# voutcn/megahit

Hardware: NVIDIA H100
Metric: sorted (k+1)-mer edges/sec at k=27 on 150bp reads (higher is better)
Workload: dtype u32

## Files before the change

include/mhb.h:

```cpp
#ifndef MHB_H
#define MHB_H
#include <stddef.h>
#include <stdint.h>

#ifdef __cplusplus
extern "C" {
#endif

#define MHB_OK 0
#define MHB_ERR_ARG 1
#define MHB_ERR_CUDA 2
#define MHB_ERR_IO 3
#define MHB_ERR_NOMEM 4

#define MHB_NUM_BUCKETS 65536
#define MHB_MAX_MUL 65535
#define MHB_MAX_K 255
#define MHB_SENTINEL_OFFSET 0xFFFFFFFFu

const char *mhb_last_error(void);
const char *mhb_version(void);
int mhb_device_count(void);
uint64_t mhb_launch_count(void);

uint32_t mhb_count_record_words(uint32_t k);
uint32_t mhb_words_per_edge(uint32_t k);
uint32_t mhb_s2s_record_words(uint32_t k);
uint32_t mhb_count_sort_bytes(uint32_t k, uint8_t *bytes);
uint32_t mhb_s2s_sort_bytes(uint32_t k, uint8_t *bytes);
size_t mhb_sort_workspace_bytes(uint64_t n, uint32_t words);


typedef struct {
  const uint32_t *bin;
  uint64_t bin_words;
  uint64_t n_reads;
  uint32_t fixed_len;
  const uint64_t *rec_off;
  const uint64_t *edge_off;
} mhb_dev_reads;

int mhb_count_extract(void *stream, const mhb_dev_reads *reads, uint32_t k, uint32_t *records,
                      uint64_t n_edges, uint64_t *hist256, int hist_byte);

int mhb_check_fixed_len(void *stream, const uint32_t *bin_dev, uint64_t n_reads, uint32_t fixed_len, uint64_t *flag_dev);

int mhb_count_extract_range(void *stream, const mhb_dev_reads *reads, uint32_t k, uint32_t lo, uint32_t hi, int write,
                            uint64_t *per_read, uint32_t *records, uint64_t *hist256, int hist_byte,
                            uint64_t *total_dev);

int mhb_count_extract_owners(void *stream, const mhb_dev_reads *reads, uint32_t k, uint64_t *hist16,
                             const uint8_t *owner_of_byte, const uint64_t *owner_base, uint64_t *cursor_dev,
                             const uint64_t *capacity_dev, const uint32_t *round_lo, const uint32_t *round_hi);

int mhb_sort_records(void *stream, uint32_t *a, uint32_t *b, uint64_t n, uint32_t words,
                     const uint8_t *bytes, uint32_t n_bytes, const uint64_t *first_hist, void *ws,
                     size_t ws_bytes, int *result_in_b);

int mhb_sort_records_relaxed(void *stream, uint32_t *a, uint32_t *b, uint64_t n, uint32_t words, const uint8_t *bytes,
                             uint32_t n_bytes, const uint64_t *first_hist, void *ws, size_t ws_bytes, int *result_in_b);

int mhb_s2s_sort(void *stream, uint32_t *a, uint32_t *b, uint64_t n, uint32_t k, const uint64_t *first_hist, void *ws,
                 size_t ws_bytes, int *result_in_b);
size_t mhb_s2s_sort_workspace_bytes(uint64_t n, uint32_t k);
int mhb_s2s_sort_hist_byte(uint64_t n, uint32_t k);
void mhb_s2s_sort_stats(uint64_t *n_oversized, uint64_t *oversized_items, uint64_t *n_large);

int mhb_s2s_sort_emit(void *stream, uint32_t *a, uint32_t *b, uint64_t n, uint32_t k, const uint64_t *first_hist,
                      uint8_t *bytes_out, uint64_t capacity_bytes, uint64_t *bucket_table, uint64_t *totals, void *ws,
                      size_t ws_bytes);
size_t mhb_s2s_sort_emit_workspace_bytes(uint64_t n, uint32_t k);

int mhb_partition_scatter(void *stream, const uint32_t *recs, uint64_t n, uint32_t words, int byte,
                          const uint8_t *owner_of_byte_dev, const uint64_t *bin_addr_dev, void *ws, size_t ws_bytes);
int mhb_partition_scatter_hist(void *stream, const uint32_t *recs, uint64_t n, uint32_t words, int byte,
                               const uint8_t *owner_of_byte_dev, const uint64_t *bin_addr_dev, void *ws, size_t ws_bytes,
                               int next_byte, uint64_t *owner_next_hist);
int mhb_plan_partition(void *stream, const uint64_t *hist_all_dev, uint32_t world, uint32_t rank, uint32_t record_bytes,
                       const uint64_t *peer_base_host, uint8_t *owner_lut_dev, uint64_t *bin_addr_dev, uint64_t *plan_dev);
int mhb_compact_tip_edges(void *stream, const uint32_t *edges, const uint8_t *aux, uint64_t n_solid, uint32_t k,
                          uint32_t *tips_out, uint8_t *tip_aux_out, uint64_t capacity, uint64_t *cursor_dev);
int mhb_dev_malloc(void **ptr, size_t bytes);
int mhb_dev_free(void *ptr);
int mhb_ipc_export(const void *dev_ptr, uint8_t *handle64);
int mhb_ipc_open(const uint8_t *handle64, void **peer_ptr);
int mhb_ipc_close(void *peer_ptr);

int mhb_sort_pass_ms(int back, double *pass_ms, uint32_t max_passes, uint32_t *n_passes, uint64_t *n_records,
                     uint32_t *words);

size_t mhb_count_solid_scratch_bytes(uint64_t n);
int mhb_count_solid(void *stream, const uint32_t *sorted_records, uint64_t n, uint32_t k, int32_t m,
                    uint32_t *edges_out, uint8_t *aux_out, uint64_t capacity_edges, uint64_t *mul_hist,
                    uint64_t *n_solid_out, void *scratch, size_t scratch_bytes);

int mhb_count_hashed_supported(uint32_t k, int32_t m);
size_t mhb_count_hashed_workspace_bytes(uint64_t n, uint32_t k, int32_t m);
int mhb_count_solid_hashed(void *stream, uint32_t *recs_a, uint32_t *recs_b, uint64_t n, uint32_t k, int32_t m,
                           const uint64_t *hist_byte5, uint32_t *edges_out, uint8_t *aux_out, uint64_t capacity_edges,
                           uint64_t *mul_hist, uint64_t *n_solid_out, void *ws, size_t ws_bytes);

size_t mhb_tipset_bytes(uint64_t n_tip_edges, uint32_t k);
int mhb_tipset_build(void *stream, const uint32_t *edges, const uint8_t *aux, uint64_t n_solid, uint32_t k,
                     void *tipset, size_t tipset_bytes, uint64_t n_tip_edges);
int mhb_count_mark_mercy(void *stream, const mhb_dev_reads *reads, uint32_t k, const void *tipset,
                         size_t tipset_bytes, uint64_t n_tip_edges, uint32_t *first_0_out, uint32_t *last_0_in);
int mhb_count_tip_edges(void *stream, const uint8_t *aux, uint64_t n_solid, uint64_t *n_tip_host);

size_t mhb_mercy_candidates_scratch_bytes(uint64_t n_reads);
int mhb_mercy_candidates(void *stream, const uint32_t *first_0_out, const uint32_t *last_0_in, uint64_t n_reads,
                         uint64_t *cand_ids, uint64_t *n_cand_host, void *scratch, size_t scratch_bytes);
size_t mhb_mercy_edges_scratch_bytes(uint64_t n_cand, uint32_t max_read_len);
int mhb_mercy_edges(void *stream, const mhb_dev_reads *reads, const uint64_t *cand_ids, uint64_t n_cand,
                    uint32_t max_read_len, uint32_t k, const uint32_t *edges, uint64_t n_edges, uint32_t *mercy_out,
                    uint64_t capacity, uint64_t *n_mercy_host, void *scratch, size_t scratch_bytes);
int mhb_mercy_edges_count(void *stream, const mhb_dev_reads *reads, const uint64_t *cand_ids, uint64_t n_cand,
                          uint32_t max_read_len, uint32_t k, uint32_t n_segs, const uint32_t *const *seg_edges,
                          const uint64_t *seg_counts, const void *const *seg_luts, const uint8_t *owner_of_byte,
                          uint64_t *n_mercy_host, void *scratch, size_t scratch_bytes);
int mhb_mercy_edges_write(void *stream, const mhb_dev_reads *reads, const uint64_t *cand_ids, uint64_t n_cand,
                          uint32_t max_read_len, uint32_t k, uint32_t *mercy_out, uint64_t capacity, uint64_t n_mercy,
                          void *scratch, size_t scratch_bytes);

size_t mhb_mercy_planes_words(uint64_t n_cand, uint32_t max_read_len);
int mhb_mercy_probe_owned(void *stream, const mhb_dev_reads *reads, const uint64_t *cand_ids, uint64_t n_cand,
                          uint32_t max_read_len, uint32_t k, const uint32_t *edges, uint64_t n_edges, const void *lut,
                          const uint8_t *owner_of_byte, uint32_t me, uint32_t *planes_out);
int mhb_mercy_count_planes(void *stream, const mhb_dev_reads *reads, const uint64_t *cand_ids, uint64_t n_cand,
                           uint32_t max_read_len, uint32_t k, const uint32_t *planes, uint32_t n_src,
                           uint64_t src_stride_words, uint64_t *n_mercy_host, void *scratch, size_t scratch_bytes);

int mhb_mercy_edges_segs(void *stream, const mhb_dev_reads *reads, const uint64_t *cand_ids, uint64_t n_cand,
                         uint32_t max_read_len, uint32_t k, uint32_t n_segs, const uint32_t *const *seg_edges,
                         const uint64_t *seg_counts, const void *const *seg_luts, const uint8_t *owner_of_byte,
                         uint32_t *mercy_out, uint64_t capacity, uint64_t *n_mercy_host, void *scratch,
                         size_t scratch_bytes);
size_t mhb_edge_lut_bytes(void);
int mhb_edge_lut_build(void *stream, const uint32_t *edges, uint64_t n_edges, uint32_t k, void *lut);

typedef struct {
  const uint32_t *words;
  uint64_t n_words;
  uint64_t n_seqs;
  uint32_t fixed_len;
  const uint64_t *word_off;
  const uint32_t *len;
  const uint64_t *item_off;
  const uint16_t *mult;
  uint32_t fixed_stride;
} mhb_dev_seqs;

int mhb_s2s_extract(void *stream, const mhb_dev_seqs *seqs, uint32_t k, uint32_t *records, uint64_t n_items,
                    uint64_t *hist256, int hist_byte);

int mhb_s2s_extract_edges_pruned(void *stream, const uint32_t *edges, const uint8_t *aux, uint64_t n_edges,
                                 uint64_t n_with_aux, uint32_t k, uint32_t *records, uint64_t capacity,
                                 uint64_t *cursor_dev, uint64_t *hist256, int hist_byte);

int mhb_s2s_extract_range(void *stream, const mhb_dev_seqs *seqs, uint32_t k, uint32_t *records, uint64_t n_items,
                          uint32_t lo, uint32_t hi, uint64_t *cursor_dev, uint64_t capacity, uint64_t *hist256,
                          int hist_byte);

int mhb_s2s_extract_owners(void *stream, const mhb_dev_seqs *seqs, uint32_t k, uint64_t n_items,
                           const uint8_t *owner_of_byte, const uint64_t *owner_base, uint64_t *cursor_dev,
                           const uint64_t *capacity_dev);
int mhb_s2s_bucket_hist(void *stream, const mhb_dev_seqs *seqs, uint32_t k, uint64_t n_items, uint64_t *hist16);
int mhb_s2s_extract_owners_round(void *stream, const mhb_dev_seqs *seqs, uint32_t k, uint64_t n_items,
                                 const uint8_t *owner_of_byte, const uint64_t *owner_base, uint64_t *cursor_dev,
                                 const uint64_t *capacity_dev, const uint32_t *round_lo, const uint32_t *round_hi);
int mhb_s2s_edges_owners(void *stream, const uint32_t *edges, const uint8_t *aux, uint64_t n_edges, uint64_t n_with_aux,
                         uint32_t k, uint64_t *hist16, const uint8_t *owner_of_byte, const uint64_t *owner_base,
                         uint64_t *cursor_dev, const uint64_t *capacity_dev, const uint32_t *round_lo,
                         const uint32_t *round_hi);

size_t mhb_s2s_emit_scratch_bytes(uint64_t n, uint32_t k);
int mhb_s2s_emit(void *stream, const uint32_t *sorted_records, uint64_t n, uint32_t k, uint8_t *bytes_out,
                 uint64_t capacity_bytes, uint64_t *bucket_table, uint64_t *totals, void *scratch,
                 size_t scratch_bytes);

int mhb_s2s_emit_fmt(void *stream, const uint32_t *sorted_records, uint64_t n, uint32_t k, uint8_t *bytes_out,
                     uint64_t capacity_bytes, uint64_t *bucket_table, uint64_t *totals, void *scratch,
                     size_t scratch_bytes, int label_fmt);

int mhb_set_device(int device);

typedef struct {
  uint32_t k;
  int32_t m;
  const uint32_t *bin;
  uint64_t bin_words;
  uint64_t n_reads;
  int want_mercy;
} mhb_count_args;

typedef struct {
  uint64_t n_edge_records;
  uint64_t n_solid;
  uint32_t words_per_edge;
  uint32_t *edges;
  uint64_t n_cand;
  uint64_t *cand_ids;
  uint64_t n_has_tips;
  int64_t counting[MHB_MAX_MUL + 1];
  double t_h2d_ms, t_extract_ms, t_sort_ms, t_count_ms, t_mercy_ms, t_d2h_ms, t_total_ms;
  uint32_t n_sort_passes;
  uint32_t n_rounds;
  double sort_pass_ms[64];
} mhb_count_result;

int mhb_count_host(const mhb_count_args *args, mhb_count_result *res);
int mhb_set_round_limit(uint64_t max_records_per_round);
int mhb_set_s2s_round_limit(uint64_t max_items_per_round);
uint64_t mhb_sdbg_round_budget(uint64_t avail_bytes, uint64_t fixed_bytes, uint32_t k, uint64_t n_total);
int mhb_plan_rounds(const uint64_t *hist256, uint64_t max_records, uint32_t *lo_out, uint32_t *hi_out);
int mhb_plan_rounds16(const uint64_t *hist256, const uint64_t *sub_hist, uint64_t max_records, uint32_t *lo16_out,
                      uint32_t *hi16_out, uint32_t cap_out);

int mhb_plan_read_chunks(const uint32_t *bin, uint64_t bin_words, uint64_t n_reads, uint64_t max_chunk_bytes,
                         uint64_t *first_read_out, uint32_t cap_out);
int mhb_read_stream_decide(uint64_t resident_bytes, uint64_t avail_bytes, int plan_failed, uint64_t chunk_limit);
int mhb_set_read_chunk_limit(uint64_t bytes);
int mhb_read_stream_stats(uint64_t *n_chunks, uint64_t *n_passes, uint64_t *h2d_bytes);
int mhb_read_stream_times(double *h2d_ms, double *kernel_ms, double *fill_ms, double *pass_ms);

typedef struct {
  uint32_t k;
  const uint32_t *words;
  const uint64_t *word_off;
  const uint32_t *len;
  const uint16_t *mult;
  uint64_t n_seqs;
} mhb_s2s_args;

typedef struct {
  uint64_t n_records;
  uint64_t n_items, n_tips, n_large_mul, n_bytes;
  uint32_t words_per_tip_label;
  uint8_t *bytes;
  uint64_t bucket_table[MHB_NUM_BUCKETS * 4];
  uint64_t w_count[9];
  uint64_t ones_in_last;
  double t_total_ms, t_extract_ms, t_sort_ms, t_emit_ms;
} mhb_s2s_result;

int mhb_s2s_host(const mhb_s2s_args *args, mhb_s2s_result *res);
int mhb_set_s2s_chunk_limit(uint64_t bytes);
int mhb_plan_seq_chunks(const uint64_t *word_off, const uint32_t *len, uint64_t n_seqs, uint32_t k, uint64_t max_chunk_bytes,
                        uint64_t *first_seq_out, uint32_t cap_out);
int mhb_plan_mercy_segments(const uint32_t *edges, uint64_t n_edges, uint32_t k, uint64_t max_segment_bytes,
                            uint32_t *first_byte_out, uint32_t cap_out);
int mhb_s2s_stream_stats(int mercy, uint64_t *n_chunks, uint64_t *n_passes, uint64_t *n_rounds, uint64_t *h2d_bytes);
int mhb_s2s_stream_times(int mercy, double *h2d_ms, double *kernel_ms, double *fill_ms, double *pass_ms);
int mhb_selftest_s2s_stream_decide(uint64_t n_seqs, uint64_t n_words, uint32_t k, uint64_t free_bytes, uint64_t chunk_limit,
                                   uint64_t *resident_bytes, int *stream);
int mhb_selftest_mercy_auto_plan(const uint64_t *byte_edges, uint32_t k, uint64_t n_cand_reads, uint64_t cand_words,
                                 uint32_t max_read_len, uint64_t free_bytes, uint32_t *first_byte_out, uint64_t *slot_bytes);
int mhb_selftest_mercy_stream_decide(uint64_t n_edges, uint32_t k, uint64_t n_cand_reads, uint64_t cand_words,
                                     uint32_t max_read_len, uint64_t free_bytes, uint64_t chunk_limit,
                                     uint64_t *resident_bytes, int *stream);

typedef struct {
  uint32_t k;
  int32_t m;
  const uint32_t *bin;
  uint64_t bin_words;
  uint64_t n_reads;
  int32_t need_mercy;
  int32_t want_edges;
  uint8_t *sdbg_out;
  uint64_t sdbg_out_capacity;
} mhb_build_args;

typedef struct {
  uint64_t n_edge_records, n_solid, n_cand, n_mercy, n_sort_items;
  uint32_t words_per_edge, words_per_tip_label;
  uint64_t n_items, n_tips, n_large_mul, n_bytes;
  uint8_t *bytes;
  uint64_t *bucket_table;
  uint64_t w_count[9];
  uint64_t ones_in_last;
  uint32_t *edges;
  uint64_t *cand_ids;
  int64_t *counting;
  double t_total_ms, t_h2d_ms, t_count_ms, t_mercy_ms, t_s2s_ms, t_d2h_ms;
  uint32_t n_rounds_s1, n_rounds_s2;
} mhb_build_result;

int mhb_build_host(const mhb_build_args *args, mhb_build_result *res);

int mhb_read2sdbg_host(const mhb_build_args *args, mhb_build_result *res);
int mhb_set_r2s_round_limit(uint64_t max_s1_records, uint64_t max_s2_items);
int mhb_set_r2s_sparse_mercy(int mode);
int mhb_r2s_mercy_stats(int *sparse, uint64_t *n_entries, uint64_t *host_bytes);

typedef struct {
  uint32_t k, step;
  const uint32_t *contig_words;
  const uint64_t *contig_word_off;
  const uint32_t *contig_len;
  uint64_t n_contigs;
  const uint32_t *bin;
  uint64_t bin_words;
  uint64_t n_reads;
} mhb_iterate_args;

typedef struct {
  uint64_t n_flanks;
  uint64_t n_aligned_reads;
  uint64_t n_candidates;
  uint64_t n_edges;
  uint32_t words_per_edge;
  uint32_t *edges;
  double t_total_ms;
} mhb_iterate_result;

int mhb_iterate_host(const mhb_iterate_args *args, mhb_iterate_result *res);

typedef struct {
  const char *type;
  const uint8_t *data[2];
  uint64_t size[2];
} mhb_buildlib_lib;

typedef struct {
  const mhb_buildlib_lib *libs;
  uint32_t n_libs;
} mhb_buildlib_args;

typedef struct {
  uint32_t *bin;
  uint64_t bin_words;
  uint64_t n_reads, n_bases;
  uint32_t n_libs;
  uint64_t *lib_begin, *lib_end;
  uint32_t *lib_max_len;
  uint64_t n_chunks;
  uint64_t n_walk_passes;
  double t_total_ms;
} mhb_buildlib_result;

int mhb_buildlib_host(const mhb_buildlib_args *args, mhb_buildlib_result *res);
void mhb_buildlib_free(mhb_buildlib_result *res);
int mhb_set_buildlib_chunk(uint64_t bytes);

int mhb_mercy_host(uint32_t k, const uint32_t *edges, uint64_t n_edges, const uint32_t *cand_bin, uint64_t cand_words,
                   uint32_t **mercy_out, uint64_t *n_mercy_out, uint64_t *n_cand_reads_out);

void mhb_free(void *p);
int mhb_release(void);

typedef struct {
  uint32_t k;
  int32_t m;
  double host_mem;
  int32_t num_cpu_threads;
  const char *read_lib_file;
  const char *output_prefix;
  int32_t mem_flag;
} mhb_count_opts;

typedef struct {
  double host_mem;
  uint32_t k;
  uint32_t k_from;
  int32_t num_cpu_threads;
  const char *contig;
  const char *bubble;
  const char *addi_contig;
  const char *local_contig;
  const char *input_prefix;
  const char *output_prefix;
  int32_t need_mercy;
  int32_t mem_flag;
} mhb_seq2sdbg_opts;

typedef struct {
  uint32_t k;
  int32_t m;
  double host_mem;
  int32_t num_cpu_threads;
  const char *read_lib_file;
  const char *output_prefix;
  int32_t mem_flag;
  int32_t need_mercy;
} mhb_read2sdbg_opts;

typedef struct {
  const char *contig_file;
  const char *bubble_file;
  const char *read_file;
  int32_t num_cpu_threads;
  uint32_t k;
  uint32_t step;
  const char *output_prefix;
} mhb_iterate_opts;

int mhb_count_run(const mhb_count_opts *opts);
int mhb_seq2sdbg_run(const mhb_seq2sdbg_opts *opts);
int mhb_iterate_run(const mhb_iterate_opts *opts);
int mhb_read2sdbg_run(const mhb_read2sdbg_opts *opts);
int mhb_buildlib_run(const char *lib_file, const char *out_prefix);

int mhb_count_run_multi(const mhb_count_opts *opts, int n_gpus);
// ... 62 lines not shown
```

megahit_b200/csrc/mhb_count.cuh:

```cuda
#pragma once
#include <stdlib.h>
#include <string.h>

#include "mhb.h"
#include "mhb_kernels.cuh"

namespace mhb {

static constexpr int kReadsPerBatch = 64;
static constexpr int kStageWords = 4096;
static constexpr int kExtractThreads = 256;

struct ReadsView {
  const u32 *bin;
  u64 bin_words;
  u64 n_reads;
  u32 fixed_len;
  u32 fixed_stride;
  const u64 *rec_off;
  const u64 *edge_off;
  __device__ __forceinline__ u64 rec_start(u64 r) const { return fixed_len ? r * fixed_stride : rec_off[r]; }
};

template <class F>
__device__ __forceinline__ void for_each_read(const ReadsView &rv, F &&f) {
  __shared__ __align__(16) u32 s_stage[2][kStageWords];
  __shared__ __align__(8) u64 s_bar[2];
  const u32 tid = threadIdx.x, warp = tid >> 5;
  constexpr int NW = kExtractThreads / 32;
  const u64 n_batches = (rv.n_reads + kReadsPerBatch - 1) / kReadsPerBatch;
  if (tid == 0) {
    mbar_init(&s_bar[0], 1);
    mbar_init(&s_bar[1], 1);
    mbar_fence_init();
  }
  __syncthreads();

  auto geom = [&](u64 b, u64 &r0, u64 &r1, u64 &a0, u64 &a1) {
    r0 = b * kReadsPerBatch;
    r1 = r0 + kReadsPerBatch < rv.n_reads ? r0 + kReadsPerBatch : rv.n_reads;
    const u64 w0 = rv.rec_start(r0);
    const u64 w1 = r1 < rv.n_reads ? rv.rec_start(r1) : rv.bin_words;
    a0 = w0 & ~3ull;
    a1 = (w1 + 3) & ~3ull;
  };
  auto issue = [&](u64 b, int st) {
    u64 r0, r1, a0, a1;
    geom(b, r0, r1, a0, a1);
    if (a1 - a0 <= (u64)kStageWords && tid == 0) {
      const u32 bytes = (u32)(a1 - a0) * 4;
      mbar_expect_tx(&s_bar[st], bytes);
      bulk_g2s(&s_stage[st][0], rv.bin + a0, bytes, &s_bar[st]);
    }
  };

  u32 parity[2] = {0, 0};
  u64 b = blockIdx.x;
  int st = 0;
  if (b < n_batches) issue(b, 0);
  for (; b < n_batches; b += gridDim.x, st ^= 1) {
    const u64 nb = b + gridDim.x;
    if (nb < n_batches) issue(nb, st ^ 1);
    u64 r0, r1, a0, a1;
    geom(b, r0, r1, a0, a1);
    const bool staged = (a1 - a0) <= (u64)kStageWords;
    if (staged) {
      mbar_wait(&s_bar[st], parity[st]);
      parity[st] ^= 1;
    }
    for (u64 r = r0 + warp; r < r1; r += NW) {
      const u64 w = rv.rec_start(r);
      const u32 *rec = staged ? &s_stage[st][w - a0] : rv.bin + w;
      const u32 L = rec[0];
      f(r, rec + 1, div_ceil(L, 16), L);
    }
    __syncthreads();
  }
}

template <int W, int WR>
__global__ void __launch_bounds__(kExtractThreads)
    k_count_extract(ReadsView rv, u32 k, u32 *__restrict__ records, u64 *hist, int hist_byte) {
  __shared__ u32 s_hist[256];
  for (int i = threadIdx.x; i < 256; i += kExtractThreads) s_hist[i] = 0;
  const u32 lane = lane_id();
  const u32 K1 = k + 1;
  for_each_read(rv, [&](u64 r, const u32 *s, u32 nwords, u32 L) {
    if (L < K1) return;
    const u32 n_e = L - k;
    const u64 base = rv.fixed_len ? r * (u64)(rv.fixed_len - k) : rv.edge_off[r];
    for (u32 q0 = 0; q0 < n_e; q0 += 32) {
      const u32 q = q0 + lane;
      if (q < n_e) {
        u32 rec[WR], strand;
        make_count_record<W, WR>(s, nwords, L, k, q, rec, strand);
        st_rec<WR>(records, base + q, rec);
        if (hist) atomicAdd(&s_hist[rec_byte<WR>(rec, hist_byte)], 1u);
      }
    }
  });
  __syncthreads();
  if (hist)
    for (int i = threadIdx.x; i < 256; i += kExtractThreads)
      if (s_hist[i]) atomicAdd((unsigned long long *)&hist[i], (unsigned long long)s_hist[i]);
}

static __global__ void __launch_bounds__(kExtractThreads)
    k_count_extract_roll(ReadsView rv, u32 k, u32 *__restrict__ records, u64 *hist, int hist_byte) {
  __shared__ u32 s_hist[256];
  for (int i = threadIdx.x; i < 256; i += kExtractThreads) s_hist[i] = 0;
  const u32 lane = lane_id();
  const u32 K1 = k + 1;
  const u32 hshift = 8u * (u32)hist_byte;
  for_each_read(rv, [&](u64 r, const u32 *s, u32 nwords, u32 L) {
    if (L < K1) return;
    const u32 n_e = L - k;
    const u64 base = rv.fixed_len ? r * (u64)(rv.fixed_len - k) : rv.edge_off[r];
    for (u32 q0 = 0; q0 < n_e; q0 += 128) {
      const u32 q = q0 + 4 * lane;
      if (q < n_e) {
        u64 rec[4];
        u32 strand[4];
        make_count_records_roll<4>(s, nwords, L, k, q, rec, strand);
        const u32 cnt = n_e - q < 4u ? n_e - q : 4u;
#pragma unroll
        for (int j = 0; j < 4; ++j) {
          if ((u32)j < cnt) {
            reinterpret_cast<uint2 *>(records)[base + q + j] = make_uint2((u32)(rec[j] >> 32), (u32)rec[j]);
            if (hist) atomicAdd(&s_hist[(u32)(rec[j] >> hshift) & 255u], 1u);
          }
        }
      }
    }
  });
  __syncthreads();
  if (hist)
    for (int i = threadIdx.x; i < 256; i += kExtractThreads)
      if (s_hist[i]) atomicAdd((unsigned long long *)&hist[i], (unsigned long long)s_hist[i]);
}

template <int W, int WR, bool WRITE>
__global__ void __launch_bounds__(kExtractThreads)
    k_count_extract_range(ReadsView rv, u32 k, u32 lo, u32 hi, u64 *__restrict__ per_read, u32 *__restrict__ records,
                          u64 *hist, int hist_byte) {
  __shared__ u32 s_hist[256];
  for (int i = threadIdx.x; i < 256; i += kExtractThreads) s_hist[i] = 0;
  const u32 lane = lane_id();
  const u32 lt_mask = lanemask_lt();
  const u32 K1 = k + 1;
  for_each_read(rv, [&](u64 r, const u32 *s, u32 nwords, u32 L) {
    if (L < K1) {
      if (!WRITE && lane == 0) per_read[r] = 0;
      return;
    }
    const u32 n_e = L - k;
    u64 run = WRITE ? per_read[r] : 0ull;
    for (u32 q0 = 0; q0 < n_e; q0 += 32) {
      const u32 q = q0 + lane;
      u32 rec[WR], strand;
      bool in = false;
      if (q < n_e) {
        make_count_record<W, WR>(s, nwords, L, k, q, rec, strand);
        const u32 top = rec[0] >> 16;
        in = top >= lo && top <= hi;
      }
      const u32 mask = __ballot_sync(0xffffffffu, in);
      if (in) {
        if constexpr (WRITE) st_rec<WR>(records, run + __popc(mask & lt_mask), rec);
        if (hist) atomicAdd(&s_hist[rec_byte<WR>(rec, hist_byte)], 1u);
      }
      run += __popc(mask);
    }
    if (!WRITE && lane == 0) per_read[r] = run;
  });
  __syncthreads();
  if (hist)
    for (int i = threadIdx.x; i < 256; i += kExtractThreads)
      if (s_hist[i]) atomicAdd((unsigned long long *)&hist[i], (unsigned long long)s_hist[i]);
}

enum { kCountOwnHist = 0, kCountOwnWrite = 1 };
template <int W, int WR, int MODE>
__global__ void __launch_bounds__(kExtractThreads)
    k_count_extract_owners(ReadsView rv, u32 k, unsigned long long *__restrict__ hist16, OwnerSink sink,
                           const u32 *__restrict__ round_lo, const u32 *__restrict__ round_hi) {
  const u32 lane = lane_id(), lt = lanemask_lt();
  const u32 K1 = k + 1;
  for_each_read(rv, [&](u64, const u32 *s, u32 nwords, u32 L) {
    if (L < K1) return;
    const u32 n_e = L - k;
    for (u32 q0 = 0; q0 < n_e; q0 += 32) {
      const u32 q = q0 + lane;
      u32 rec[WR], strand;
      bool in = q < n_e;
      u32 b = 0xFFFFFFFFu;
      if (in) {
        make_count_record<W, WR>(s, nwords, L, k, q, rec, strand);
        b = rec[0] >> 16;
      }
      if constexpr (MODE == kCountOwnHist) {
        const u32 peers = __match_any_sync(0xffffffffu, b);
        if (in && lane == (u32)__ffs(peers) - 1) atomicAdd(hist16 + b, (unsigned long long)__popc(peers));
      } else {
        if (in) {
          const u32 o = __ldg(sink.owner + (b >> 8));
          in = b >= __ldg(round_lo + o) && b <= __ldg(round_hi + o);
        }
        const u32 mask = __ballot_sync(0xffffffffu, in);
        if (mask) sink.template put<WR>(in, rec, mask, lane, lt);
      }
    }
  });
}

template <int WR>
__device__ __forceinline__ bool same_edge(const u32 (&a)[WR], const u32 (&b)[WR]) {
  bool eq = true;
#pragma unroll
  for (int j = 0; j < WR; ++j) {
    const u32 m = (j == WR - 1) ? ~63u : ~0u;
    eq = eq && ((a[j] & m) == (b[j] & m));
  }
  return eq;
}

static constexpr int kMulHistSmem = 1024;

static __global__ void __launch_bounds__(1024) k_scan_u64(u64 *v, u64 nb, u64 *total_out) {
  __shared__ u64 s_w[33];
  __shared__ u64 s_carry;
  if (threadIdx.x == 0) s_carry = 0;
  __syncthreads();
  const u32 lane = lane_id(), warp = threadIdx.x >> 5;
  for (u64 base = 0; base < nb; base += 1024) {
    const u64 i = base + threadIdx.x;
    const u64 x = i < nb ? v[i] : 0;
    u64 inc = x;
#pragma unroll
    for (int d = 1; d < 32; d <<= 1) {
      u64 t = __shfl_up_sync(0xffffffffu, inc, d);
      if (lane >= (u32)d) inc += t;
    }
    if (lane == 31) s_w[warp] = inc;
    __syncthreads();
    if (warp == 0) {
      u64 w = s_w[lane], winc = w;
#pragma unroll
      for (int d = 1; d < 32; d <<= 1) {
        u64 t = __shfl_up_sync(0xffffffffu, winc, d);
        if (lane >= (u32)d) winc += t;
      }
      s_w[lane] = winc - w;
      if (lane == 31) s_w[32] = winc;
    }
    __syncthreads();
    if (i < nb) v[i] = s_carry + s_w[warp] + inc - x;
    __syncthreads();
    if (threadIdx.x == 0) s_carry += s_w[32];
    __syncthreads();
  }
  if (threadIdx.x == 0 && total_out) *total_out = s_carry;
}

struct TipsetHeader {
  u64 capacity;
  u64 filter_words;
  u32 fold;
  u32 filter_bits;
  u32 resident;
  u32 reserved;
};
static_assert(sizeof(TipsetHeader) == 32, "tip set header");
static constexpr u64 kTipFilterSmemWords = 224 * 1024 / 4;
static constexpr u64 kTipMul = 0x9E3779B97F4A7C15ull;

struct TipsetPlan {
  u64 capacity, filter_words;
  u32 fold, filter_bits, resident;
  __host__ __device__ u64 global_words() const { return fold * filter_words; }
  __host__ __device__ u64 folded_words() const { return fold > 1 ? filter_words : 0; }
};

inline TipsetPlan tipset_plan(u64 n_tip, const char *spec) {
  TipsetPlan p;
  p.capacity = 1024;
  while (p.capacity < 2 * n_tip) p.capacity <<= 1;
  char *end = nullptr;
  const unsigned long long forced = spec && *spec ? strtoull(spec, &end, 10) : 0ull;
  if (forced > 0 && end && *end == '\0') {
    p.filter_words = (forced + 3) & ~3ull;
    p.fold = 1;
    p.resident = p.filter_words <= kTipFilterSmemWords;
  } else {
    const u64 want = ((n_tip + 1) / 2 + 3) & ~3ull;
    p.filter_words = want < 1024 ? 1024 : (want > kTipFilterSmemWords ? kTipFilterSmemWords : want);
    p.fold = (u32)((n_tip + p.filter_words - 1) / p.filter_words);
    if (p.fold < 1) p.fold = 1;
    p.resident = 3 * n_tip <= 32 * kTipFilterSmemWords && !(spec && !strcmp(spec, "global"));
  }
  const u64 probed_words = p.resident ? p.filter_words : p.global_words();
  p.filter_bits = 32 * probed_words >= 5 * n_tip ? 3 : 2;
  return p;
}
__host__ __device__ constexpr u32 tipset_slot_words(u32 W) { return W == 2 ? 4u : W + 1; }

template <int W>
__device__ __forceinline__ u32 hash_key(const u32 (&key)[W]) {
  u32 h = 0x9E3779B1u;
#pragma unroll
  for (int j = 0; j < W; ++j) {
    h = (h ^ key[j]) * 0x85EBCA77u;
    h ^= h >> 15;
  }
  h *= 0x2C1B3C6Du;
  return h ^ (h >> 13);
}

__device__ __forceinline__ u64 tip_filter_hash64(u64 key, u32 K1) { return (key >> (64 - 2 * K1)) * kTipMul; }
template <int W>
__device__ __forceinline__ u64 tip_filter_hash(const u32 (&key)[W], u32 K1) {
  if constexpr (W == 1) {
    return (u64)(key[0] >> (32 - 2 * K1)) * kTipMul;
  } else if constexpr (W == 2) {
    return tip_filter_hash64(((u64)key[0] << 32) | key[1], K1);
  } else {
    u64 a = 0;
#pragma unroll
    for (int j = 0; j < W; j += 2) {
      a = (a ^ (((u64)key[j] << 32) | (j + 1 < W ? key[j + 1] : 0u))) * kTipMul;
      a ^= a >> 32;
    }
    return a * kTipMul;
  }
}
__device__ __forceinline__ u32 tip_filter_word(u64 h, u32 n_words) { return __umulhi((u32)(h >> 32), n_words); }
__device__ __forceinline__ u32 tip_filter_mask(u64 h, u32 bits) {
  const u32 lo = (u32)h;
  return (1u << (lo >> 27)) | (1u << ((lo >> 22) & 31u)) | (bits > 2 ? 1u << ((lo >> 17) & 31u) : 0u);
}

static __global__ void k_count_tips(const uint8_t *aux, u64 n, unsigned long long *out) {
  u64 c = 0;
  for (u64 i = (u64)blockIdx.x * blockDim.x + threadIdx.x; i < n; i += (u64)gridDim.x * blockDim.x)
    c += aux[i] != 0;
  for (int d = 16; d; d >>= 1) c += __shfl_xor_sync(0xffffffffu, c, d);
  if (lane_id() == 0 && c) atomicAdd(out, (unsigned long long)c);
}

template <int W>
__global__ void k_tipset_insert(const u32 *__restrict__ edges, const uint8_t *__restrict__ aux, u64 n, u32 k,
                                u32 *filter, TipsetPlan plan, u32 *table) {
  const u64 i = (u64)blockIdx.x * blockDim.x + threadIdx.x;
  if (i >= n || aux[i] == 0) return;
  const u32 WE = words_per_edge(k), SW = tipset_slot_words(W);
  u32 key[W];
#pragma unroll
  for (int j = 0; j < W; ++j) {
    const u32 keep = 2 * (k + 1) - 32 * j;
    key[j] = edges[i * WE + j] & top_mask(keep > 32 ? 32 : keep);
  }
  const u64 fh = tip_filter_hash<W>(key, k + 1);
  atomicOr(&filter[tip_filter_word(fh, (u32)plan.global_words())], tip_filter_mask(fh, plan.filter_bits));
  const u64 cap = plan.capacity;
  u64 slot = hash_key<W>(key) & (cap - 1);
  while (true) {
    u32 *e = table + slot * SW;
    if (atomicCAS(e, 0u, (u32)aux[i]) == 0u) {
#pragma unroll
      for (int j = 0; j < W; ++j) e[1 + j] = key[j];
      return;
    }
    slot = (slot + 1) & (cap - 1);
  }
}

static __global__ void k_tipset_fold(const u32 *__restrict__ filter, u64 n, u32 fold, u32 *__restrict__ folded) {
  for (u64 i = (u64)blockIdx.x * blockDim.x + threadIdx.x; i < n; i += (u64)gridDim.x * blockDim.x) {
    u32 w = 0;
    for (u32 j = 0; j < fold; ++j) w |= filter[i * fold + j];
    folded[i] = w;
  }
}

static constexpr int kMarkThreads = 1024;

struct TipsetDev {
  const u32 *filter;
  const u32 *table;
  u32 n1, n2, filter_bits;
  u64 cap;
  bool smem;
};
__device__ __forceinline__ TipsetDev tipset_open(const void *tipset, u32 smem_words, u32 *s_filter) {
  const TipsetHeader hd = *reinterpret_cast<const TipsetHeader *>(tipset);
  TipsetPlan p;
  p.capacity = hd.capacity;
  p.filter_words = hd.filter_words;
  p.fold = hd.fold;
  TipsetDev t;
  t.filter = reinterpret_cast<const u32 *>((const char *)tipset + sizeof(TipsetHeader));
  t.table = t.filter + p.global_words() + p.folded_words();
  t.filter_bits = hd.filter_bits;
  t.cap = hd.capacity;
  t.smem = hd.resident && hd.filter_words <= smem_words;
  t.n1 = t.smem ? (u32)hd.filter_words : (u32)p.global_words();
  t.n2 = t.smem && hd.fold > 1 ? (u32)p.global_words() : 0u;
  if (t.smem) {
// ... 571 lines not shown
```

megahit_b200/csrc/mhb_device.cu:

```cuda
#include <cuda_runtime.h>
#include <stdarg.h>
#include <stdio.h>
#include <stdlib.h>
#include <string.h>

#include "mhb.h"
#include "mhb_count.cuh"
#include "mhb_internal.h"
#include "mhb_mercy.cuh"
#include "mhb_s2s.cuh"
#include "mhb_common.cuh"

using namespace mhb;

static thread_local char g_err[1024] = "";
int mhb_set_error(int code, const char *fmt, ...) {
  va_list ap;
  va_start(ap, fmt);
  vsnprintf(g_err, sizeof(g_err), fmt, ap);
  va_end(ap);
  return code;
}
extern "C" const char *mhb_last_error(void) { return g_err; }
extern "C" const char *mhb_version(void) { return "megahit_b200 0.1 (sm_90a; formats of megahit v1.2.9)"; }
extern "C" int mhb_device_count(void) {
  int n = 0;
  if (cudaGetDeviceCount(&n) != cudaSuccess) {
    cudaGetLastError();
    return 0;
  }
  return n;
}
extern "C" void mhb_free(void *p) { free(p); }
unsigned long long g_mhb_launches = 0;
extern "C" uint64_t mhb_launch_count(void) { return g_mhb_launches; }


extern "C" uint32_t mhb_count_record_words(uint32_t k) { return count_record_words(k); }
extern "C" uint32_t mhb_words_per_edge(uint32_t k) { return words_per_edge(k); }
extern "C" uint32_t mhb_s2s_record_words(uint32_t k) { return s2s_record_words(k); }

extern "C" uint32_t mhb_count_sort_bytes(uint32_t k, uint8_t *bytes) {
  const u32 wr = count_record_words(k), total_bits = 32 * wr, key_bits = 2 * (k + 1);
  const u32 lo = (total_bits - key_bits) / 8;
  u32 n = 0;
  for (u32 b = lo; b < 4 * wr; ++b) bytes[n++] = (uint8_t)b;
  return n;
}
extern "C" uint32_t mhb_s2s_sort_bytes(uint32_t k, uint8_t *bytes) {
  const u32 w = s2s_record_words(k), total_bits = 32 * w, key_bits = 2 * k;
  const u32 lo = (total_bits - key_bits) / 8;
  u32 n = 0;
  for (u32 b = 2; b < 4 * w; ++b)
    if (b == 2 || b >= lo) bytes[n++] = (uint8_t)b;
  return n;
}


static int g_sm_count = 0;
static int g_bound_device = -1;
int mhb_sm_count() {
  if (!g_sm_count) {
    int dev = 0;
    cudaGetDevice(&dev);
    cudaDeviceGetAttribute(&g_sm_count, cudaDevAttrMultiProcessorCount, dev);
    if (g_sm_count <= 0) g_sm_count = 132;
    if (g_bound_device < 0) g_bound_device = dev;
  }
  return g_sm_count;
}

ReadsView make_reads_view(const mhb_dev_reads *r) {
  ReadsView v;
  v.bin = r->bin;
  v.bin_words = r->bin_words;
  v.n_reads = r->n_reads;
  v.fixed_len = r->fixed_len;
  v.fixed_stride = r->fixed_len ? 1 + div_ceil(r->fixed_len, 16) : 0;
  v.rec_off = r->rec_off;
  v.edge_off = r->edge_off;
  return v;
}

int check_reads(const mhb_dev_reads *r, uint32_t k) {
  if (!r || k < 1 || k > MHB_MAX_K) return mhb_set_error(MHB_ERR_ARG, "bad reads/k (k=%u)", k);
  if (r->n_reads && !r->bin) return mhb_set_error(MHB_ERR_ARG, "reads->bin is NULL");
  if (((uintptr_t)r->bin & 15) != 0) return mhb_set_error(MHB_ERR_ARG, "reads->bin must be 16-byte aligned");
  if (!r->fixed_len && r->n_reads && (!r->rec_off || !r->edge_off))
    return mhb_set_error(MHB_ERR_ARG, "variable-length reads need rec_off and edge_off");
  return MHB_OK;
}

static int grow_scratch(size_t bytes, void **out) {
  static void *buf[64] = {nullptr};
  static size_t cap[64] = {0};
  int dev = 0;
  CK(cudaGetDevice(&dev));
  if (dev < 0 || dev >= 64) return mhb_set_error(MHB_ERR_CUDA, "device index %d out of range", dev);
  if (cap[dev] < bytes) {
    CK(cudaDeviceSynchronize());
    if (buf[dev]) cudaFree(buf[dev]);
    buf[dev] = nullptr;
    cap[dev] = 0;
    const size_t want = (bytes + 4095) & ~(size_t)4095;
    CK(cudaMalloc(&buf[dev], want));
    cap[dev] = want;
  }
  *out = buf[dev];
  return MHB_OK;
}
static int scan64(cudaStream_t st, u64 *v, u64 n, u64 *total_dev, u64 *bsum);

static __global__ void k_check_fixed_len(const u32 *__restrict__ bin, u64 n_reads, u32 stride, u32 L, unsigned long long *flag) {
  bool bad = false;
  for (u64 r = (u64)blockIdx.x * blockDim.x + threadIdx.x; r < n_reads; r += (u64)gridDim.x * blockDim.x) bad |= bin[r * stride] != L;
  if (__any_sync(0xffffffffu, bad) && (threadIdx.x & 31) == 0) atomicOr(flag, 1ull);
}
extern "C" int mhb_check_fixed_len(void *stream, const uint32_t *bin_dev, uint64_t n_reads, uint32_t fixed_len, uint64_t *flag_dev) {
  if (n_reads == 0) return MHB_OK;
  if (!bin_dev || !flag_dev || !fixed_len) return mhb_set_error(MHB_ERR_ARG, "bad arguments");
  k_check_fixed_len<<<mhb_sm_count() * 8, 256, 0, (cudaStream_t)stream>>>(bin_dev, n_reads, 1 + div_ceil(fixed_len, 16), fixed_len,
                                                                     (unsigned long long *)flag_dev);
  CK_LAUNCH();
  return MHB_OK;
}

extern "C" int mhb_count_extract(void *stream, const mhb_dev_reads *reads, uint32_t k, uint32_t *records,
                                 uint64_t n_edges, uint64_t *hist256, int hist_byte) {
  if (int rc = check_reads(reads, k)) return rc;
  if (reads->n_reads == 0 || n_edges == 0) return MHB_OK;
  cudaStream_t st = (cudaStream_t)stream;
  const ReadsView rv = make_reads_view(reads);
  const u32 W = count_key_words(k), WR = count_record_words(k);
  const int grid = (int)grid_cap(rv.n_reads, kReadsPerBatch, 8);
  static const bool roll = getenv("MHB_EXTRACT_ROLL") && !strcmp(getenv("MHB_EXTRACT_ROLL"), "1");
  if (roll && W == 2 && WR == 2 && k + 1 >= 17) {
    k_count_extract_roll<<<grid, kExtractThreads, 0, st>>>(rv, k, records, hist256, hist_byte);
    CK_LAUNCH();
    return MHB_OK;
  }
#define M(WW)                                                                                              \
  if (W == WW && WR == WW)                                                                                 \
    k_count_extract<WW, WW><<<grid, kExtractThreads, 0, st>>>(rv, k, records, hist256, hist_byte);         \
  else if (W == WW && WR == WW + 1)                                                                        \
    k_count_extract<WW, WW + 1><<<grid, kExtractThreads, 0, st>>>(rv, k, records, hist256, hist_byte);     \
  else
  MHB_FOR_W(M) return mhb_set_error(MHB_ERR_ARG, "unsupported k=%u", k);
#undef M
  CK_LAUNCH();
  return MHB_OK;
}

extern "C" int mhb_count_extract_range(void *stream, const mhb_dev_reads *reads, uint32_t k, uint32_t lo, uint32_t hi,
                                       int write, uint64_t *per_read, uint32_t *records, uint64_t *hist256, int hist_byte,
                                       uint64_t *total_dev) {
  if (int rc = check_reads(reads, k)) return rc;
  if (lo > hi || hi > 65535) return mhb_set_error(MHB_ERR_ARG, "bad bucket range [%u, %u]", lo, hi);
  if (!per_read || (write && !records) || (!write && !total_dev)) return mhb_set_error(MHB_ERR_ARG, "null buffer");
  cudaStream_t st = (cudaStream_t)stream;
  if (reads->n_reads == 0) {
    if (!write) CK(cudaMemsetAsync(total_dev, 0, 8, st));
    return MHB_OK;
  }
  const ReadsView rv = make_reads_view(reads);
  const u32 W = count_key_words(k), WR = count_record_words(k);
  const int grid = (int)grid_cap(rv.n_reads, kReadsPerBatch, 8);
#define M2(WW, WRR)                                                                                                   \
  if (W == WW && WR == WRR) {                                                                                         \
    if (write)                                                                                                        \
      k_count_extract_range<WW, WRR, true><<<grid, kExtractThreads, 0, st>>>(rv, k, lo, hi, per_read, records, hist256, hist_byte); \
    else                                                                                                              \
      k_count_extract_range<WW, WRR, false><<<grid, kExtractThreads, 0, st>>>(rv, k, lo, hi, per_read, records, hist256, hist_byte); \
  } else
#define M(WW) M2(WW, WW) M2(WW, WW + 1)
  MHB_FOR_W(M) return mhb_set_error(MHB_ERR_ARG, "unsupported k=%u", k);
#undef M
#undef M2
  CK_LAUNCH();
  if (!write) {
    u64 *bsum = nullptr;
    if (int rc = grow_scratch(((rv.n_reads / kScanTile) + 2) * 8, (void **)&bsum)) return rc;
    if (int rc = scan64(st, per_read, rv.n_reads, total_dev, bsum)) return rc;
    CK(cudaMemcpyAsync(per_read + rv.n_reads, total_dev, 8, cudaMemcpyDeviceToDevice, st));
  }
  return MHB_OK;
}

extern "C" int mhb_count_extract_owners(void *stream, const mhb_dev_reads *reads, uint32_t k, uint64_t *hist16,
                                        const uint8_t *owner_of_byte, const uint64_t *owner_base, uint64_t *cursor_dev,
                                        const uint64_t *capacity_dev, const uint32_t *round_lo, const uint32_t *round_hi) {
  if (int rc = check_reads(reads, k)) return rc;
  if (!hist16 && (!owner_of_byte || !owner_base || !cursor_dev || !capacity_dev || !round_lo || !round_hi))
    return mhb_set_error(MHB_ERR_ARG, "bad args");
  if (reads->n_reads == 0) return MHB_OK;
  cudaStream_t st = (cudaStream_t)stream;
  const ReadsView rv = make_reads_view(reads);
  const u32 W = count_key_words(k), WR = count_record_words(k);
  const int grid = (int)grid_cap(rv.n_reads, kReadsPerBatch, 8);
  const OwnerSink sink{owner_of_byte, owner_base, (unsigned long long *)cursor_dev, capacity_dev};
  unsigned long long *h = (unsigned long long *)hist16;
#define M2(WW, WRR)                                                                                                         \
  if (W == WW && WR == WRR) {                                                                                               \
    if (hist16)                                                                                                             \
      k_count_extract_owners<WW, WRR, kCountOwnHist><<<grid, kExtractThreads, 0, st>>>(rv, k, h, sink, round_lo, round_hi);  \
    else                                                                                                                    \
      k_count_extract_owners<WW, WRR, kCountOwnWrite><<<grid, kExtractThreads, 0, st>>>(rv, k, h, sink, round_lo, round_hi); \
  } else
#define M(WW) M2(WW, WW) M2(WW, WW + 1)
  MHB_FOR_W(M) return mhb_set_error(MHB_ERR_ARG, "unsupported k=%u", k);
#undef M
#undef M2
  CK_LAUNCH();
  return MHB_OK;
}

extern "C" int mhb_count_solid(void *stream, const uint32_t *sorted_records, uint64_t n, uint32_t k, int32_t m,
                               uint32_t *edges_out, uint8_t *aux_out, uint64_t capacity_edges, uint64_t *mul_hist,
                               uint64_t *n_solid_out, void *scratch, size_t scratch_bytes) {
  if (k < 1 || k > MHB_MAX_K || !mul_hist || !n_solid_out) return mhb_set_error(MHB_ERR_ARG, "bad args");
  if (n == 0) return MHB_OK;
  const size_t need = mhb_count_solid_scratch_bytes(n);
  if (scratch_bytes < need) return mhb_set_error(MHB_ERR_ARG, "count scratch too small (%zu < %zu)", scratch_bytes, need);
  cudaStream_t st = (cudaStream_t)stream;
  const u32 WR = count_record_words(k);
  {
#define M(WW)                                                                                                          \
  if (WR == WW) {                                                                                                      \
    constexpr int CH = 32 * count3_ipl(WW);                                                                            \
    const u64 n_chunks = (n + CH - 1) / CH;                                                                            \
    if (n_chunks >= (1ull << 32)) return mhb_set_error(MHB_ERR_ARG, "too many records for one count launch");          \
    const u64 n_sblk = (n_chunks + kScanTile - 1) / kScanTile;                                                         \
    char *p = (char *)scratch;                                                                                         \
    u32 *ticket = (u32 *)p;                                                                                            \
    p += 256;                                                                                                          \
    uint2 *solid_list = (uint2 *)p;                                                                                    \
    p += pad256((size_t)n_chunks * CH * 8);                                                                            \
    u32 *chunk_count = (u32 *)p;                                                                                       \
    p += pad256((size_t)n_chunks * 4);                                                                                 \
    u64 *chunk_off = (u64 *)p;                                                                                         \
    p += pad256((size_t)n_chunks * 8);                                                                                 \
    u64 *bsum = (u64 *)p;                                                                                              \
    CK(cudaMemsetAsync(ticket, 0, 256, st));                                                                           \
    const size_t smem = (size_t)kCount3Warps * count3_warp_words(WW) * 4;                                              \
    static int bps = 0;                                                                                                \
    if (!bps) {                                                                                                        \
      CK(cudaFuncSetAttribute(k_count_lanes<WW>, cudaFuncAttributeMaxDynamicSharedMemorySize, (int)smem));             \
      CK(cudaOccupancyMaxActiveBlocksPerMultiprocessor(&bps, k_count_lanes<WW>, kCount3Warps * 32, smem));             \
      if (bps < 1) bps = 1;                                                                                            \
    }                                                                                                                  \
    u64 grid = (u64)sm_count() * bps;                                                                                  \
    if (grid > (n_chunks + kCount3Warps - 1) / kCount3Warps) grid = (n_chunks + kCount3Warps - 1) / kCount3Warps;      \
    k_count_lanes<WW><<<(unsigned)grid, kCount3Warps * 32, smem, st>>>(sorted_records, n, k, m, (u32)n_chunks, ticket,  \
                                                                      solid_list, chunk_count, mul_hist);             \
    CK_LAUNCH();                                                                                                       \
    k_scan32_sums<<<(unsigned)n_sblk, kScanThreads, 0, st>>>(chunk_count, n_chunks, bsum);                             \
    CK_LAUNCH();                                                                                                       \
    k_scan_u64<<<1, 1024, 0, st>>>(bsum, n_sblk, n_solid_out);                                                         \
    CK_LAUNCH();                                                                                                       \
    k_scan32_apply<<<(unsigned)n_sblk, kScanThreads, 0, st>>>(chunk_count, n_chunks, bsum, chunk_off);                 \
    CK_LAUNCH();                                                                                                       \
    k_count_write<WW><<<grid_cap(n_chunks, 8, 16), 256, 0, st>>>(sorted_records, k, (u32)n_chunks, solid_list, chunk_count, \
                                                    chunk_off, edges_out, aux_out, capacity_edges);                   \
  }
    MHB_FOR_WR(M)
#undef M
    CK_LAUNCH();
    return MHB_OK;
  }
  return mhb_set_error(MHB_ERR_ARG, "unsupported k=%u", k);
}

extern "C" size_t mhb_count_solid_scratch_bytes(uint64_t n) {
  return (size_t)(n + 1024) * 8 + (size_t)(n / 128 + 2) * 12 + (size_t)(n / 128 / kScanTile + 2) * 8 + 4096;
}

static TipsetPlan tipset_plan_env(uint64_t n_tip) { return tipset_plan(n_tip, getenv("MHB_TIPSET_FILTER")); }

extern "C" size_t mhb_tipset_bytes(uint64_t n_tip_edges, uint32_t k) {
  const TipsetPlan p = tipset_plan_env(n_tip_edges);
  return sizeof(TipsetHeader) + (p.global_words() + p.folded_words()) * 4 +
         p.capacity * (size_t)tipset_slot_words(count_key_words(k)) * 4;
}

static int small_scratch(unsigned long long **out) {
  static unsigned long long *buf[64] = {nullptr};
  int dev = 0;
  CK(cudaGetDevice(&dev));
  if (dev < 0 || dev >= 64) return mhb_set_error(MHB_ERR_CUDA, "device index %d out of range", dev);
  if (!buf[dev]) CK(cudaMalloc((void **)&buf[dev], 256));
  *out = buf[dev];
  return MHB_OK;
}

extern "C" int mhb_count_tip_edges(void *stream, const uint8_t *aux, uint64_t n_solid, uint64_t *n_tip_host) {
  cudaStream_t st = (cudaStream_t)stream;
  unsigned long long *d = nullptr;
  *n_tip_host = 0;
  if (n_solid == 0) return MHB_OK;
  if (int rc = small_scratch(&d)) return rc;
  CK(cudaMemsetAsync(d, 0, 8, st));
  k_count_tips<<<sm_count() * 4, 256, 0, st>>>(aux, n_solid, d);
  CK_LAUNCH();
  CK(cudaMemcpyAsync(n_tip_host, d, 8, cudaMemcpyDeviceToHost, st));
  CK(cudaStreamSynchronize(st));
  return MHB_OK;
}

extern "C" int mhb_tipset_build(void *stream, const uint32_t *edges, const uint8_t *aux, uint64_t n_solid, uint32_t k,
                                void *tipset, size_t tipset_bytes, uint64_t n_tip_edges) {
  if (tipset_bytes < mhb_tipset_bytes(n_tip_edges, k)) return mhb_set_error(MHB_ERR_ARG, "tipset too small");
  cudaStream_t st = (cudaStream_t)stream;
  const TipsetPlan plan = tipset_plan_env(n_tip_edges);
  TipsetHeader hdr;
  memset(&hdr, 0, sizeof(hdr));
  hdr.capacity = plan.capacity;
  hdr.filter_words = plan.filter_words;
  hdr.fold = plan.fold;
  hdr.filter_bits = plan.filter_bits;
  hdr.resident = plan.resident;
  CK(cudaMemsetAsync(tipset, 0, mhb_tipset_bytes(n_tip_edges, k), st));
  CK(cudaMemcpyAsync(tipset, &hdr, sizeof(hdr), cudaMemcpyHostToDevice, st));
  if (n_solid == 0) return MHB_OK;
  u32 *filter = (u32 *)((char *)tipset + sizeof(TipsetHeader));
  u32 *table = filter + plan.global_words() + plan.folded_words();
  const u32 W = count_key_words(k);
  const u64 g = (n_solid + 255) / 256;
#define M(WW) \
  if (W == WW) k_tipset_insert<WW><<<(unsigned)g, 256, 0, st>>>(edges, aux, n_solid, k, filter, plan, table);
  MHB_FOR_W(M)
#undef M
  CK_LAUNCH();
  if (plan.fold > 1) {
    k_tipset_fold<<<(unsigned)((plan.filter_words + 255) / 256), 256, 0, st>>>(filter, plan.filter_words, plan.fold,
                                                                              filter + plan.global_words());
    CK_LAUNCH();
  }
  return MHB_OK;
}

template <class Kernel>
static int launch_mark(Kernel kern, int threads, const ReadsView &rv, uint32_t k, const void *tipset, u32 smem_words,
                       uint32_t *first_0_out, uint32_t *last_0_in, cudaStream_t st) {
  const size_t smem = (size_t)smem_words * 4;
  CK(cudaFuncSetAttribute(kern, cudaFuncAttributeMaxDynamicSharedMemorySize, (int)smem));
  int bps = 0;
  CK(cudaOccupancyMaxActiveBlocksPerMultiprocessor(&bps, kern, threads, smem));
  if (bps < 1) return mhb_set_error(MHB_ERR_CUDA, "mercy-mark kernel: no CTA of %d threads and %zu B fits an SM", threads, smem);
  const u64 warps = threads / 32;
  u64 grid = (u64)sm_count() * bps;
  if (grid > (rv.n_reads + warps - 1) / warps) grid = (rv.n_reads + warps - 1) / warps;
  kern<<<(unsigned)grid, threads, smem, st>>>(rv, k, tipset, smem_words, first_0_out, last_0_in);
  CK_LAUNCH();
  return MHB_OK;
}

extern "C" int mhb_count_mark_mercy(void *stream, const mhb_dev_reads *reads, uint32_t k, const void *tipset,
                                    size_t tipset_bytes, uint64_t n_tip_edges, uint32_t *first_0_out,
                                    uint32_t *last_0_in) {
  if (int rc = check_reads(reads, k)) return rc;
  if (reads->n_reads == 0) return MHB_OK;
  if (tipset_bytes < mhb_tipset_bytes(n_tip_edges, k)) return mhb_set_error(MHB_ERR_ARG, "bad tipset");
  cudaStream_t st = (cudaStream_t)stream;
  const ReadsView rv = make_reads_view(reads);
  const u32 W = count_key_words(k), WR = count_record_words(k);
  const TipsetPlan plan = tipset_plan_env(n_tip_edges);
  const u32 smem_words = plan.resident ? (u32)plan.filter_words : 0u;
  static const bool roll = !(getenv("MHB_EXTRACT_ROLL") && !strcmp(getenv("MHB_EXTRACT_ROLL"), "0"));
  if (roll && W == 2 && WR == 2 && k + 1 >= 17)
    return launch_mark(k_mark_mercy_roll, kMarkThreads, rv, k, tipset, smem_words, first_0_out, last_0_in, st);
#define M(WW)                                                                                                          \
  if (W == WW && WR == WW)                                                                                             \
    return launch_mark(k_mark_mercy<WW, WW>, mark_threads(WW), rv, k, tipset, smem_words, first_0_out, last_0_in, st);                   \
  else if (W == WW && WR == WW + 1)                                                                                    \
    return launch_mark(k_mark_mercy<WW, WW + 1>, mark_threads(WW), rv, k, tipset, smem_words, first_0_out, last_0_in, st);               \
  else
  MHB_FOR_W(M) return mhb_set_error(MHB_ERR_ARG, "unsupported k=%u", k);
#undef M
}

static SeqsView make_seqs_view(const mhb_dev_seqs *s) {
  SeqsView v;
  v.words = s->words;
  v.n_words = s->n_words;
  v.n_seqs = s->n_seqs;
  v.fixed_len = s->fixed_len;
  v.word_off = s->word_off;
  v.len = s->len;
  v.item_off = s->item_off;
  v.mult = s->mult;
  v.fixed_stride = s->fixed_stride;
  return v;
}

extern "C" int mhb_s2s_extract(void *stream, const mhb_dev_seqs *seqs, uint32_t k, uint32_t *records,
                               uint64_t n_items, uint64_t *hist256, int hist_byte) {
  if (!seqs || k < 9 || k > MHB_MAX_K) return mhb_set_error(MHB_ERR_ARG, "kmer size must be >= 9 and <= 255");
  if (n_items == 0) return MHB_OK;
  if (!seqs->mult && !(seqs->fixed_len && seqs->fixed_stride))
    return mhb_set_error(MHB_ERR_ARG, "seqs->mult is NULL (only allowed for fixed-stride edge records)");
  if (!seqs->fixed_len && (!seqs->word_off || !seqs->len || !seqs->item_off))
    return mhb_set_error(MHB_ERR_ARG, "variable-length sequences need word_off, len and item_off");
  if (seqs->fixed_len && seqs->fixed_len < k + 1) return mhb_set_error(MHB_ERR_ARG, "fixed_len < k+1");
  cudaStream_t st = (cudaStream_t)stream;
  const SeqsView sv = make_seqs_view(seqs);
  const u32 W = s2s_record_words(k);
  if (seqs->fixed_len == k + 1 && seqs->fixed_stride && !seqs->mult && k + 1 <= 32 && k + 1 > 16 &&
      n_items == seqs->n_seqs * 6) {
    const unsigned ge = grid_cap(seqs->n_seqs, 256, 32);
    if (W == 2) k_s2s_extract_edges<2><<<ge, 256, 0, st>>>(seqs->words, seqs->n_seqs, seqs->fixed_stride, k, records, hist256, hist_byte);
    else if (W == 3) k_s2s_extract_edges<3><<<ge, 256, 0, st>>>(seqs->words, seqs->n_seqs, seqs->fixed_stride, k, records, hist256, hist_byte);
    else return mhb_set_error(MHB_ERR_ARG, "internal: unexpected record width %u", W);
    CK_LAUNCH();
    return MHB_OK;
  }
  const unsigned g = grid_cap(n_items, 256, 32);
#define M(WW) \
  if (W == WW) k_s2s_extract<WW><<<g, 256, 0, st>>>(sv, k, records, n_items, hist256, hist_byte);
  MHB_FOR_WR(M)
#undef M
  CK_LAUNCH();
  return MHB_OK;
}

extern "C" int mhb_s2s_extract_edges_pruned(void *stream, const uint32_t *edges, const uint8_t *aux, uint64_t n_edges,
                                            uint64_t n_with_aux, uint32_t k, uint32_t *records, uint64_t capacity,
                                            uint64_t *cursor_dev, uint64_t *hist256, int hist_byte) {
  if (!edges || (!aux && n_with_aux) || !records || !cursor_dev || k < 9 || k > MHB_MAX_K || n_with_aux > n_edges)
    return mhb_set_error(MHB_ERR_ARG, "bad args");
  if (n_edges == 0) return MHB_OK;
  cudaStream_t st = (cudaStream_t)stream;
  const u32 W = s2s_record_words(k), WE = words_per_edge(k);
  const unsigned g = grid_cap(n_edges, 256, 32);
#define M(WW)                                                                                                        \
  if (W == WW)                                                                                                       \
    k_s2s_extract_edges_pruned<WW><<<g, 256, 0, st>>>(edges, aux, n_edges, n_with_aux, WE, k, records,               \
                                                               (unsigned long long *)cursor_dev, capacity, hist256, hist_byte);
  MHB_FOR_WR(M)
#undef M
  CK_LAUNCH();
  return MHB_OK;
}

template <class Sink>
static int launch_extract_range(cudaStream_t st, const mhb_dev_seqs *seqs, uint32_t k, uint64_t n_items, uint32_t lo,
                                uint32_t hi, const Sink &sink, uint64_t *hist256, int hist_byte) {
  if (!seqs->mult && !(seqs->fixed_len && seqs->fixed_stride))
    return mhb_set_error(MHB_ERR_ARG, "seqs->mult is NULL (only allowed for fixed-stride edge records)");
  if (!seqs->fixed_len && (!seqs->word_off || !seqs->len || !seqs->item_off))
    return mhb_set_error(MHB_ERR_ARG, "variable-length sequences need word_off, len and item_off");
  if (seqs->fixed_len && seqs->fixed_len < k + 1) return mhb_set_error(MHB_ERR_ARG, "fixed_len < k+1");
  const SeqsView sv = make_seqs_view(seqs);
// ... 367 lines not shown
```

megahit_b200/csrc/mhb_hashcount.cu:

```cuda
#include <cuda_runtime.h>
#include <stdio.h>
#include <string.h>

#include "mhb.h"
#include "mhb_common.cuh"
#include "mhb_count.cuh"

using namespace mhb;

namespace {

constexpr int kHcHist = 1024;
constexpr u64 kHcEmpty = ~0ull;
constexpr int kHcBatch = 8;
constexpr u32 kRemBits = 42;
constexpr u32 kHcHotCount = 256;
constexpr int kHcHotRound = 32;
constexpr int kHcMaxProbes = 48;
constexpr int kHcStack = 72;
constexpr u32 kHcHistDone = 1u << 31;
constexpr u32 kHcPrefetchChunk = 16384;

__device__ __forceinline__ u64 rec_key64(const uint2 r) { return ((u64)r.x << 32) | r.y; }

// ... 180 lines not shown
      ntk = atomicAdd(ticket, 1u);
    }
    auto publish_next = [&]() {
      if (tid != 0) return;
      s.nx_sl[(it + 1) & 1] = tk;
      if (tk < n_slices) {
        s.nx_range[(it + 1) & 1] = nx;
        hc_prefetch_l2(recs, nx.x, nx.y);
      }
      tk = ntk;
    };
    if (hi <= lo) {
      publish_next();
      __syncthreads();
      continue;
    }
    const u64 base = lo / (u64)m + sl;
    u32 out_cursor = 0, sp = 0;
    u64 prefix = 0;
    u32 bits = 0;
    bool hist_done = false, first = true;
    while (true) {
      const u32 par = q & 1;
      ++q;
      for (u64 i0 = lo + tid; i0 < hi; i0 += (u64)THREADS * kHcBatch) {
        uint2 v[kHcBatch];
#pragma unroll
        for (int j = 0; j < kHcBatch; ++j) {
          const u64 i = i0 + (u64)j * THREADS;
          v[j] = i < hi ? recs[i] : make_uint2(0, 0);
        }
#pragma unroll
        for (int j = 0; j < kHcBatch; ++j) {
          const u64 i = i0 + (u64)j * THREADS;
          if (i >= hi) break;
          const u64 key = rec_key64(v[j]);
          const u64 r = (key >> 6) & ((1ull << kRemBits) - 1);
          if (bits && (r >> (kRemBits - bits)) != prefix) continue;
          const u32 h = hc_insert<G>(s, r);
          if (h == (u32)SLOTS) {
            s.overflow[par] = 1;
            continue;
          }
          smem_add(&s.cnt[h], 1u);
          const u32 p = (u32)(key >> 3) & 7u, nx_ = (u32)key & 7u;
          if (p < 4) smem_add(&s.pt[h], 1u << (8 * p));
          if (nx_ < 4) smem_add(&s.nt[h], 1u << (8 * nx_));
        }
        if (s.overflow[par]) break;
      }
      if (first) publish_next();
      first = false;
      __syncthreads();
      const bool overflowed = s.overflow[par] != 0;
      if (tid == 0) s.n_solid[par ^ 1] = s.n_hot[par ^ 1] = s.overflow[par ^ 1] = 0;
      const bool count_hist = !overflowed && !hist_done;
      for (u32 slot = tid; slot < (u32)SLOTS; slot += THREADS) {
        const u64 key = s.keys[slot];
        const bool on = key != kHcEmpty;
        u32 c = 0, ptv = 0, ntv = 0;
        if (on) {
          c = s.cnt[slot];
          ptv = s.pt[slot];
          ntv = s.nt[slot];
          s.keys[slot] = kHcEmpty;
          s.cnt[slot] = 0;
          s.pt[slot] = 0;
          s.nt[slot] = 0;
        }
        if (overflowed) continue;
        const u32 c16 = c > 65535u ? 65535u : c;
        if (count_hist) {
          const u32 ones = __ballot_sync(0xffffffffu, on && c16 == 1u), twos = __ballot_sync(0xffffffffu, on && c16 == 2u);
          if (on && c16 > 2u) {
            if (c16 < (u32)kHcHist) smem_add(&s.cta_hist[c16], 1u);
            else atomicAdd((unsigned long long *)&mul_hist[c16], 1ull);
          }
          if ((tid & 31) == 0) {
            if (ones) smem_add(&s.cta_hist[1], (u32)__popc(ones));
            if (twos) smem_add(&s.cta_hist[2], (u32)__popc(twos));
          }
        }
        const bool solid = on && c >= um;
        const u32 sm_ = __ballot_sync(0xffffffffu, solid);
        if (!sm_) continue;
        u32 wbase = 0;
        if ((tid & 31) == 0) wbase = atomicAdd(&s.n_solid[par], (u32)__popc(sm_));
        wbase = __shfl_sync(0xffffffffu, wbase, 0);
        if (solid) {
          const u32 rank = wbase + __popc(sm_ & lane_lt_mask());
          if (rank < (u32)MAX_SOLID) {
            u64 e = (key << 22) | ((u64)c16 << 6);
            if (c >= kHcHotCount) {
              s.hot_rank[atomicAdd(&s.n_hot[par], 1u)] = (uint16_t)rank;
            } else {
              e |= (hc_any_byte_ge(ptv, um) ? 0ull : 1ull) | (hc_any_byte_ge(ntv, um) ? 0ull : 2ull);
            }
            s.sorted[rank] = e;
            smem_add(&s.cell_cur[(u32)((e << bits) >> cshift)], 1u);
          }
        }
      }
      __syncthreads();
      const u32 ns = s.n_solid[par];
      const bool failed = overflowed || ns > (u32)MAX_SOLID;
      if (!failed && ns) {
        const u32 n_hot = s.n_hot[par];
        if (n_hot) {
          for (u32 i = tid; i < n_hot; i += THREADS) {
            const u64 r = s.sorted[s.hot_rank[i]] >> 22;
            u32 h = hc_hash<G>(r);
            while (atomicCAS((unsigned long long *)&s.keys[h], kHcEmpty, r) != kHcEmpty) h = (h + 1) & (SLOTS - 1);
            s.pt[h] = i;
          }
          for (u32 h0 = 0; h0 < n_hot; h0 += kHcHotRound) {
            for (u32 i = tid; i < (u32)kHcHotRound * 8; i += THREADS) s.wide[i >> 3][i & 7] = 0;
            __syncthreads();
            for (u64 i0 = lo + tid; i0 < hi; i0 += (u64)THREADS * kHcBatch) {
              uint2 v[kHcBatch];
#pragma unroll
              for (int j = 0; j < kHcBatch; ++j) {
                const u64 i = i0 + (u64)j * THREADS;
                v[j] = i < hi ? recs[i] : make_uint2(0, 0);
              }
#pragma unroll
              for (int j = 0; j < kHcBatch; ++j) {
                const u64 i = i0 + (u64)j * THREADS;
                if (i >= hi) break;
                const u64 key = rec_key64(v[j]);
                const u64 r = (key >> 6) & ((1ull << kRemBits) - 1);
                if (bits && (r >> (kRemBits - bits)) != prefix) continue;
                const u32 slot = hc_lookup<G>(s, r);
                if (slot == (u32)SLOTS) continue;
                const u32 hidx = s.pt[slot] - h0;
                if (hidx >= (u32)kHcHotRound) continue;
                const u32 p = (u32)(key >> 3) & 7u, nx_ = (u32)key & 7u;
                if (p < 4) smem_add(&s.wide[hidx][p], 1u);
                if (nx_ < 4) smem_add(&s.wide[hidx][4 + nx_], 1u);
              }
            }
            __syncthreads();
            for (u32 i = tid; i < (u32)kHcHotRound && h0 + i < n_hot; i += THREADS) {
              bool has_in = false, has_out = false;
#pragma unroll
              for (int c = 0; c < 4; ++c) {
                has_in = has_in || s.wide[i][c] >= um;
                has_out = has_out || s.wide[i][4 + c] >= um;
              }
              s.sorted[s.hot_rank[h0 + i]] |= (has_in ? 0ull : 1ull) | (has_out ? 0ull : 2ull);
            }
            __syncthreads();
          }
          for (u32 i = tid; i < (u32)SLOTS; i += THREADS) {
            s.keys[i] = kHcEmpty;
            s.pt[i] = 0;
          }
        }
        hc_scan_cells<G>(s);
        for (u32 i = tid; i < ns; i += THREADS) {
          const u64 e = s.sorted[i];
          s.tmp[atomicAdd(&s.cell_cur[(u32)((e << bits) >> cshift)], 1u)] = e;
        }
        __syncthreads();
        for (u32 i = tid; i < (u32)CELLS; i += THREADS) s.cell_cur[i] = 0;
        for (u32 i = tid; i < ns; i += THREADS) {
          const u64 e = s.tmp[i];
          const u32 c = (u32)((e << bits) >> cshift);
          const u32 b0 = s.cell_base[c], b1 = c + 1 < (u32)CELLS ? s.cell_base[c + 1] : ns;
          u32 r = b0;
          for (u32 j = b0; j < b1; ++j) r += s.tmp[j] < e ? 1u : 0u;
          list[base + out_cursor + r] = e;
        }
        out_cursor += ns;
      }
      if (failed) {
        for (u32 i = tid; i < (u32)CELLS; i += THREADS) s.cell_cur[i] = 0;
        if (bits + 2 > kRemBits || sp + 4 > (u32)kHcStack) {
          if (tid == 0) atomicExch(err_flag, 1u);
        } else {
          const u32 flag = (hist_done || !overflowed) ? kHcHistDone : 0u;
          if (tid == 0)
            for (int c = 3; c >= 0; --c) {
              s.st_prefix[sp + 3 - c] = (prefix << 2) | (u64)c;
              s.st_bits[sp + 3 - c] = (bits + 2) | flag;
            }
          sp += 4;
        }
        __syncthreads();
      }
      if (sp == 0) break;
      --sp;
      prefix = s.st_prefix[sp];
      bits = s.st_bits[sp] & ~kHcHistDone;
      hist_done = (s.st_bits[sp] & kHcHistDone) != 0;
    }
    if (tid == 0) slice_count[sl] = out_cursor;
  }
  __syncthreads();
  for (u32 i = tid; i < kHcHist; i += THREADS)
    if (s.cta_hist[i]) atomicAdd((unsigned long long *)&mul_hist[i], (unsigned long long)s.cta_hist[i]);
}

using HcGeomB = HcGeom<512, 12, 2>;

__global__ void k_slice_counts(const u64 *__restrict__ bounds, u32 T, u32 *__restrict__ cnt) {
  const u32 b = blockIdx.x * blockDim.x + threadIdx.x;
  if (b >= 65536u) return;
  const u64 nb = bounds[b + 1] - bounds[b];
  cnt[b] = (u32)((nb + T - 1) / T);
}

__global__ void __launch_bounds__(256)
    k_hash_gather(const u64 *__restrict__ list, const u64 *__restrict__ n_slices_dev, const u32 *__restrict__ slice_count,
                  const u64 *__restrict__ slice_dst, const u64 *__restrict__ slice_base, const u32 *__restrict__ slice_bucket,
                  u32 we, u32 *__restrict__ edges, uint8_t *__restrict__ aux, u64 capacity, const u32 *err_flag,
                  u64 *n_solid_out) {
  const u32 lane = threadIdx.x & 31;
  if (blockIdx.x == 0 && threadIdx.x == 0 && *err_flag) *n_solid_out = ~0ull;
  const u64 n_slices = *n_slices_dev;
  for (u64 sl = (u64)blockIdx.x * 8 + (threadIdx.x >> 5); sl < n_slices; sl += (u64)gridDim.x * 8) {
    const u32 cnt = slice_count[sl];
    if (!cnt) continue;
    const u64 base = slice_base[sl], off = slice_dst[sl], b = slice_bucket[sl];
    for (u32 x = lane; x < cnt; x += 32) {
      if (off + x >= capacity) break;
      const u64 ent = list[base + x];
      const u64 key = (b << 48) | ((ent >> 22) << 6);
      u32 *e = edges + (off + x) * we;
      e[0] = (u32)(key >> 32);
      e[1] = (u32)key;
      if (we == 3) e[2] = 0;
      e[we - 1] |= (u32)(ent >> 6) & 0xFFFFu;
      aux[off + x] = (uint8_t)(ent & 3u);
    }
  }
}

int scan_counts(cudaStream_t st, const u32 *in, u64 n, u64 *out, u64 *total_dev, u64 *bsum) {
  const u64 nb = (n + kScanTile - 1) / kScanTile;
  k_scan32_sums<<<(unsigned)nb, kScanThreads, 0, st>>>(in, n, bsum);
  CK_LAUNCH();
  k_scan_u64<<<1, 1024, 0, st>>>(bsum, nb, total_dev);
  CK_LAUNCH();
  k_scan32_apply<<<(unsigned)nb, kScanThreads, 0, st>>>(in, n, bsum, out);
  CK_LAUNCH();
  return MHB_OK;
}

template <class G>
static int launch_hash_count(cudaStream_t st, const uint2 *recs, const ulonglong2 *plan, const u64 *n_slices_dev, int m, u32 *misc,
                             u64 *list, u32 *slice_count, u64 *mul_hist) {
  static int bps = 0;
  const size_t smem = sizeof(HcShared<G>);
  if (!bps) {
    CK(cudaFuncSetAttribute(k_hash_count<G>, cudaFuncAttributeMaxDynamicSharedMemorySize, (int)smem));
    CK(cudaOccupancyMaxActiveBlocksPerMultiprocessor(&bps, k_hash_count<G>, G::THREADS, smem));
    if (bps < 1) return mhb_set_error(MHB_ERR_CUDA, "hash-count kernel does not fit an SM (%zu B shared memory)", smem);
    if (getenv("MHB_VERBOSE")) fprintf(stderr, "[mhb] hash count: %d threads, %d slots, %zu B smem, %d CTA/SM, slice %u\n", G::THREADS, G::SLOTS, smem, bps, G::SLICE);
  }
  k_hash_count<G><<<sm_count() * bps, G::THREADS, smem, st>>>(recs, plan, n_slices_dev, m, misc, list, slice_count, mul_hist,
                                                             misc + 1);
  CK_LAUNCH();
  return MHB_OK;
}

struct HcLayout {
  size_t sort_ws, off_bounds, off_bcnt, off_soff, off_bsum, off_misc, off_scount, off_sdst, off_sbase, off_sbucket, off_plan,
      off_list, total;
  uint64_t max_slices;
};
HcLayout hc_layout(uint64_t n, int32_t m) {
  HcLayout L;
  L.max_slices = n / HcGeomB::SLICE + 65536 + 2;
  L.sort_ws = pad256(mhb_sort_workspace_bytes(n, 2));
  size_t p = L.sort_ws;
  L.off_bounds = p;
  p += pad256(65537 * 8);
  L.off_bcnt = p;
  p += pad256(65537 * 4);
  L.off_soff = p;
  p += pad256(65537 * 8);
  L.off_bsum = p;
  p += pad256((L.max_slices / kScanTile + 4) * 8);
  L.off_misc = p;
  p += 256;
  L.off_scount = p;
  p += pad256(L.max_slices * 4);
  L.off_sdst = p;
  p += pad256(L.max_slices * 8);
  L.off_sbase = p;
  p += pad256(L.max_slices * 8);
  L.off_sbucket = p;
  p += pad256(L.max_slices * 4);
  L.off_plan = p;
  p += pad256(L.max_slices * 16);
  L.off_list = p;
  p += pad256((size_t)(n / (uint64_t)(m < 1 ? 1 : m) + L.max_slices + 8) * 8);
  L.total = p;
  return L;
}

}

extern "C" int mhb_count_hashed_supported(uint32_t k, int32_t m) {
  return count_record_words(k) == 2 && 2 * (k + 1) >= 24 && m >= 1 && m <= kHcHist;
}

extern "C" size_t mhb_count_hashed_workspace_bytes(uint64_t n, uint32_t k, int32_t m) {
  (void)k;
  return hc_layout(n, m).total;
}

extern "C" int mhb_count_solid_hashed(void *stream, uint32_t *recs_a, uint32_t *recs_b, uint64_t n, uint32_t k, int32_t m,
                                      const uint64_t *hist_byte5, uint32_t *edges_out, uint8_t *aux_out,
                                      uint64_t capacity_edges, uint64_t *mul_hist, uint64_t *n_solid_out, void *ws,
                                      size_t ws_bytes) {
  if (!mhb_count_hashed_supported(k, m)) return mhb_set_error(MHB_ERR_ARG, "hashed count needs 8-byte records (13 <= k <= 28) and 1 <= m <= %d", kHcHist);
  if (!mul_hist || !n_solid_out || !ws) return mhb_set_error(MHB_ERR_ARG, "bad args");
  if (n == 0) return MHB_OK;
  if (n >= (1ull << 40)) return mhb_set_error(MHB_ERR_ARG, "too many records for one hashed count call");
  const HcLayout L = hc_layout(n, m);
  if (ws_bytes < L.total) return mhb_set_error(MHB_ERR_ARG, "hashed count workspace too small (%zu < %zu)", ws_bytes, L.total);
  cudaStream_t st = (cudaStream_t)stream;
  const uint8_t bytes[3] = {5, 6, 7};
  int in_b = 0;
  if (int rc = mhb_sort_records_impl(st, recs_a, recs_b, n, 2, bytes, 3, hist_byte5, ws, L.sort_ws, &in_b, nullptr)) return rc;
  const uint2 *recs = (const uint2 *)(in_b ? recs_b : recs_a);
  char *w = (char *)ws;
  u64 *bounds = (u64 *)(w + L.off_bounds);
  u32 *bcnt = (u32 *)(w + L.off_bcnt);
  u64 *slice_off = (u64 *)(w + L.off_soff);
  u64 *bsum = (u64 *)(w + L.off_bsum);
  u32 *misc = (u32 *)(w + L.off_misc);
  u32 *slice_count = (u32 *)(w + L.off_scount);
  u64 *slice_dst = (u64 *)(w + L.off_sdst);
  u64 *slice_base = (u64 *)(w + L.off_sbase);
  u32 *slice_bucket = (u32 *)(w + L.off_sbucket);
  ulonglong2 *plan = (ulonglong2 *)(w + L.off_plan);
  u64 *list = (u64 *)(w + L.off_list);
  u64 *n_slices_dev = (u64 *)(misc + 2);
  CK(cudaMemsetAsync(misc, 0, 256, st));
  CK(cudaMemsetAsync(slice_count, 0, L.max_slices * 4, st));
  k_bucket_bounds<2><<<(65537 + 255) / 256, 256, 0, st>>>(reinterpret_cast<const u32 *>(recs), n, bounds);
  CK_LAUNCH();
  k_slice_counts<<<65536 / 256, 256, 0, st>>>(bounds, HcGeomB::SLICE, bcnt);
  CK_LAUNCH();
  if (int rc = scan_counts(st, bcnt, 65536, slice_off, n_slices_dev, bsum)) return rc;
  CK(cudaMemcpyAsync(slice_off + 65536, n_slices_dev, 8, cudaMemcpyDeviceToDevice, st));
  k_slice_plan<<<65536 / 256, 256, 0, st>>>(recs, bounds, slice_off, m, plan, slice_base, slice_bucket);
  CK_LAUNCH();
  if (int rc = launch_hash_count<HcGeomB>(st, recs, plan, n_slices_dev, m, misc, list, slice_count, mul_hist)) return rc;
  if (int rc = scan_counts(st, slice_count, L.max_slices, slice_dst, n_solid_out, bsum)) return rc;
  k_hash_gather<<<sm_count() * 4, 256, 0, st>>>(list, n_slices_dev, slice_count, slice_dst, slice_base, slice_bucket,
                                               words_per_edge(k), edges_out, aux_out, capacity_edges, misc + 1, n_solid_out);
  CK_LAUNCH();
  return MHB_OK;
}
```

megahit_b200/csrc/mhb_internal.h:

```cpp
#pragma once
#include <stddef.h>
#include <stdint.h>
#include <stdio.h>
#include <sys/time.h>

#include <algorithm>
#include <functional>
#include <string>
#include <vector>

#include "mhb.h"

int mhb_set_error(int code, const char *fmt, ...);

#define XINFO(...)                                                    \
  do {                                                                \
    fprintf(stderr, "INFO  %-30s: %4d - ", "megahit_b200", __LINE__); \
    fprintf(stderr, __VA_ARGS__);                                     \
  } while (0)

inline double now_s() {
  timeval tv;
  gettimeofday(&tv, nullptr);
  return tv.tv_sec + tv.tv_usec * 1e-6;
}

#define CKR(call)        \
  do {                   \
    int rc_ = (call);    \
    if (rc_) return rc_; \
  } while (0)

inline size_t pad256(size_t bytes) { return (bytes + 255) & ~(size_t)255; }

size_t free_device_bytes();

struct DevBuf {
  void *p = nullptr;
  size_t bytes = 0;
  DevBuf() = default;
  DevBuf(const DevBuf &) = delete;
  DevBuf &operator=(const DevBuf &) = delete;
  ~DevBuf() { release(); }
  int alloc(size_t b, const char *what);
  int ensure(size_t b, const char *what) { return p && bytes >= b ? MHB_OK : alloc(b, what); }
  void release();
  void swap(DevBuf &o) {
    std::swap(p, o.p);
    std::swap(bytes, o.bytes);
  }
  template <class T>
  T *as() const { return reinterpret_cast<T *>(p); }
  static void reset_peak();
  static size_t peak_bytes();
};

template <class F>
uint64_t largest_round(uint64_t n_max, size_t fixed, size_t avail, F bytes) {
  if (fixed + bytes(1) > avail) return 0;
  uint64_t lo = 1, hi = std::max<uint64_t>(n_max, 1);
  while (lo < hi) {
    const uint64_t mid = lo + (hi - lo + 1) / 2;
    if (fixed + bytes(mid) <= avail) lo = mid;
    else hi = mid - 1;
  }
  return lo;
}

struct CountWork {
  bool hashed;
  size_t bytes;
  size_t ws_bytes;
  int hist_byte;
};
CountWork count_work_plan(uint64_t n, uint32_t k, int32_t m);
int run_count_stage(void *stream, const CountWork &cw, uint32_t *d_a, uint32_t *d_b, uint64_t n, uint32_t k, int32_t m,
                    const uint64_t *d_hist0, uint32_t *d_edges, uint8_t *d_aux, uint64_t cap_edges, uint64_t *d_mul_hist,
                    uint64_t *d_nsolid, char *work, double *pass_ms, uint32_t *n_passes);
size_t round_bytes(uint64_t n, uint32_t WR, uint32_t WE, int32_t m, uint32_t k);
uint64_t count_round_limit();

int mhb_sort_records_impl(void *stream, uint32_t *a, uint32_t *b, uint64_t n, uint32_t words, const uint8_t *bytes,
                          uint32_t n_bytes, const uint64_t *first_hist, void *ws, size_t ws_bytes, int *result_in_b,
                          double *pass_ms_host);
int mhb_sort_records_ex(void *stream, uint32_t *a, uint32_t *b, uint64_t n, uint32_t words, const uint8_t *bytes,
                        uint32_t n_bytes, const uint64_t *first_hist, void *ws, size_t ws_bytes, int *result_in_b,
                        double *pass_ms_host, int relaxed);
int mhb_sort_records_untraced(void *stream, uint32_t *a, uint32_t *b, uint64_t n, uint32_t words, const uint8_t *bytes,
                              uint32_t n_bytes, const uint64_t *first_hist, void *ws, size_t ws_bytes, int *result_in_b);

size_t mhb_arena_bytes(void);

struct ReadLibIndex {
  uint32_t fixed_len = 0;
  std::vector<uint64_t> rec_off, unit_off;
  uint64_t n_units = 0;
  uint64_t word_of(uint64_t r) const {
    return fixed_len ? r * (1 + (fixed_len + 15) / 16) : rec_off.empty() ? 0 : rec_off[r];
  }
};
enum class FixedCheck { kFull, kSerial, kSampled };
int index_read_lib(const uint32_t *bin, uint64_t bin_words, uint64_t n_reads, uint32_t k, ReadLibIndex *ix,
                   FixedCheck check = FixedCheck::kFull);
int load_read_lib(const std::string &prefix, std::vector<uint32_t> *bin, long long *n_reads, long long *total_bases);

int write_bytes(const std::string &path, const void *data, size_t n);
int write_sdbg_info(const std::string &prefix, uint32_t k, uint32_t words_per_tip_label, int num_files,
                    const std::vector<const uint64_t *> &tables);
int write_edges_info(const std::string &prefix, uint32_t k, uint32_t words_per_edge,
                     const std::vector<std::vector<int64_t>> &counts);
int write_counting(const std::string &prefix, const int64_t *hist);
void append_cand_reversed(const uint32_t *read, std::vector<uint32_t> *out);
void log_sdbg_summary(const uint64_t tot[16]);

struct StreamStats {
  uint64_t chunks = 0, passes = 0, h2d_bytes = 0;
  double copy_ms = 0, kernel_ms = 0, fill_ms = 0, pass_ms = 0;
};

constexpr int kMaxRanks = 16;
inline uint64_t seq_items(uint32_t len, uint32_t k) { return len >= k + 1 ? 2ull * (len - k + 2) : 0; }
inline void fold_bucket_hist(const uint64_t *h16, uint64_t *h256) {
  for (int b = 0; b < 256; ++b) h256[b] = 0;
  for (int b = 0; b < 65536; ++b) h256[b >> 8] += h16[b];
}
void owner_bounds(const uint64_t *total256, int world, uint32_t *bounds, uint8_t *owner);
using BucketRanges = std::vector<std::pair<uint32_t, uint32_t>>;
int plan_bucket_rounds(const uint64_t *h256, const uint64_t *h16, uint32_t byte_lo, uint32_t byte_hi, uint64_t cap,
                       uint32_t cap_out, int rank, BucketRanges *ranges);
int plan_stage_rounds(const uint64_t *h16, uint64_t cap, BucketRanges *ranges);
int plan_bucket_passes(uint64_t cap, const std::function<int(uint64_t *)> &top,
                       const std::function<int(const std::vector<uint32_t> &, uint64_t *)> &sub, BucketRanges *ranges,
                       std::vector<uint64_t> *pre);
struct OwnerPlan {
  int world = 0;
  uint32_t bounds[kMaxRanks + 1];
  uint8_t owner[256];
  int R = 1;
  std::vector<uint32_t> lo, hi;
  std::vector<uint64_t> n, off;
  size_t at(int t, int o, int s) const { return ((size_t)t * world + o) * world + s; }
};
int plan_owner_rounds(const uint64_t *const *h16, int world, const uint64_t *cap, OwnerPlan *p);
void plan_chunks(const uint64_t *word_off, uint64_t stride_words, uint64_t extra_bytes, uint64_t n, uint64_t max_bytes,
                 std::vector<uint64_t> *first);
void edge_byte_starts(const uint32_t *edges, uint64_t n_edges, uint32_t WE, uint64_t start[257]);
int plan_mercy_segments(const uint64_t start[257], uint32_t WE, uint64_t target, uint64_t limit, std::vector<uint32_t> *first);
void plan_seq_shares(const uint32_t *len, uint64_t n, uint32_t k, uint32_t n_ranks, uint64_t *first);
void plan_read_shares(const uint32_t *bin, const ReadLibIndex &ix, uint64_t n_reads, uint32_t n_ranks, uint64_t *first);

class ChunkStager {
 public:
  struct Copies {
    size_t off[6], bytes[6];
    int n = 0;
    void add(size_t o, size_t b) {
      if (b) {
        off[n] = o;
        bytes[n++] = b;
      }
    }
  };
  using Fill = std::function<int(uint64_t chunk, char *host, Copies *up)>;
  using Run = std::function<int(uint64_t chunk, const char *slot)>;
  ChunkStager() = default;
  ChunkStager(const ChunkStager &) = delete;
  ChunkStager &operator=(const ChunkStager &) = delete;
  ~ChunkStager();
  int init(size_t slot_bytes, uint64_t n_chunks, StreamStats *stats);
  size_t device_bytes() const { return 2 * slot_bytes_; }
  void bind(char *device) { dev_ = device; }
  int pass(void *stream, const Fill &fill, const Run &run);
  int upload(void *stream, const char *host, const std::vector<size_t> &off, const Run &run);

 private:
  int stage(uint64_t i, const Fill &fill);
  size_t slot_bytes_ = 0;
  uint64_t n_chunks_ = 0;
  StreamStats *st_ = nullptr;
  char *dev_ = nullptr;
  char *host_[2] = {nullptr, nullptr};
  void *copy_ = nullptr;
  std::vector<void *> ev_;
};

struct ChunkView {
  uint64_t index, first, n;
  const uint32_t *words;
  uint64_t n_words;
  const void *side[4];
  template <class T>
  const T *at(int j) const { return static_cast<const T *>(side[j]); }
};
class ChunkStream {
 public:
  struct Side {
    const void *host = nullptr;
    uint32_t elem = 0;
  };
  struct Input {
    const uint32_t *image = nullptr;
    uint64_t words = 0;
    uint64_t n = 0;
    const uint64_t *word_off = nullptr;
    uint64_t stride = 0;
    Side side[4];
    uint64_t word_of(uint64_t i) const { return !n ? 0 : word_off ? word_off[i] : i * stride; }
  };
  ChunkStream() = default;
  ChunkStream(const ChunkStream &) = delete;
  ChunkStream &operator=(const ChunkStream &) = delete;
  int init(const Input &in, std::vector<uint64_t> first, StreamStats *stats, uint32_t pieces = 1);
  static size_t image_bytes(uint64_t words) { return pad256(((words * 4 + 15) & ~(uint64_t)15) + 16); }
  static size_t side_bytes(uint64_t units, uint32_t elem) { return pad256((units + 1) * (elem ? elem : 8)); }
  size_t device_bytes() const { return (resident_ ? 1 : 2) * slot_bytes_; }
  int bind(void *device, void *stream);
  uint64_t n_chunks() const { return resident_ ? 0 : first_.size() - 1; }
  uint64_t max_chunk_units() const { return max_units_; }
  const std::vector<uint64_t> &bounds() const { return first_; }
  int pass(void *stream, const std::function<int(const ChunkView &)> &fn);

 private:
  int fill(uint64_t i, char *h, ChunkStager::Copies *up) const;
  ChunkView view(uint64_t i, const char *slot) const;
  Input in_;
  bool resident_ = true;
  std::vector<uint64_t> first_, pieces_;
  uint64_t max_units_ = 0;
  size_t side_at_[4] = {0, 0, 0, 0}, slot_bytes_ = 0;
  char *dev_ = nullptr;
  ChunkStager stager_;
};
int init_read_stream(ChunkStream *rs, const uint32_t *bin, uint64_t bin_words, uint64_t n_reads, const ReadLibIndex &ix,
                     uint64_t max_chunk_bytes, uint32_t pieces = 1);
void read_stream_stats_reset();
uint64_t read_chunk_limit();
uint64_t read_chunk_auto_bytes();

struct HostSeqs {
  std::vector<uint32_t> words;
  std::vector<uint64_t> word_off{0};
  std::vector<uint32_t> len;
  std::vector<uint16_t> mult;
  size_t size() const { return len.size(); }
  void append_packed(const uint32_t *w, uint32_t L, uint16_t m);
  void append_ascii(const char *s, uint32_t L, bool reverse, uint16_t m);
};

int seq2sdbg_check_opts(const mhb_seq2sdbg_opts *o);
bool seq2sdbg_prebuilt(const mhb_seq2sdbg_opts *o, double t0);
int seq2sdbg_load(const mhb_seq2sdbg_opts *o, HostSeqs *seqs);

int iterate_check_opts(const mhb_iterate_opts *o);
int iterate_load(const mhb_iterate_opts *o, HostSeqs *contigs, std::vector<uint32_t> *bin, uint64_t *n_reads);
int iterate_write_info(const std::string &prefix, uint32_t k_out, uint32_t words_per_edge, uint64_t n);

int iterate_check_args(uint32_t k, uint32_t step);
struct IterFlanks {
  DevBuf tab, lut;
  uint64_t n = 0;
};
int iter_build_flanks(const mhb_iterate_args *a, IterFlanks *f);
int iter_collect(const mhb_iterate_args *a, const IterFlanks &f, DevBuf *set, uint64_t *n_set, uint64_t *n_cand,
                 uint64_t *n_aligned);
int iter_sort_unique(uint32_t *a, uint32_t *b, uint64_t n, uint32_t k, uint32_t step, uint32_t **out, uint64_t *n_out);
int hist_byte(void *stream, const uint32_t *recs, uint64_t n, uint32_t words, int byte, uint64_t *hist);

int read2sdbg_load(const mhb_read2sdbg_opts *o, std::vector<uint32_t> *bin, long long *n_reads);
int read2sdbg_build(const mhb_read2sdbg_opts *o, std::vector<uint32_t> &bin, long long n_reads, double t0);

struct OwnerRoute {
  int n_owners;
  const uint8_t *owner;
  const uint64_t *base, *row0, *info0, *off, *cap;
  uint64_t *cursor;
  const uint32_t *lo, *hi;
};

class R2sShare {
 public:
  R2sShare();
  ~R2sShare();
  R2sShare(const R2sShare &) = delete;
  R2sShare &operator=(const R2sShare &) = delete;
  int load(const mhb_build_args *a, const ReadLibIndex &li, uint64_t first, uint64_t end);
  bool want_cand_lists(size_t avail) const;
  int bind_planes(bool lists);
  bool cand_lists() const;
  uint64_t base_of(uint64_t read) const;
  const std::vector<std::vector<uint64_t>> &cand_made() const;
  void cand_take(std::vector<std::vector<uint64_t>> *lists);
  uint32_t s1_record_words() const;
  bool s1_narrow() const;
  uint64_t s1_round_budget(size_t avail, int n_owners, uint64_t n_total) const;
  uint64_t s2_round_budget(size_t avail, uint64_t n_total) const;
  int s1_hist(uint64_t *hist);
  int s2_hist(uint64_t *hist);
  int s1_count(const OwnerRoute &rt);
  int s1_store(const OwnerRoute &rt);
  int s1_own(uint32_t *recs, uint64_t *info, uint64_t n, uint64_t n_max);
  void s1_end();
  void *planes() const;
  int or_planes(const void *peer_planes);
  int mercy_count(uint64_t *n_items, uint64_t *n_mercy);
  int s2_send(const OwnerRoute &rt);
  int s2_own(uint32_t *items, uint64_t n, uint64_t n_max);
  void s2_result(std::vector<uint8_t> *bytes, std::vector<uint64_t> *table, uint64_t *totals);
  int counting(uint64_t *hist);
  uint64_t n_reads() const;

 private:
  struct Impl;
  Impl *d_;
};
int mercy_probe_owned(void *stream, const mhb_dev_reads *reads, const uint64_t *cand_ids, uint64_t n_cand,
                      uint32_t max_read_len, uint32_t k, const uint32_t *edges, uint64_t n_edges, const void *lut,
                      const uint8_t *owner_of_byte, uint32_t me, uint32_t *planes_out, bool accumulate);

struct SdbgStitch {
  std::vector<uint8_t> bytes;
  std::vector<uint64_t> table = std::vector<uint64_t>((size_t)65536 * 4);
  uint64_t tot[16] = {0};
  int append(void *stream, const uint8_t *d_bytes, uint64_t cap_bytes, const uint64_t *d_table, const uint64_t *d_totals);

 private:
  std::vector<uint64_t> round_table = std::vector<uint64_t>((size_t)65536 * 4);
};

template <class R>
void set_sdbg_totals(R *res, const uint64_t tot[16]) {
  res->n_bytes = tot[0];
  res->n_items = tot[1];
  res->n_tips = tot[2];
  res->n_large_mul = tot[3];
  for (int i = 0; i < 9; ++i) res->w_count[i] = tot[4 + i];
  res->ones_in_last = tot[13];
}
template <class R>
void get_sdbg_totals(const R &res, uint64_t tot[16]) {
  std::fill(tot, tot + 16, 0);
  tot[0] = res.n_bytes;
  tot[1] = res.n_items;
  tot[2] = res.n_tips;
  tot[3] = res.n_large_mul;
  for (int i = 0; i < 9; ++i) tot[4 + i] = res.w_count[i];
  tot[13] = res.ones_in_last;
}
```

megahit_b200/csrc/mhb_sort3.cuh:

```cuda
#pragma once
#include "mhb_kernels.cuh"

namespace mhb {

template <int WR>
struct SortGeom {
  static constexpr int THREADS = 384;
  static constexpr int MIN_BLOCKS = 2;
  static constexpr int IPT = WR <= 2 ? 18 : (WR <= 3 ? 12 : (WR <= 4 ? 10 : (WR <= 6 ? 6 : (WR <= 9 ? 4 : 2))));
  static constexpr int TILE = THREADS * IPT;
  static constexpr int NW = THREADS / 32;
  static constexpr size_t SMEM = 256 * 8  + (size_t)NW * 256 * 4  + 256 * 4  +
                                 256 * 4  + 16 * 4  + (size_t)TILE * WR * 4;
};

__global__ void k_hist_scan256(const u64 *hist, u64 *bin_addr, u64 out_addr, u32 rec_bytes) {
  __shared__ u64 s[256];
  const u32 t = threadIdx.x;
  s[t] = hist[t];
  __syncthreads();
  for (int d = 1; d < 256; d <<= 1) {
    u64 v = t >= (u32)d ? s[t - d] : 0;
    __syncthreads();
    s[t] += v;
    __syncthreads();
  }
  bin_addr[t] = out_addr + (s[t] - hist[t]) * rec_bytes;
}

template <int WR>
__global__ void k_hist_byte(const u32 *in, u64 n, int byte_idx, u64 *hist) {
  __shared__ u32 s_h[256];
  for (int i = threadIdx.x; i < 256; i += blockDim.x) s_h[i] = 0;
  __syncthreads();
  for (u64 i = (u64)blockIdx.x * blockDim.x + threadIdx.x; i < n; i += (u64)gridDim.x * blockDim.x) {
    u32 r[WR];
    ld_rec<WR>(in, i, r);
    atomicAdd(&s_h[rec_byte<WR>(r, byte_idx)], 1u);
  }
  __syncthreads();
  for (int i = threadIdx.x; i < 256; i += blockDim.x)
    if (s_h[i]) atomicAdd((unsigned long long *)&hist[i], (unsigned long long)s_h[i]);
}

template <int WR>
__device__ __forceinline__ u32 rec_digit(const u32 (&r)[WR], u32 widx, u32 bsel) {
  u32 w;
  if constexpr (WR == 1) w = r[0];
  else if constexpr (WR == 2) w = widx ? r[1] : r[0];
  else w = pick<WR>(r, widx);
  return __byte_perm(w, 0, 0x4440u | bsel);
}

template <int WR>
__device__ __forceinline__ void ld_rec_pinned(const u32 *base, u64 idx, u32 (&r)[WR]) {
  const u32 *p = base + idx * WR;
  if constexpr (WR % 4 == 0) {
#pragma unroll
    for (int j = 0; j < WR; j += 4)
      asm volatile("ld.global.nc.v4.u32 {%0, %1, %2, %3}, [%4];"
                   : "=r"(r[j]), "=r"(r[j + 1]), "=r"(r[j + 2]), "=r"(r[j + 3])
                   : "l"(p + j));
  } else if constexpr (WR % 2 == 0) {
#pragma unroll
    for (int j = 0; j < WR; j += 2) asm volatile("ld.global.nc.v2.u32 {%0, %1}, [%2];" : "=r"(r[j]), "=r"(r[j + 1]) : "l"(p + j));
  } else {
#pragma unroll
    for (int j = 0; j < WR; ++j) asm volatile("ld.global.nc.u32 %0, [%1];" : "=r"(r[j]) : "l"(p + j));
  }
}

template <int WR>
__device__ __forceinline__ void st_global_rec(u64 addr, const u32 (&q)[WR]) {
  if constexpr (WR % 4 == 0) {
#pragma unroll
    for (int j = 0; j < WR; j += 4)
      asm volatile("st.global.v4.u32 [%0], {%1, %2, %3, %4};" ::"l"(addr + 4 * j), "r"(q[j]), "r"(q[j + 1]), "r"(q[j + 2]), "r"(q[j + 3]));
  } else if constexpr (WR % 2 == 0) {
#pragma unroll
    for (int j = 0; j < WR; j += 2) asm volatile("st.global.v2.u32 [%0], {%1, %2};" ::"l"(addr + 4 * j), "r"(q[j]), "r"(q[j + 1]));
  } else {
#pragma unroll
    for (int j = 0; j < WR; ++j) asm volatile("st.global.u32 [%0], %1;" ::"l"(addr + 4 * j), "r"(q[j]));
  }
}
__device__ __forceinline__ void red_shared_inc(u32 *p) {
  asm volatile("red.shared.add.u32 [%0], 1;" ::"r"(smem_u32(p)));
}
template <int WR>
__device__ __forceinline__ void st_shared_rec(u32 *base, u32 idx, const u32 (&q)[WR]) {
  const u32 a = smem_u32(base) + idx * (WR * 4);
  if constexpr (WR % 4 == 0) {
#pragma unroll
    for (int j = 0; j < WR; j += 4)
      asm volatile("st.shared.v4.u32 [%0], {%1, %2, %3, %4};" ::"r"(a + 4 * j), "r"(q[j]), "r"(q[j + 1]), "r"(q[j + 2]), "r"(q[j + 3]));
  } else if constexpr (WR % 2 == 0) {
#pragma unroll
    for (int j = 0; j < WR; j += 2) asm volatile("st.shared.v2.u32 [%0], {%1, %2};" ::"r"(a + 4 * j), "r"(q[j]), "r"(q[j + 1]));
  } else {
#pragma unroll
    for (int j = 0; j < WR; ++j) asm volatile("st.shared.u32 [%0], %1;" ::"r"(a + 4 * j), "r"(q[j]));
  }
}

#ifdef MHB_SORT_TIMELINE
__device__ unsigned long long *g_sort_timeline = nullptr;
__device__ unsigned long long g_sort_timeline_rows = 0;
#define MHB_TL_DECL                                                                             \
  __shared__ unsigned int s_tl_depth_max, s_tl_depth_sum, s_tl_spin_max, s_tl_spin_sum;         \
  unsigned long long tl_t0 = 0, tl_g0 = 0, tl_v[8] = {0, 0, 0, 0, 0, 0, 0, 0};                  \
  unsigned int tl_depth = 0, tl_spin = 0;
#define MHB_TL_START()                                                                          \
  do {                                                                                          \
    if (tid == 0) {                                                                             \
      tl_t0 = clock64();                                                                        \
      asm volatile("mov.u64 %0, %%globaltimer;" : "=l"(tl_g0));                                 \
      s_tl_depth_max = s_tl_depth_sum = s_tl_spin_max = s_tl_spin_sum = 0;                      \
    }                                                                                           \
    tl_depth = tl_spin = 0;                                                                     \
  } while (0)
#define MHB_TL_MARK(i)                         \
  do {                                         \
    if (tid == 0) tl_v[i] = clock64() - tl_t0; \
  } while (0)
#define MHB_TL_DEPTH() (++tl_depth)
#define MHB_TL_SPIN() (++tl_spin)
#define MHB_TL_LB_DONE()                       \
  do {                                         \
    atomicMax(&s_tl_depth_max, tl_depth);      \
    atomicAdd(&s_tl_depth_sum, tl_depth);      \
    atomicMax(&s_tl_spin_max, tl_spin);        \
    atomicAdd(&s_tl_spin_sum, tl_spin);        \
  } while (0)
#define MHB_TL_FLUSH()                                                                          \
  do {                                                                                          \
    if (tid == 0 && g_sort_timeline && (unsigned long long)tile < g_sort_timeline_rows) {       \
      unsigned long long *row = g_sort_timeline + (unsigned long long)tile * 16;                \
      unsigned int smid;                                                                        \
      asm volatile("mov.u32 %0, %%smid;" : "=r"(smid));                                         \
      row[0] = tile;                                                                            \
      row[1] = smid;                                                                            \
      row[2] = tl_g0;                                                                           \
      for (int q_ = 0; q_ < 8; ++q_) row[3 + q_] = tl_v[q_];                                    \
      row[11] = s_tl_depth_max;                                                                 \
      row[12] = s_tl_depth_sum;                                                                 \
      row[13] = s_tl_spin_max;                                                                  \
      row[14] = s_tl_spin_sum;                                                                  \
      row[15] = blockIdx.x;                                                                     \
    }                                                                                           \
  } while (0)
#else
#define MHB_TL_DECL
#define MHB_TL_START() ((void)0)
#define MHB_TL_MARK(i) ((void)0)
#define MHB_TL_DEPTH() ((void)0)
#define MHB_TL_SPIN() ((void)0)
#define MHB_TL_LB_DONE() ((void)0)
#define MHB_TL_FLUSH() ((void)0)
#endif

template <int WR, bool HAS_NEXT = true>
__global__ void __launch_bounds__(SortGeom<WR>::THREADS, SortGeom<WR>::MIN_BLOCKS)
    k_radix_pass3(const u32 *__restrict__ in, u64 n, u32 num_tiles, int byte_idx,
                  const u64 *__restrict__ bin_addr , u64 *lookback,
                  u32 *tile_counter, u64 *next_hist, int next_byte, u32 epoch) {
  using G = SortGeom<WR>;
  constexpr int THREADS = G::THREADS, IPT = G::IPT, TILE = G::TILE, NW = G::NW;
  constexpr int LB1 = 1, LBW = 2;
  extern __shared__ __align__(16) unsigned char smem_raw[];
  u64 *s_glob = reinterpret_cast<u64 *>(smem_raw);
  u32 *s_cnt = reinterpret_cast<u32 *>(s_glob + 256);
  u32 *s_next = s_cnt + NW * 256;
  u32 *s_early = s_next + 256;
  u32 *s_misc = s_early + 256;
  u32 *s_recs = s_misc + 16;

  const u32 tid = threadIdx.x, lane = tid & 31, warp = tid >> 5;
  const u32 lt_mask = lanemask_lt();
  const u32 widx = (u32)(WR - 1 - (byte_idx >> 2)), bsel = (u32)(byte_idx & 3);
  const u32 nwidx = (u32)(WR - 1 - (next_byte >> 2)), nbsel = (u32)(next_byte & 3);
  u32 *my_cnt = s_cnt + warp * 256;
  MHB_TL_DECL

  for (int i = tid; i < 256; i += THREADS) s_next[i] = 0;
  for (int i = tid; i < 256; i += THREADS) s_early[i] = 0;
  for (int i = tid; i < NW * 256; i += THREADS) s_cnt[i] = 0;
  if (tid == 0) s_misc[0] = atomicAdd(tile_counter, 1u);
  __syncthreads();
  u32 tile = s_misc[0];

  u32 r[IPT][WR];
  auto load_tile = [&](u32 t) {
    const u64 tb = (u64)t * TILE;
    const u64 warp_base = tb + (u64)warp * 32 * IPT + lane;
    if (tb + TILE <= n) {
#pragma unroll
      for (int i = 0; i < IPT; ++i) ld_rec_pinned<WR>(in, warp_base + (u64)i * 32, r[i]);
    } else {
#pragma unroll
      for (int i = 0; i < IPT; ++i) {
        const u64 idx = warp_base + (u64)i * 32;
        if (idx < n) {
          ld_rec_pinned<WR>(in, idx, r[i]);
        } else {
#pragma unroll
          for (int j = 0; j < WR; ++j) r[i][j] = 0xFFFFFFFFu;
        }
      }
    }
  };

  while (tile < num_tiles) {
    u32 next_ticket = 0;
    MHB_TL_START();
    if (tid == 0) next_ticket = atomicAdd(tile_counter, 1u);
    const u64 tile_base = (u64)tile * TILE;
    const bool full = tile_base + TILE <= n;
    const u32 valid = full ? (u32)TILE : (u32)(n - tile_base);

    load_tile(tile);

#ifdef MHB_SORT_TIMELINE
    if (tid == 0) {
      volatile u32 sink = r[0][0];
      (void)sink;
      tl_v[0] = clock64() - tl_t0;
    }
#endif
#pragma unroll
    for (int i = 0; i < IPT; ++i) red_shared_inc(&s_early[rec_digit<WR>(r[i], widx, bsel)]);
    __syncthreads();
    if (tid < 256) {
      const u32 c = s_early[tid] - ((tid == 255u) ? (u32)(TILE - valid) : 0u);
      st_relaxed(lookback + (u64)tile * 256 + tid, (tile == 0 ? kLbInclusive : kLbPartial) | lb_epoch(epoch) | (u64)c);
    }

    MHB_TL_MARK(1);
    u32 rk[IPT];
#pragma unroll
    for (int i = 0; i < IPT; ++i) {
      const u32 d = rec_digit<WR>(r[i], widx, bsel);
      u32 peers = 0xffffffffu;
#pragma unroll
      for (int bit = 0; bit < 8; ++bit) {
        u32 mask;
        asm("{\n\t.reg .pred p;\n\t.reg .b32 t;\n\tand.b32 t, %1, %2;\n\tsetp.ne.u32 p, t, 0;\n\t"
            "vote.sync.ballot.b32 %0, p, 0xffffffff;\n\t@!p not.b32 %0, %0;\n\t}"
            : "=r"(mask)
            : "r"(d), "r"(1u << bit));
        peers &= mask;
      }
      volatile u32 *slot = my_cnt + d;
      const u32 old = *slot;
      __syncwarp();
      const u32 below = __popc(peers & lt_mask);
      if ((peers >> lane) <= 1u) *slot = old + below + 1u;
      __syncwarp();
      rk[i] = ((old + below) << 8) | d;
    }
    __syncthreads();
    MHB_TL_MARK(2);

    u32 total = 0, excl = 0;
    if (tid < 256) {
#pragma unroll
      for (int w = 0; w < NW; ++w) total += s_cnt[w * 256 + tid];
      u32 inc = total;
#pragma unroll
      for (int dd = 1; dd < 32; dd <<= 1) {
        const u32 t = __shfl_up_sync(0xffffffffu, inc, dd);
        if (lane >= (u32)dd) inc += t;
      }
      if (lane == 31) s_misc[4 + warp] = inc;
      excl = inc - total;
    }
    __syncthreads();
    u32 pub = 0;
    u64 win[LB1];
    if (tid == 0) s_misc[0] = next_ticket;
    if (tid < 256) {
#pragma unroll
      for (int w = 0; w < 7; ++w) excl += (warp > (u32)w) ? s_misc[4 + w] : 0u;
      pub = total - ((tid == 255u) ? (u32)(TILE - valid) : 0u);
#pragma unroll
      for (int j = 0; j < LB1; ++j)
        win[j] = (tile > (u32)j) ? ld_relaxed(lookback + (u64)(tile - 1 - j) * 256 + tid) : 0ull;
      u32 run = excl;
#pragma unroll
      for (int w = 0; w < NW; ++w) {
        const u32 c = s_cnt[w * 256 + tid];
        s_cnt[w * 256 + tid] = run;
        run += c;
      }
    }
    __syncthreads();
    MHB_TL_MARK(3);

#pragma unroll
    for (int i = 0; i < IPT; ++i) {
      const u32 pos = my_cnt[rk[i] & 255u] + (rk[i] >> 8);
      st_rec<WR>(s_recs, pos, r[i]);
    }
    MHB_TL_MARK(4);
    const u32 next_tile = s_misc[0];

    if (tid < 256) {
      u64 prefix = 0;
      if (tile > 0) {
        const u64 epv = lb_epoch(epoch);
        u32 p = tile - 1;
        bool done = false;
#pragma unroll
        for (int j = 0; j < LB1; ++j) {
          if (!done) {
            u64 v = win[j];
            const u64 *pp = lookback + (u64)(p - j) * 256 + tid;
            MHB_TL_DEPTH();
            while ((v & kLbStatusMask) == 0 || (v & lb_epoch(255)) != epv) {
              MHB_TL_SPIN();
              v = ld_relaxed(pp);
            }
            prefix += v & kLbValueMask;
            if ((v & kLbStatusMask) == kLbInclusive || p == (u32)j) done = true;
          }
        }
        while (!done) {
          p -= LB1;
          u64 wv[LBW];
#pragma unroll
          for (int j = 0; j < LBW; ++j)
            wv[j] = (p >= (u32)j) ? ld_relaxed(lookback + (u64)(p - j) * 256 + tid) : 0ull;
#pragma unroll
          for (int j = 0; j < LBW; ++j) {
            if (!done) {
              u64 v = wv[j];
              const u64 *pp = lookback + (u64)(p - j) * 256 + tid;
              MHB_TL_DEPTH();
              while ((v & kLbStatusMask) == 0 || (v & lb_epoch(255)) != epv) {
                MHB_TL_SPIN();
                v = ld_relaxed(pp);
              }
              prefix += v & kLbValueMask;
              if ((v & kLbStatusMask) == kLbInclusive || p == (u32)j) done = true;
            }
          }
          p -= (u32)(LBW - LB1);
        }
        st_relaxed(lookback + (u64)tile * 256 + tid, kLbInclusive | epv | (prefix + (u64)pub));
      }
      s_glob[tid] = bin_addr[tid] + (prefix - (u64)excl) * (u64)(WR * 4);
      MHB_TL_LB_DONE();
      MHB_TL_MARK(5);
    }
    __syncthreads();
    MHB_TL_MARK(6);

    {
      uint4 *z = reinterpret_cast<uint4 *>(s_cnt);
      for (int i = tid; i < NW * 256 / 4; i += THREADS) z[i] = make_uint4(0u, 0u, 0u, 0u);
      for (int i = tid; i < 256; i += THREADS) s_early[i] = 0;
    }
    if (full) {
      const u64 my_off = (u64)tid * (WR * 4);
#pragma unroll
      for (int i = 0; i < IPT; ++i) {
        const u32 p = (u32)i * THREADS + tid;
        u32 q[WR];
        ld_rec<WR>(s_recs, p, q);
        const u32 dd = rec_digit<WR>(q, widx, bsel);
        st_rec<WR>(reinterpret_cast<u32 *>(s_glob[dd] + my_off + (u64)i * (THREADS * WR * 4)), 0, q);
        if constexpr (HAS_NEXT) atomicAdd(&s_next[rec_digit<WR>(q, nwidx, nbsel)], 1u);
      }
    } else {
#pragma unroll
      for (int i = 0; i < IPT; ++i) {
        const u32 p = (u32)i * THREADS + tid;
        if (p < valid) {
          u32 q[WR];
          ld_rec<WR>(s_recs, p, q);
          const u32 dd = rec_digit<WR>(q, widx, bsel);
          st_rec<WR>(reinterpret_cast<u32 *>(s_glob[dd] + (u64)p * (WR * 4)), 0, q);
          if constexpr (HAS_NEXT) atomicAdd(&s_next[rec_digit<WR>(q, nwidx, nbsel)], 1u);
        }
      }
    }
    __syncthreads();
    MHB_TL_MARK(7);
    MHB_TL_FLUSH();
    tile = next_tile;
  }

  if constexpr (HAS_NEXT) {
    for (int i = tid; i < 256; i += THREADS)
      if (s_next[i]) atomicAdd((unsigned long long *)&next_hist[i], (unsigned long long)s_next[i]);
  }
}

}
```

megahit_b200/csrc/mhb_sortdisp.cu:

```cuda
#include <cuda_runtime.h>
#include <stdio.h>
#include <stdlib.h>
#include <string.h>

#include "mhb.h"
#include "mhb_common.cuh"
#include "mhb_kernels.cuh"
#include "mhb_sort3.cuh"
#include "mhb_part.cuh"

using namespace mhb;

template <int WR>
static u64 sort_tiles(u64 n) {
  return (n + SortGeom<WR>::TILE - 1) / SortGeom<WR>::TILE;
}
static u64 sort_num_tiles(u64 n, u32 words) {
#define M(WW) \
  if (words == WW) return sort_tiles<WW>(n);
  MHB_FOR_WR(M)
#undef M
  return 0;
}
static constexpr size_t kSortHeadBytes = (size_t)(72 + 1) * 256 * 8  + 256 * 8  + 128 * 4 + 256 * 8 ;

extern "C" size_t mhb_sort_workspace_bytes(uint64_t n, uint32_t words) {
  return kSortHeadBytes + (size_t)sort_num_tiles(n, words) * 256 * 8 + 256;
}

template <int WR>
static int launch_radix_pass(cudaStream_t st, const u32 *in, u64 n, int byte_idx, const u64 *bin_base,
                             u64 *lookback, u32 *tile_counter, u64 *next_hist, int next_byte, u32 epoch) {
  using G = SortGeom<WR>;
  static int blocks_per_sm = 0;
  if (!blocks_per_sm) {
    CK(cudaFuncSetAttribute(k_radix_pass3<WR, true>, cudaFuncAttributeMaxDynamicSharedMemorySize, (int)G::SMEM));
    CK(cudaFuncSetAttribute(k_radix_pass3<WR, false>, cudaFuncAttributeMaxDynamicSharedMemorySize, (int)G::SMEM));
    CK(cudaOccupancyMaxActiveBlocksPerMultiprocessor(&blocks_per_sm, k_radix_pass3<WR, true>, G::THREADS, G::SMEM));
    if (blocks_per_sm < 1) return mhb_set_error(MHB_ERR_CUDA, "radix pass kernel (WR=%d) does not fit an SM", WR);
    if (getenv("MHB_VERBOSE")) fprintf(stderr, "[mhb] radix pass WR=%d: %d threads x %d rec, %zu B smem, %d CTA/SM\n", WR, G::THREADS, G::IPT, G::SMEM, blocks_per_sm);
  }
  const u64 tiles = sort_tiles<WR>(n);
  u64 grid = (u64)blocks_per_sm * sm_count();
  if (grid > tiles) grid = tiles;
  if (next_hist)
    k_radix_pass3<WR, true><<<(int)grid, G::THREADS, G::SMEM, st>>>(in, n, (u32)tiles, byte_idx, bin_base, lookback,
                                                                     tile_counter, next_hist, next_byte, epoch);
  else
    k_radix_pass3<WR, false><<<(int)grid, G::THREADS, G::SMEM, st>>>(in, n, (u32)tiles, byte_idx, bin_base, lookback,
                                                                      tile_counter, nullptr, 0, epoch);
  CK_LAUNCH();
  return MHB_OK;
}

template <int WR, bool OWNER_LUT>
static int launch_part_unstable(cudaStream_t st, const u32 *in, u64 n, int byte_idx, const u64 *bin_base,
                                unsigned long long *gcursor, u32 *tile_counter, u64 *next_hist, int next_byte,
                                const uint8_t *lut) {
  using C = PartCfg<WR>;
  constexpr size_t SMEM_HIST = OWNER_LUT ? C::SMEM_OWNER_HIST : C::SMEM;
  static int bps = 0;
  if (!bps) {
    CK(cudaFuncSetAttribute(k_part_unstable<WR, OWNER_LUT, true>, cudaFuncAttributeMaxDynamicSharedMemorySize, (int)SMEM_HIST));
    CK(cudaFuncSetAttribute(k_part_unstable<WR, OWNER_LUT, false>, cudaFuncAttributeMaxDynamicSharedMemorySize, (int)C::SMEM));
    CK(cudaOccupancyMaxActiveBlocksPerMultiprocessor(&bps, k_part_unstable<WR, OWNER_LUT, true>, C::THREADS, SMEM_HIST));
    if (bps < 1) return mhb_set_error(MHB_ERR_CUDA, "partition pass (WR=%d) does not fit an SM", WR);
    if (getenv("MHB_VERBOSE")) fprintf(stderr, "[mhb] unstable partition pass WR=%d owner=%d: %d threads x %d rec, %zu B smem, %d CTA/SM\n", WR, (int)OWNER_LUT, C::THREADS, C::IPT, SMEM_HIST, bps);
  }
  const u64 tiles = (n + C::TILE - 1) / C::TILE;
  u64 grid = (u64)bps * sm_count();
  if (grid > tiles) grid = tiles;
  if (next_hist)
    k_part_unstable<WR, OWNER_LUT, true><<<(int)grid, C::THREADS, SMEM_HIST, st>>>(in, n, (u32)tiles, byte_idx, bin_base, gcursor,
                                                                                   tile_counter, next_hist, next_byte, lut);
  else
    k_part_unstable<WR, OWNER_LUT, false><<<(int)grid, C::THREADS, C::SMEM, st>>>(in, n, (u32)tiles, byte_idx, bin_base, gcursor,
                                                                                  tile_counter, nullptr, 0, lut);
  CK_LAUNCH();
  return MHB_OK;
}

#ifdef MHB_SORT_TIMELINE
extern "C" int mhb_debug_set_sort_timeline(unsigned long long *dev_buf, unsigned long long rows) {
  CK(cudaMemcpyToSymbol(g_sort_timeline, &dev_buf, sizeof(dev_buf)));
  CK(cudaMemcpyToSymbol(g_sort_timeline_rows, &rows, sizeof(rows)));
  return MHB_OK;
}
#endif

namespace {
struct SortTrace {
  cudaEvent_t ev[74];
  bool created = false;
  uint32_t n_passes = 0, words = 0;
  uint64_t n = 0;
};
SortTrace g_trace[4];
uint64_t g_trace_seq = 0;
}

static int sort_records_core(void *stream, uint32_t *a, uint32_t *b, uint64_t n, uint32_t words, const uint8_t *bytes,
                             uint32_t n_bytes, const uint64_t *first_hist, void *ws, size_t ws_bytes, int *result_in_b,
                             double *pass_ms_host, int relaxed, bool trace);
int mhb_sort_records_impl(void *stream, uint32_t *a, uint32_t *b, uint64_t n, uint32_t words, const uint8_t *bytes,
                          uint32_t n_bytes, const uint64_t *first_hist, void *ws, size_t ws_bytes, int *result_in_b,
                          double *pass_ms_host) {
  return sort_records_core(stream, a, b, n, words, bytes, n_bytes, first_hist, ws, ws_bytes, result_in_b, pass_ms_host, 1, true);
}
int mhb_sort_records_ex(void *stream, uint32_t *a, uint32_t *b, uint64_t n, uint32_t words, const uint8_t *bytes,
                        uint32_t n_bytes, const uint64_t *first_hist, void *ws, size_t ws_bytes, int *result_in_b,
                        double *pass_ms_host, int relaxed) {
  return sort_records_core(stream, a, b, n, words, bytes, n_bytes, first_hist, ws, ws_bytes, result_in_b, pass_ms_host, relaxed, true);
}
int mhb_sort_records_untraced(void *stream, uint32_t *a, uint32_t *b, uint64_t n, uint32_t words, const uint8_t *bytes,
                              uint32_t n_bytes, const uint64_t *first_hist, void *ws, size_t ws_bytes, int *result_in_b) {
  return sort_records_core(stream, a, b, n, words, bytes, n_bytes, first_hist, ws, ws_bytes, result_in_b, nullptr, 1, false);
}
static int sort_records_core(void *stream, uint32_t *a, uint32_t *b, uint64_t n, uint32_t words, const uint8_t *bytes,
                             uint32_t n_bytes, const uint64_t *first_hist, void *ws, size_t ws_bytes, int *result_in_b,
                             double *pass_ms_host, int relaxed, bool trace) {
  if (pass_ms_host && !trace) return mhb_set_error(MHB_ERR_ARG, "per-pass times need a traced sort");
  if (words < 1 || words > 17 || n_bytes > 72 || !result_in_b)
    return mhb_set_error(MHB_ERR_ARG, "bad sort geometry (words=%u n_bytes=%u)", words, n_bytes);
  *result_in_b = 0;
  if (n == 0 || n_bytes == 0) return MHB_OK;
  if (ws_bytes < mhb_sort_workspace_bytes(n, words)) return mhb_set_error(MHB_ERR_ARG, "sort workspace too small");
  if (n >= (1ull << 53)) return mhb_set_error(MHB_ERR_ARG, "too many records");
  cudaStream_t st = (cudaStream_t)stream;
  u64 *hist = (u64 *)ws;
  u64 *bin_base = hist + (72 + 1) * 256;
  u32 *tile_counter = (u32 *)(bin_base + 256);
  unsigned long long *gcursor = (unsigned long long *)(tile_counter + 128);
  u64 *lookback = (u64 *)((char *)ws + kSortHeadBytes);
  CK(cudaMemsetAsync(ws, 0, mhb_sort_workspace_bytes(n, words), st));
  if (first_hist) {
    CK(cudaMemcpyAsync(hist, first_hist, 256 * 8, cudaMemcpyDeviceToDevice, st));
  } else {
#define M(WW) \
  if (words == WW) k_hist_byte<WW><<<sm_count() * 4, 256, 0, st>>>(a, n, bytes[0], hist);
    MHB_FOR_WR(M)
#undef M
    CK_LAUNCH();
  }
  SortTrace *tr = nullptr;
  if (trace) {
    tr = &g_trace[g_trace_seq++ & 3];
    if (!tr->created) {
      for (int i = 0; i < 74; ++i) CK(cudaEventCreate(&tr->ev[i]));
      tr->created = true;
    }
    tr->n_passes = n_bytes;
    tr->words = words;
    tr->n = n;
    CK(cudaEventRecord(tr->ev[0], st));
  }
  u32 *in = a, *out = b;
  for (u32 p = 0; p < n_bytes; ++p) {
    k_hist_scan256<<<1, 256, 0, st>>>(hist + (u64)p * 256, bin_base, (u64)(uintptr_t)out, words * 4);
    CK_LAUNCH();
    u64 *next_hist = p + 1 < n_bytes ? hist + (u64)(p + 1) * 256 : nullptr;
    const int next_byte = p + 1 < n_bytes ? bytes[p + 1] : 0;
    int rc = MHB_ERR_ARG;
    if (p == 0 && relaxed && words == 2) rc = launch_part_unstable<2, false>(st, in, n, bytes[p], bin_base, gcursor, tile_counter + p, next_hist, next_byte, nullptr);
    else if (p == 0 && relaxed && words == 3) rc = launch_part_unstable<3, false>(st, in, n, bytes[p], bin_base, gcursor, tile_counter + p, next_hist, next_byte, nullptr);
    else {
#define M(WW) \
  if (words == WW) rc = launch_radix_pass<WW>(st, in, n, bytes[p], bin_base, lookback, tile_counter + p, next_hist, next_byte, p + 1);
      MHB_FOR_WR(M)
#undef M
    }
    if (rc) return rc;
    if (tr) CK(cudaEventRecord(tr->ev[p + 1], st));
    u32 *t = in;
    in = out;
    out = t;
  }
  *result_in_b = (in == b) ? 1 : 0;
  if (pass_ms_host) {
    CK(cudaEventSynchronize(tr->ev[n_bytes]));
    for (u32 p = 0; p < n_bytes; ++p) {
      float ms = 0;
      CK(cudaEventElapsedTime(&ms, tr->ev[p], tr->ev[p + 1]));
      pass_ms_host[p] = ms;
    }
  }
  return MHB_OK;
}

int hist_byte(void *stream, const uint32_t *recs, uint64_t n, uint32_t words, int byte, uint64_t *hist) {
  if (words < 1 || words > 17 || byte < 0 || byte >= (int)(4 * words)) return mhb_set_error(MHB_ERR_ARG, "bad geometry");
  if (n == 0) return MHB_OK;
  cudaStream_t st = (cudaStream_t)stream;
#define M(WW) \
  if (words == WW) k_hist_byte<WW><<<sm_count() * 4, 256, 0, st>>>(recs, n, byte, hist);
  MHB_FOR_WR(M)
#undef M
  CK_LAUNCH();
  return MHB_OK;
}

static int partition_scatter_impl(void *stream, const uint32_t *recs, uint64_t n, uint32_t words, int byte,
                                  const uint8_t *owner_of_byte_dev, const uint64_t *bin_addr_dev, void *ws, size_t ws_bytes,
                                  int next_byte, uint64_t *owner_next_hist) {
  if (words < 1 || words > 17 || byte < 0 || byte >= (int)(4 * words)) return mhb_set_error(MHB_ERR_ARG, "bad geometry");
  if (!owner_of_byte_dev) return mhb_set_error(MHB_ERR_ARG, "the partition pass needs an owner table");
  if (n == 0) return MHB_OK;
  if (ws_bytes < kSortHeadBytes) return mhb_set_error(MHB_ERR_ARG, "sort workspace too small");
  cudaStream_t st = (cudaStream_t)stream;
  u32 *tile_counter = (u32 *)((u64 *)ws + (72 + 1) * 256 + 256);
  unsigned long long *gcursor = (unsigned long long *)(tile_counter + 128);
  CK(cudaMemsetAsync(ws, 0, kSortHeadBytes, st));
  int rc = MHB_ERR_ARG;
#define M(WW)                                                                                                        \
  if (words == WW)                                                                                                   \
    rc = launch_part_unstable<WW, true>(st, recs, n, byte, bin_addr_dev, gcursor, tile_counter, owner_next_hist, next_byte, \
                                        owner_of_byte_dev);
  MHB_FOR_WR(M)
#undef M
  return rc;
}
extern "C" int mhb_partition_scatter(void *stream, const uint32_t *recs, uint64_t n, uint32_t words, int byte,
                                     const uint8_t *owner_of_byte_dev, const uint64_t *bin_addr_dev, void *ws,
                                     size_t ws_bytes) {
  return partition_scatter_impl(stream, recs, n, words, byte, owner_of_byte_dev, bin_addr_dev, ws, ws_bytes, 0, nullptr);
}
extern "C" int mhb_partition_scatter_hist(void *stream, const uint32_t *recs, uint64_t n, uint32_t words, int byte,
                                          const uint8_t *owner_of_byte_dev, const uint64_t *bin_addr_dev, void *ws,
                                          size_t ws_bytes, int next_byte, uint64_t *owner_next_hist) {
  if (!owner_next_hist || next_byte < 0 || next_byte >= (int)(4 * words))
    return mhb_set_error(MHB_ERR_ARG, "bad owner-histogram arguments");
  return partition_scatter_impl(stream, recs, n, words, byte, owner_of_byte_dev, bin_addr_dev, ws, ws_bytes, next_byte,
                                owner_next_hist);
}

extern "C" int mhb_dev_malloc(void **ptr, size_t bytes) {
  CK(cudaMalloc(ptr, bytes));
  return MHB_OK;
}
extern "C" int mhb_dev_free(void *ptr) {
  CK(cudaFree(ptr));
  return MHB_OK;
}
extern "C" int mhb_ipc_export(const void *dev_ptr, uint8_t *handle64) {
  static_assert(sizeof(cudaIpcMemHandle_t) == 64, "handle size");
  cudaIpcMemHandle_t h;
  CK(cudaIpcGetMemHandle(&h, const_cast<void *>(dev_ptr)));
  memcpy(handle64, &h, 64);
  return MHB_OK;
}
extern "C" int mhb_ipc_open(const uint8_t *handle64, void **peer_ptr) {
  cudaIpcMemHandle_t h;
  memcpy(&h, handle64, 64);
  CK(cudaIpcOpenMemHandle(peer_ptr, h, cudaIpcMemLazyEnablePeerAccess));
  return MHB_OK;
}
extern "C" int mhb_ipc_close(void *peer_ptr) {
  CK(cudaIpcCloseMemHandle(peer_ptr));
  return MHB_OK;
}

extern "C" int mhb_sort_pass_ms(int back, double *pass_ms, uint32_t max_passes, uint32_t *n_passes, uint64_t *n_records,
                                uint32_t *words) {
  if (back < 0 || back > 3 || (uint64_t)back >= g_trace_seq) return mhb_set_error(MHB_ERR_ARG, "no such sort in the trace ring");
  SortTrace &tr = g_trace[(g_trace_seq - 1 - back) & 3];
  CK(cudaEventSynchronize(tr.ev[tr.n_passes]));
  for (u32 p = 0; p < tr.n_passes && p < max_passes; ++p) {
    float ms = 0;
    CK(cudaEventElapsedTime(&ms, tr.ev[p], tr.ev[p + 1]));
    pass_ms[p] = ms;
  }
  if (n_passes) *n_passes = tr.n_passes;
  if (n_records) *n_records = tr.n;
  if (words) *words = tr.words;
  return MHB_OK;
}

extern "C" int mhb_sort_records(void *stream, uint32_t *a, uint32_t *b, uint64_t n, uint32_t words,
                                const uint8_t *bytes, uint32_t n_bytes, const uint64_t *first_hist, void *ws,
                                size_t ws_bytes, int *result_in_b) {
  return mhb_sort_records_ex(stream, a, b, n, words, bytes, n_bytes, first_hist, ws, ws_bytes, result_in_b, nullptr, 0);
}

extern "C" int mhb_sort_records_relaxed(void *stream, uint32_t *a, uint32_t *b, uint64_t n, uint32_t words,
                                        const uint8_t *bytes, uint32_t n_bytes, const uint64_t *first_hist, void *ws,
                                        size_t ws_bytes, int *result_in_b) {
  return mhb_sort_records_ex(stream, a, b, n, words, bytes, n_bytes, first_hist, ws, ws_bytes, result_in_b, nullptr, 1);
}
```

megahit_b200/dev.py:

```python
from __future__ import annotations

import ctypes as C
import os

import numpy as np
import torch

from . import lib


def _ptr(t):
    return C.c_void_p(t.data_ptr()) if t is not None else None


def _stream():
    return C.c_void_p(torch.cuda.current_stream().cuda_stream)


def sort_records(a: torch.Tensor, b: torch.Tensor, n: int, words: int, sort_bytes, first_hist=None, ws=None, relaxed=False):
    L = lib.load()
    need = L.mhb_sort_workspace_bytes(n, words)
    if ws is None or ws.numel() < need:
        ws = torch.empty(need, dtype=torch.uint8, device=a.device)
    bytes_arr = (C.c_uint8 * len(sort_bytes))(*sort_bytes)
    in_b = C.c_int(0)
    fn = L.mhb_sort_records_relaxed if relaxed else L.mhb_sort_records
    lib._check(fn(_stream(), _ptr(a), _ptr(b), n, words, bytes_arr, len(sort_bytes), _ptr(first_hist), _ptr(ws), ws.numel(),
                  C.byref(in_b)))
    return b if in_b.value else a


def s2s_sort(a: torch.Tensor, b: torch.Tensor, n: int, k: int, first_hist=None, ws=None):
    L = lib.load()
    need = L.mhb_s2s_sort_workspace_bytes(n, k)
    if ws is None or ws.numel() < need:
        ws = torch.empty(need, dtype=torch.uint8, device=a.device)
    in_b = C.c_int(0)
    lib._check(L.mhb_s2s_sort(_stream(), _ptr(a), _ptr(b), n, k, _ptr(first_hist), _ptr(ws), ws.numel(), C.byref(in_b)))
    return b if in_b.value else a


def s2s_sort_emit(a: torch.Tensor, b: torch.Tensor, n: int, k: int, first_hist, bytes_out: torch.Tensor, table: torch.Tensor,
                  totals: torch.Tensor, ws=None, cap_bytes: int | None = None):
    L = lib.load()
    need = L.mhb_s2s_sort_emit_workspace_bytes(n, k)
    if ws is None or ws.numel() < need:
        ws = torch.empty(need, dtype=torch.uint8, device=a.device)
    cap = bytes_out.numel() if cap_bytes is None else cap_bytes
    lib._check(L.mhb_s2s_sort_emit(_stream(), _ptr(a), _ptr(b), n, k, _ptr(first_hist), _ptr(bytes_out), cap, _ptr(table),
                                   _ptr(totals), _ptr(ws), ws.numel()))
    return totals


class CountPlan:

    def __init__(self, n_reads: int, read_len: int, k: int, m: int, device, want_mercy: bool = True, mode: str | None = None):
        import os
        L = lib.load()
        self.L, self.k, self.m, self.n_reads, self.read_len, self.device = L, k, m, n_reads, read_len, device
        self.want_mercy = want_mercy
        mode = mode or os.environ.get("MHB_COUNT_MODE") or "auto"
        ok = bool(L.mhb_count_hashed_supported(k, m))
        if mode == "hashed" and not ok:
            raise lib.MhbError(f"hashed count is not available for k={k}, m={m}")
        self.hashed = ok and mode in ("hashed", "auto")
        self.n = n_reads * (read_len - k) if read_len >= k + 1 else 0
        self.WR, self.WE = lib.count_record_words(k), lib.words_per_edge(k)
        self.sort_bytes = lib.count_sort_bytes(k)
        n = self.n
        i32 = dict(dtype=torch.int32, device=device)
        self.a = torch.empty(n * self.WR + 4, **i32)
        self.b = torch.empty(n * self.WR + 4, **i32)
        if self.hashed:
            self.ws = torch.empty(L.mhb_count_hashed_workspace_bytes(n, k, m), dtype=torch.uint8, device=device)
            self.scratch = None
        else:
            self.ws = torch.empty(L.mhb_sort_workspace_bytes(n, self.WR), dtype=torch.uint8, device=device)
            self.scratch = torch.empty(L.mhb_count_solid_scratch_bytes(n), dtype=torch.uint8, device=device)
        self.cap_edges = n // max(1, m) + 1
        self.edges = torch.empty(self.cap_edges * self.WE, **i32)
        self.aux = torch.empty(self.cap_edges, dtype=torch.uint8, device=device)
        self.mul_hist = torch.zeros(65536, dtype=torch.int64, device=device)
        self.hist0 = torch.zeros(256, dtype=torch.int64, device=device)
        self.n_solid_dev = torch.zeros(8, dtype=torch.int64, device=device)
        self.first = torch.empty(n_reads + 1, **i32) if want_mercy else None
        self.last = torch.empty(n_reads + 1, **i32) if want_mercy else None
        self.tipset = None
        self.events = {}

    def _reads(self, bin_dev: torch.Tensor) -> lib.DevReads:
        return lib.DevReads(bin_dev.data_ptr(), bin_dev.numel(), self.n_reads, self.read_len, None, None)

    def _mark(self, name):
        ev = torch.cuda.Event(enable_timing=True)
        ev.record()
        self.events.setdefault(name, []).append(ev)

    def extract(self, bin_dev):
        self.hist0.zero_()
        lib._check(self.L.mhb_count_extract(_stream(), C.byref(self._reads(bin_dev)), self.k, _ptr(self.a), self.n,
                                            _ptr(self.hist0), 5 if self.hashed else self.sort_bytes[0]))

    def sort(self):
        if self.hashed:
            return None
        self.sorted = sort_records(self.a, self.b, self.n, self.WR, self.sort_bytes, self.hist0, self.ws, relaxed=True)
        return self.sorted

    def count(self):
        self.mul_hist.zero_()
        self.n_solid_dev.zero_()
        if self.hashed:
            lib._check(self.L.mhb_count_solid_hashed(_stream(), _ptr(self.a), _ptr(self.b), self.n, self.k, self.m,
                                                     _ptr(self.hist0), _ptr(self.edges), _ptr(self.aux), self.cap_edges,
                                                     _ptr(self.mul_hist), _ptr(self.n_solid_dev), _ptr(self.ws), self.ws.numel()))
            return
        lib._check(self.L.mhb_count_solid(_stream(), _ptr(self.sorted), self.n, self.k, self.m, _ptr(self.edges),
                                          _ptr(self.aux), self.cap_edges, _ptr(self.mul_hist), _ptr(self.n_solid_dev),
                                          _ptr(self.scratch), self.scratch.numel()))

    def mercy(self, bin_dev):
        n_solid = int(self.n_solid_dev[0].item())
        n_tip = C.c_uint64(0)
        lib._check(self.L.mhb_count_tip_edges(_stream(), _ptr(self.aux), n_solid, C.byref(n_tip)))
        need = self.L.mhb_tipset_bytes(n_tip.value, self.k)
        if self.tipset is None or self.tipset.numel() < need:
            self.tipset = torch.empty(need, dtype=torch.uint8, device=self.device)
        lib._check(self.L.mhb_tipset_build(_stream(), _ptr(self.edges), _ptr(self.aux), n_solid, self.k,
                                           _ptr(self.tipset), need, n_tip.value))
        lib._check(self.L.mhb_count_mark_mercy(_stream(), C.byref(self._reads(bin_dev)), self.k, _ptr(self.tipset),
                                               need, n_tip.value, _ptr(self.first), _ptr(self.last)))
        return n_solid, n_tip.value

    def mercy_edges(self, bin_dev: torch.Tensor, n_solid: int) -> int:
        L = self.L
        if not hasattr(self, "cand"):
            self.cand = torch.empty(self.n_reads + 1, dtype=torch.int64, device=self.device)
            self.cand_scratch = torch.empty(L.mhb_mercy_candidates_scratch_bytes(self.n_reads), dtype=torch.uint8, device=self.device)
            self.mercy_scratch = None
        nc = C.c_uint64(0)
        lib._check(L.mhb_mercy_candidates(_stream(), _ptr(self.first), _ptr(self.last), self.n_reads, _ptr(self.cand), C.byref(nc),
                                          _ptr(self.cand_scratch), self.cand_scratch.numel()))
        self.n_cand = nc.value
        if not self.n_cand:
            return 0
        need = L.mhb_mercy_edges_scratch_bytes(self.n_cand, self.read_len)
        if self.mercy_scratch is None or self.mercy_scratch.numel() < need:
            self.mercy_scratch = torch.empty(int(need * 1.2), dtype=torch.uint8, device=self.device)
        nm = C.c_uint64(0)
        lib._check(L.mhb_mercy_edges(_stream(), C.byref(self._reads(bin_dev)), _ptr(self.cand), self.n_cand, self.read_len, self.k,
                                     _ptr(self.edges), n_solid, C.c_void_p(self.edges.data_ptr() + n_solid * self.WE * 4),
                                     self.cap_edges - n_solid, C.byref(nm), _ptr(self.mercy_scratch), self.mercy_scratch.numel()))
        return nm.value

    def run(self, bin_dev: torch.Tensor, timed: bool = False):
        if timed:
            self._mark("t0")
        self.extract(bin_dev)
        if timed:
            self._mark("extract")
        self.sort()
        if timed:
            self._mark("sort")
        self.count()
        if timed:
            self._mark("count")
        if self.want_mercy:
            n_solid, _ = self.mercy(bin_dev)
        else:
            n_solid = int(self.n_solid_dev[0].item())
        if timed:
            self._mark("mercy")
        return n_solid

    def edges_host(self, n_solid: int) -> np.ndarray:
        return self.edges[: n_solid * self.WE].cpu().numpy().view(np.uint32).reshape(-1, self.WE)


class S2sPlan:

    def __init__(self, n_seqs: int, seq_len: int, k: int, device):
        L = lib.load()
        self.L, self.k, self.n_seqs, self.seq_len, self.device = L, k, n_seqs, seq_len, device
        self.W = lib.s2s_record_words(k)
        self.sort_bytes = lib.s2s_sort_bytes(k)
        self.n_items = n_seqs * 2 * (seq_len - k + 2)
        n = self.n_items
        i32 = dict(dtype=torch.int32, device=device)
        self.a = torch.empty(n * self.W + 4, **i32)
        self.b = torch.empty(n * self.W + 4, **i32)
        self.ws = torch.empty(L.mhb_s2s_sort_emit_workspace_bytes(n, k), dtype=torch.uint8, device=device)
        wpt = (k + 15) // 16
        self.cap_bytes = n * (4 + 4 * wpt) + 16
        self.bytes = torch.empty(self.cap_bytes, dtype=torch.uint8, device=device)
        self.table = torch.zeros(65536 * 4, dtype=torch.int64, device=device)
        self.totals = torch.zeros(16, dtype=torch.int64, device=device)
        self.hist0 = torch.zeros(256, dtype=torch.int64, device=device)
        self.cursor = torch.zeros(1, dtype=torch.int64, device=device)
        self.events = []

    def run(self, words: torch.Tensor, mult: torch.Tensor | None = None, n_seqs: int | None = None, stride: int = 0,
            timed: bool = False, aux: torch.Tensor | None = None, n_aux: int = 0):
        n_seqs = self.n_seqs if n_seqs is None else n_seqs
        assert n_seqs <= self.n_seqs
        self.n_items = n_seqs * 2 * (self.seq_len - self.k + 2)
        if aux is not None and mult is None and not os.environ.get("MHB_S2S_NO_PRUNE"):
            return self._run_pruned(words, n_seqs, aux, n_aux, timed)
        seqs = lib.DevSeqs(words.data_ptr(), words.numel(), n_seqs, self.seq_len, None, None, None,
                           mult.data_ptr() if mult is not None else None, stride)
        self.hist0.zero_()
        ev = [torch.cuda.Event(enable_timing=True) for _ in range(4)] if timed else None
        if timed:
            ev[0].record()
        lib._check(self.L.mhb_s2s_extract(_stream(), C.byref(seqs), self.k, _ptr(self.a), self.n_items, _ptr(self.hist0),
                                          lib.s2s_sort_hist_byte(self.n_items, self.k)))
        if timed:
            ev[1].record()
        self._sort_emit(self.hist0)
        if timed:
            ev[2].record()
            ev[3].record()
            self.events.append(ev)
        return self.totals

    def _sort_emit(self, hist):
        s2s_sort_emit(self.a, self.b, self.n_items, self.k, hist, self.bytes, self.table, self.totals, self.ws, self.cap_bytes)

    def _run_pruned(self, edges: torch.Tensor, n_edges: int, aux: torch.Tensor, n_aux: int, timed: bool):
        cap = self.n_items
        self.hist0.zero_()
        self.cursor.zero_()
        ev = [torch.cuda.Event(enable_timing=True) for _ in range(4)] if timed else None
        if timed:
            ev[0].record()
        lib._check(self.L.mhb_s2s_extract_edges_pruned(_stream(), _ptr(edges), _ptr(aux), n_edges, n_aux, self.k, _ptr(self.a),
                                                       cap, _ptr(self.cursor), _ptr(self.hist0),
                                                       lib.s2s_sort_hist_byte(cap, self.k)))
        self.n_items = int(self.cursor.item())
        assert self.n_items <= cap
        if timed:
            ev[1].record()
        same = lib.s2s_sort_hist_byte(self.n_items, self.k) == lib.s2s_sort_hist_byte(cap, self.k)
        self._sort_emit(self.hist0 if same else None)
        if timed:
            ev[2].record()
            ev[3].record()
            self.events.append(ev)
        return self.totals
```

megahit_b200/lib.py:

```python
from __future__ import annotations

import ctypes as C
import os

import numpy as np

_HERE = os.path.dirname(os.path.abspath(__file__))
LIB_PATH = os.environ.get("MHB_LIB") or os.path.join(_HERE, "libmhb.so")
NUM_BUCKETS = 65536
SENTINEL_OFFSET = 0xFFFFFFFF

_lib = None


class MhbError(RuntimeError):
    pass


class DevReads(C.Structure):
    _fields_ = [("bin", C.c_void_p), ("bin_words", C.c_uint64), ("n_reads", C.c_uint64), ("fixed_len", C.c_uint32),
                ("rec_off", C.c_void_p), ("edge_off", C.c_void_p)]


class DevSeqs(C.Structure):
    _fields_ = [("words", C.c_void_p), ("n_words", C.c_uint64), ("n_seqs", C.c_uint64), ("fixed_len", C.c_uint32),
                ("word_off", C.c_void_p), ("len", C.c_void_p), ("item_off", C.c_void_p), ("mult", C.c_void_p),
                ("fixed_stride", C.c_uint32)]


class CountArgs(C.Structure):
    _fields_ = [("k", C.c_uint32), ("m", C.c_int32), ("bin", C.c_void_p), ("bin_words", C.c_uint64),
                ("n_reads", C.c_uint64), ("want_mercy", C.c_int)]


class CountResult(C.Structure):
    _fields_ = [("n_edge_records", C.c_uint64), ("n_solid", C.c_uint64), ("words_per_edge", C.c_uint32),
                ("edges", C.POINTER(C.c_uint32)), ("n_cand", C.c_uint64), ("cand_ids", C.POINTER(C.c_uint64)),
                ("n_has_tips", C.c_uint64), ("counting", C.c_int64 * 65536),
                ("t_h2d_ms", C.c_double), ("t_extract_ms", C.c_double), ("t_sort_ms", C.c_double),
                ("t_count_ms", C.c_double), ("t_mercy_ms", C.c_double), ("t_d2h_ms", C.c_double),
                ("t_total_ms", C.c_double), ("n_sort_passes", C.c_uint32), ("n_rounds", C.c_uint32), ("sort_pass_ms", C.c_double * 64)]


class S2sArgs(C.Structure):
    _fields_ = [("k", C.c_uint32), ("words", C.c_void_p), ("word_off", C.c_void_p), ("len", C.c_void_p),
                ("mult", C.c_void_p), ("n_seqs", C.c_uint64)]


class S2sResult(C.Structure):
    _fields_ = [("n_records", C.c_uint64), ("n_items", C.c_uint64), ("n_tips", C.c_uint64),
                ("n_large_mul", C.c_uint64), ("n_bytes", C.c_uint64), ("words_per_tip_label", C.c_uint32),
                ("bytes", C.POINTER(C.c_uint8)), ("bucket_table", C.c_uint64 * (65536 * 4)),
                ("w_count", C.c_uint64 * 9), ("ones_in_last", C.c_uint64),
                ("t_total_ms", C.c_double), ("t_extract_ms", C.c_double), ("t_sort_ms", C.c_double),
                ("t_emit_ms", C.c_double)]


class BuildArgs(C.Structure):
    _fields_ = [("k", C.c_uint32), ("m", C.c_int32), ("bin", C.c_void_p), ("bin_words", C.c_uint64),
                ("n_reads", C.c_uint64), ("need_mercy", C.c_int32), ("want_edges", C.c_int32),
                ("sdbg_out", C.c_void_p), ("sdbg_out_capacity", C.c_uint64)]


class BuildResult(C.Structure):
    _fields_ = [("n_edge_records", C.c_uint64), ("n_solid", C.c_uint64), ("n_cand", C.c_uint64), ("n_mercy", C.c_uint64),
                ("n_sort_items", C.c_uint64), ("words_per_edge", C.c_uint32), ("words_per_tip_label", C.c_uint32),
                ("n_items", C.c_uint64), ("n_tips", C.c_uint64), ("n_large_mul", C.c_uint64), ("n_bytes", C.c_uint64),
                ("bytes", C.POINTER(C.c_uint8)), ("bucket_table", C.POINTER(C.c_uint64)), ("w_count", C.c_uint64 * 9),
                ("ones_in_last", C.c_uint64), ("edges", C.POINTER(C.c_uint32)), ("cand_ids", C.POINTER(C.c_uint64)),
                ("counting", C.POINTER(C.c_int64)),
                ("t_total_ms", C.c_double), ("t_h2d_ms", C.c_double), ("t_count_ms", C.c_double),
                ("t_mercy_ms", C.c_double), ("t_s2s_ms", C.c_double), ("t_d2h_ms", C.c_double),
                ("n_rounds_s1", C.c_uint32), ("n_rounds_s2", C.c_uint32)]


class CountOpts(C.Structure):
    _fields_ = [("k", C.c_uint32), ("m", C.c_int32), ("host_mem", C.c_double), ("num_cpu_threads", C.c_int32),
                ("read_lib_file", C.c_char_p), ("output_prefix", C.c_char_p), ("mem_flag", C.c_int32)]


class Seq2SdbgOpts(C.Structure):
    _fields_ = [("host_mem", C.c_double), ("k", C.c_uint32), ("k_from", C.c_uint32), ("num_cpu_threads", C.c_int32),
                ("contig", C.c_char_p), ("bubble", C.c_char_p), ("addi_contig", C.c_char_p),
                ("local_contig", C.c_char_p), ("input_prefix", C.c_char_p), ("output_prefix", C.c_char_p),
                ("need_mercy", C.c_int32), ("mem_flag", C.c_int32)]


class Read2SdbgOpts(C.Structure):
    _fields_ = [("k", C.c_uint32), ("m", C.c_int32), ("host_mem", C.c_double), ("num_cpu_threads", C.c_int32),
                ("read_lib_file", C.c_char_p), ("output_prefix", C.c_char_p), ("mem_flag", C.c_int32),
                ("need_mercy", C.c_int32)]


class IterateArgs(C.Structure):
    _fields_ = [("k", C.c_uint32), ("step", C.c_uint32), ("contig_words", C.c_void_p), ("contig_word_off", C.c_void_p),
                ("contig_len", C.c_void_p), ("n_contigs", C.c_uint64), ("bin", C.c_void_p), ("bin_words", C.c_uint64),
                ("n_reads", C.c_uint64)]


class IterateResult(C.Structure):
    _fields_ = [("n_flanks", C.c_uint64), ("n_aligned_reads", C.c_uint64), ("n_candidates", C.c_uint64), ("n_edges", C.c_uint64),
                ("words_per_edge", C.c_uint32), ("edges", C.POINTER(C.c_uint32)), ("t_total_ms", C.c_double)]


class IterateOpts(C.Structure):
    _fields_ = [("contig_file", C.c_char_p), ("bubble_file", C.c_char_p), ("read_file", C.c_char_p),
                ("num_cpu_threads", C.c_int32), ("k", C.c_uint32), ("step", C.c_uint32), ("output_prefix", C.c_char_p)]


class BuildlibLib(C.Structure):
    _fields_ = [("type", C.c_char_p), ("data", C.c_void_p * 2), ("size", C.c_uint64 * 2)]


class BuildlibArgs(C.Structure):
    _fields_ = [("libs", C.POINTER(BuildlibLib)), ("n_libs", C.c_uint32)]


class BuildlibResult(C.Structure):
    _fields_ = [("bin", C.POINTER(C.c_uint32)), ("bin_words", C.c_uint64), ("n_reads", C.c_uint64), ("n_bases", C.c_uint64),
                ("n_libs", C.c_uint32), ("lib_begin", C.POINTER(C.c_uint64)), ("lib_end", C.POINTER(C.c_uint64)),
                ("lib_max_len", C.POINTER(C.c_uint32)), ("n_chunks", C.c_uint64), ("n_walk_passes", C.c_uint64),
                ("t_total_ms", C.c_double)]


SYMBOLS = [
    "mhb_last_error", "mhb_version", "mhb_device_count", "mhb_launch_count", "mhb_count_record_words", "mhb_words_per_edge",
    "mhb_s2s_record_words", "mhb_count_sort_bytes", "mhb_s2s_sort_bytes", "mhb_sort_workspace_bytes",
    "mhb_count_extract", "mhb_count_extract_owners", "mhb_check_fixed_len", "mhb_count_extract_range", "mhb_set_round_limit", "mhb_set_s2s_round_limit", "mhb_set_r2s_round_limit", "mhb_plan_rounds", "mhb_plan_rounds16", "mhb_sort_records", "mhb_sort_records_relaxed", "mhb_sort_pass_ms", "mhb_partition_scatter", "mhb_partition_scatter_hist", "mhb_plan_partition", "mhb_compact_tip_edges", "mhb_dev_malloc", "mhb_dev_free",
    "mhb_ipc_export", "mhb_ipc_open", "mhb_ipc_close", "mhb_count_solid_scratch_bytes", "mhb_count_solid", "mhb_count_hashed_supported", "mhb_count_hashed_workspace_bytes", "mhb_count_solid_hashed", "mhb_tipset_bytes",
    "mhb_tipset_build", "mhb_count_mark_mercy", "mhb_count_tip_edges", "mhb_s2s_extract", "mhb_s2s_extract_range",
    "mhb_s2s_emit_scratch_bytes", "mhb_s2s_emit", "mhb_set_device", "mhb_count_host", "mhb_s2s_host", "mhb_build_host", "mhb_free",
    "mhb_mercy_candidates_scratch_bytes", "mhb_mercy_candidates", "mhb_mercy_edges_scratch_bytes", "mhb_mercy_edges", "mhb_mercy_edges_count", "mhb_mercy_edges_write", "mhb_mercy_edges_segs", "mhb_mercy_host", "mhb_mercy_planes_words", "mhb_mercy_probe_owned", "mhb_mercy_count_planes", "mhb_edge_lut_bytes", "mhb_edge_lut_build",
    "mhb_release", "mhb_count_run", "mhb_count_run_multi", "mhb_plan_count_owner_rounds", "mhb_seq2sdbg_run", "mhb_seq2sdbg_run_multi",
    "mhb_plan_seq_shares", "mhb_s2s_extract_owners","mhb_selftest_count_record", "mhb_selftest_count_records_roll", "mhb_selftest_s2s_record",
    "mhb_iterate_host", "mhb_iterate_run", "mhb_iterate_run_multi", "mhb_plan_read_shares", "mhb_selftest_iterate", "mhb_s2s_extract_edges_pruned", "mhb_s2s_emit_fmt", "mhb_read2sdbg_host", "mhb_read2sdbg_run", "mhb_read2sdbg_run_multi", "mhb_plan_r2s_owners", "mhb_selftest_r2s_s1_record", "mhb_selftest_r2s_item",
    "mhb_selftest_kmsort", "mhb_selftest_kmsort_smem", "mhb_selftest_r2s_s1_group", "mhb_selftest_r2s_mercy_read",
    "mhb_selftest_r2s_chunk_index", "mhb_selftest_r2s_stream_decide",
    "mhb_set_r2s_sparse_mercy", "mhb_r2s_mercy_stats", "mhb_selftest_r2s_mercy_form", "mhb_selftest_r2s_s1_cand",
    "mhb_selftest_r2s_mercy_lists",
    "mhb_selftest_kmsort_narrow", "mhb_selftest_r2s_s1_plan", "mhb_selftest_read2sdbg_narrow", "mhb_selftest_iterate_narrow",
    "mhb_buildlib_host", "mhb_buildlib_free", "mhb_set_buildlib_chunk", "mhb_buildlib_run", "mhb_selftest_fastx",
    "mhb_s2s_sort", "mhb_s2s_sort_workspace_bytes", "mhb_s2s_sort_hist_byte", "mhb_s2s_sort_stats",
    "mhb_s2s_sort_emit", "mhb_s2s_sort_emit_workspace_bytes",
    "mhb_selftest_s2s_local_key",
    "mhb_plan_read_chunks", "mhb_read_stream_decide", "mhb_set_read_chunk_limit", "mhb_read_stream_stats",
    "mhb_read_stream_times",
    "mhb_set_s2s_chunk_limit", "mhb_plan_seq_chunks", "mhb_plan_mercy_segments", "mhb_s2s_stream_stats",
    "mhb_s2s_stream_times", "mhb_selftest_s2s_stream_decide", "mhb_selftest_mercy_stream_decide",
    "mhb_selftest_mercy_auto_plan",
    "mhb_s2s_bucket_hist", "mhb_s2s_extract_owners_round", "mhb_s2s_edges_owners", "mhb_sdbg_round_budget",
]


def load():
    global _lib
    if _lib is not None:
        return _lib
    if not os.path.exists(LIB_PATH):
        raise MhbError(f"{LIB_PATH} is missing: build it with `make -C megahit_b200/csrc` "
                       "(there is no CPU fallback for the CUDA path)")
    L = C.CDLL(LIB_PATH)
    L.mhb_last_error.restype = C.c_char_p
    L.mhb_version.restype = C.c_char_p
    for f in ("mhb_count_record_words", "mhb_words_per_edge", "mhb_s2s_record_words", "mhb_count_sort_bytes",
              "mhb_s2s_sort_bytes"):
        getattr(L, f).restype = C.c_uint32
    for f in ("mhb_sort_workspace_bytes", "mhb_count_solid_scratch_bytes", "mhb_tipset_bytes",
              "mhb_s2s_emit_scratch_bytes"):
        getattr(L, f).restype = C.c_size_t
    L.mhb_sort_workspace_bytes.argtypes = [C.c_uint64, C.c_uint32]
    L.mhb_count_solid_scratch_bytes.argtypes = [C.c_uint64]
    L.mhb_tipset_bytes.argtypes = [C.c_uint64, C.c_uint32]
    L.mhb_s2s_emit_scratch_bytes.argtypes = [C.c_uint64, C.c_uint32]
    L.mhb_count_extract.argtypes = [C.c_void_p, C.POINTER(DevReads), C.c_uint32, C.c_void_p, C.c_uint64, C.c_void_p,
                                    C.c_int]
    L.mhb_sort_records.argtypes = [C.c_void_p, C.c_void_p, C.c_void_p, C.c_uint64, C.c_uint32, C.c_void_p, C.c_uint32,
                                   C.c_void_p, C.c_void_p, C.c_size_t, C.POINTER(C.c_int)]
    L.mhb_sort_records_relaxed.argtypes = L.mhb_sort_records.argtypes
    L.mhb_s2s_sort.argtypes = [C.c_void_p, C.c_void_p, C.c_void_p, C.c_uint64, C.c_uint32, C.c_void_p, C.c_void_p, C.c_size_t,
                               C.POINTER(C.c_int)]
    L.mhb_s2s_sort_workspace_bytes.argtypes = [C.c_uint64, C.c_uint32]
    L.mhb_s2s_sort_workspace_bytes.restype = C.c_size_t
    L.mhb_s2s_sort_hist_byte.argtypes = [C.c_uint64, C.c_uint32]
    L.mhb_s2s_sort_stats.argtypes = [C.POINTER(C.c_uint64), C.POINTER(C.c_uint64), C.POINTER(C.c_uint64)]
    L.mhb_s2s_sort_stats.restype = None
    L.mhb_s2s_sort_emit.argtypes = [C.c_void_p, C.c_void_p, C.c_void_p, C.c_uint64, C.c_uint32, C.c_void_p, C.c_void_p,
                                    C.c_uint64, C.c_void_p, C.c_void_p, C.c_void_p, C.c_size_t]
    L.mhb_s2s_sort_emit_workspace_bytes.argtypes = [C.c_uint64, C.c_uint32]
    L.mhb_s2s_sort_emit_workspace_bytes.restype = C.c_size_t
    L.mhb_selftest_s2s_local_key.argtypes = [C.c_void_p, C.c_uint64, C.c_uint32, C.c_void_p]
    L.mhb_count_solid.argtypes = [C.c_void_p, C.c_void_p, C.c_uint64, C.c_uint32, C.c_int32, C.c_void_p, C.c_void_p,
                                  C.c_uint64, C.c_void_p, C.c_void_p, C.c_void_p, C.c_size_t]
    L.mhb_count_hashed_workspace_bytes.restype = C.c_size_t
    L.mhb_count_hashed_workspace_bytes.argtypes = [C.c_uint64, C.c_uint32, C.c_int32]
    L.mhb_count_hashed_supported.argtypes = [C.c_uint32, C.c_int32]
    L.mhb_count_solid_hashed.argtypes = [C.c_void_p, C.c_void_p, C.c_void_p, C.c_uint64, C.c_uint32, C.c_int32, C.c_void_p,
                                         C.c_void_p, C.c_void_p, C.c_uint64, C.c_void_p, C.c_void_p, C.c_void_p, C.c_size_t]
    L.mhb_tipset_build.argtypes = [C.c_void_p, C.c_void_p, C.c_void_p, C.c_uint64, C.c_uint32, C.c_void_p, C.c_size_t,
                                   C.c_uint64]
    L.mhb_count_mark_mercy.argtypes = [C.c_void_p, C.POINTER(DevReads), C.c_uint32, C.c_void_p, C.c_size_t, C.c_uint64,
                                       C.c_void_p, C.c_void_p]
    L.mhb_count_tip_edges.argtypes = [C.c_void_p, C.c_void_p, C.c_uint64, C.POINTER(C.c_uint64)]
    L.mhb_s2s_extract.argtypes = [C.c_void_p, C.POINTER(DevSeqs), C.c_uint32, C.c_void_p, C.c_uint64, C.c_void_p,
                                  C.c_int]
    L.mhb_s2s_emit.argtypes = [C.c_void_p, C.c_void_p, C.c_uint64, C.c_uint32, C.c_void_p, C.c_uint64, C.c_void_p,
                               C.c_void_p, C.c_void_p, C.c_size_t]
    L.mhb_count_host.argtypes = [C.POINTER(CountArgs), C.POINTER(CountResult)]
    L.mhb_s2s_host.argtypes = [C.POINTER(S2sArgs), C.POINTER(S2sResult)]
    L.mhb_build_host.argtypes = [C.POINTER(BuildArgs), C.POINTER(BuildResult)]
    L.mhb_mercy_candidates_scratch_bytes.restype = C.c_size_t
    L.mhb_mercy_candidates_scratch_bytes.argtypes = [C.c_uint64]
    L.mhb_mercy_edges_scratch_bytes.restype = C.c_size_t
    L.mhb_mercy_edges_scratch_bytes.argtypes = [C.c_uint64, C.c_uint32]
    L.mhb_mercy_candidates.argtypes = [C.c_void_p, C.c_void_p, C.c_void_p, C.c_uint64, C.c_void_p, C.POINTER(C.c_uint64),
                                       C.c_void_p, C.c_size_t]
    L.mhb_mercy_edges.argtypes = [C.c_void_p, C.POINTER(DevReads), C.c_void_p, C.c_uint64, C.c_uint32, C.c_uint32,
                                  C.c_void_p, C.c_uint64, C.c_void_p, C.c_uint64, C.POINTER(C.c_uint64), C.c_void_p,
                                  C.c_size_t]
    L.mhb_mercy_edges_segs.argtypes = [C.c_void_p, C.POINTER(DevReads), C.c_void_p, C.c_uint64, C.c_uint32, C.c_uint32,
                                       C.c_uint32, C.c_void_p, C.c_void_p, C.c_void_p, C.c_void_p, C.c_void_p, C.c_uint64,
                                       C.POINTER(C.c_uint64), C.c_void_p, C.c_size_t]
    L.mhb_mercy_edges_count.argtypes = [C.c_void_p, C.POINTER(DevReads), C.c_void_p, C.c_uint64, C.c_uint32, C.c_uint32,
                                        C.c_uint32, C.c_void_p, C.c_void_p, C.c_void_p, C.c_void_p, C.POINTER(C.c_uint64),
                                        C.c_void_p, C.c_size_t]
    L.mhb_mercy_edges_write.argtypes = [C.c_void_p, C.POINTER(DevReads), C.c_void_p, C.c_uint64, C.c_uint32, C.c_uint32,
                                        C.c_void_p, C.c_uint64, C.c_uint64, C.c_void_p, C.c_size_t]
    L.mhb_mercy_planes_words.restype = C.c_size_t
    L.mhb_mercy_planes_words.argtypes = [C.c_uint64, C.c_uint32]
    L.mhb_mercy_probe_owned.argtypes = [C.c_void_p, C.POINTER(DevReads), C.c_void_p, C.c_uint64, C.c_uint32, C.c_uint32,
                                        C.c_void_p, C.c_uint64, C.c_void_p, C.c_void_p, C.c_uint32, C.c_void_p]
    L.mhb_mercy_count_planes.argtypes = [C.c_void_p, C.POINTER(DevReads), C.c_void_p, C.c_uint64, C.c_uint32, C.c_uint32,
                                         C.c_void_p, C.c_uint32, C.c_uint64, C.POINTER(C.c_uint64), C.c_void_p, C.c_size_t]
    L.mhb_plan_partition.argtypes = [C.c_void_p, C.c_void_p, C.c_uint32, C.c_uint32, C.c_uint32, C.c_void_p, C.c_void_p,
                                     C.c_void_p, C.c_void_p]
    L.mhb_edge_lut_bytes.restype = C.c_size_t
    L.mhb_edge_lut_build.argtypes = [C.c_void_p, C.c_void_p, C.c_uint64, C.c_uint32, C.c_void_p]
    L.mhb_sort_pass_ms.argtypes = [C.c_int, C.c_void_p, C.c_uint32, C.POINTER(C.c_uint32), C.POINTER(C.c_uint64),
                                   C.POINTER(C.c_uint32)]
    L.mhb_set_device.argtypes = [C.c_int]
    L.mhb_partition_scatter.argtypes = [C.c_void_p, C.c_void_p, C.c_uint64, C.c_uint32, C.c_int, C.c_void_p, C.c_void_p,
                                        C.c_void_p, C.c_size_t]
    L.mhb_partition_scatter_hist.argtypes = [C.c_void_p, C.c_void_p, C.c_uint64, C.c_uint32, C.c_int, C.c_void_p, C.c_void_p,
                                             C.c_void_p, C.c_size_t, C.c_int, C.c_void_p]
    L.mhb_dev_malloc.argtypes = [C.POINTER(C.c_void_p), C.c_size_t]
    L.mhb_dev_free.argtypes = [C.c_void_p]
    L.mhb_ipc_export.argtypes = [C.c_void_p, C.c_void_p]
    L.mhb_ipc_open.argtypes = [C.c_void_p, C.POINTER(C.c_void_p)]
    L.mhb_ipc_close.argtypes = [C.c_void_p]
    L.mhb_free.argtypes = [C.c_void_p]
    L.mhb_count_run.argtypes = [C.POINTER(CountOpts)]
    L.mhb_count_run_multi.argtypes = [C.POINTER(CountOpts), C.c_int]
    L.mhb_count_extract_owners.argtypes = [C.c_void_p, C.POINTER(DevReads), C.c_uint32, C.c_void_p, C.c_void_p, C.c_void_p,
                                           C.c_void_p, C.c_void_p, C.c_void_p, C.c_void_p]
    L.mhb_plan_count_owner_rounds.argtypes = [C.c_void_p, C.c_uint32, C.c_uint64, C.c_uint32, C.c_void_p, C.c_void_p,
                                              C.c_void_p, C.c_void_p, C.c_void_p, C.c_void_p, C.POINTER(C.c_uint32)]
    L.mhb_seq2sdbg_run.argtypes = [C.POINTER(Seq2SdbgOpts)]
    L.mhb_seq2sdbg_run_multi.argtypes = [C.POINTER(Seq2SdbgOpts), C.c_int]
    L.mhb_plan_seq_shares.argtypes = [C.c_void_p, C.c_uint64, C.c_uint32, C.c_uint32, C.c_void_p]
    L.mhb_s2s_extract_range.argtypes = [C.c_void_p, C.POINTER(DevSeqs), C.c_uint32, C.c_void_p, C.c_uint64, C.c_uint32,
                                        C.c_uint32, C.c_void_p, C.c_uint64, C.c_void_p, C.c_int]
    L.mhb_s2s_extract_owners.argtypes = [C.c_void_p, C.POINTER(DevSeqs), C.c_uint32, C.c_uint64, C.c_void_p, C.c_void_p,
                                         C.c_void_p, C.c_void_p]
    L.mhb_s2s_bucket_hist.argtypes = [C.c_void_p, C.POINTER(DevSeqs), C.c_uint32, C.c_uint64, C.c_void_p]
    L.mhb_s2s_extract_owners_round.argtypes = L.mhb_s2s_extract_owners.argtypes + [C.c_void_p, C.c_void_p]
    L.mhb_s2s_edges_owners.argtypes = [C.c_void_p, C.c_void_p, C.c_void_p, C.c_uint64, C.c_uint64, C.c_uint32, C.c_void_p,
                                       C.c_void_p, C.c_void_p, C.c_void_p, C.c_void_p, C.c_void_p, C.c_void_p]
    L.mhb_sdbg_round_budget.argtypes = [C.c_uint64, C.c_uint64, C.c_uint32, C.c_uint64]
    L.mhb_sdbg_round_budget.restype = C.c_uint64
    L.mhb_selftest_count_record.argtypes = [C.c_void_p, C.c_uint32, C.c_uint32, C.c_uint32, C.c_uint32, C.c_void_p,
                                            C.POINTER(C.c_uint32)]
    L.mhb_selftest_count_records_roll.argtypes = [C.c_void_p, C.c_uint32, C.c_uint32, C.c_uint32, C.c_uint32, C.c_void_p,
                                                  C.c_void_p]
    L.mhb_selftest_s2s_record.argtypes = [C.c_void_p, C.c_uint32, C.c_uint32, C.c_uint32, C.c_uint32, C.c_uint32,
                                          C.c_uint32, C.c_void_p]
    L.mhb_s2s_emit_fmt.argtypes = L.mhb_s2s_emit.argtypes + [C.c_int]
    L.mhb_iterate_host.argtypes = [C.POINTER(IterateArgs), C.POINTER(IterateResult)]
    L.mhb_selftest_iterate.argtypes = [C.POINTER(IterateArgs), C.POINTER(IterateResult)]
    L.mhb_iterate_run.argtypes = [C.POINTER(IterateOpts)]
    L.mhb_iterate_run_multi.argtypes = [C.POINTER(IterateOpts), C.c_int]
    L.mhb_plan_read_shares.argtypes = [C.c_void_p, C.c_uint64, C.c_uint64, C.c_uint32, C.c_void_p]
    L.mhb_s2s_extract_edges_pruned.argtypes = [C.c_void_p, C.c_void_p, C.c_void_p, C.c_uint64, C.c_uint64, C.c_uint32,
                                               C.c_void_p, C.c_uint64, C.c_void_p, C.c_void_p, C.c_int]
    L.mhb_read2sdbg_host.argtypes = [C.POINTER(BuildArgs), C.POINTER(BuildResult)]
    L.mhb_read2sdbg_run.argtypes = [C.POINTER(Read2SdbgOpts)]
    L.mhb_read2sdbg_run_multi.argtypes = [C.POINTER(Read2SdbgOpts), C.c_int]
    L.mhb_plan_r2s_owners.argtypes = [C.c_void_p, C.c_uint32, C.c_void_p, C.c_void_p]
    L.mhb_selftest_r2s_s1_record.argtypes = [C.c_void_p, C.c_uint32, C.c_uint32, C.c_uint32, C.c_uint32, C.c_uint64, C.c_void_p]
    L.mhb_selftest_r2s_item.argtypes = [C.c_void_p, C.c_uint32, C.c_uint32, C.c_uint32, C.c_uint32, C.c_uint32, C.c_uint32,
                                        C.c_void_p, C.POINTER(C.c_uint32)]
    L.mhb_selftest_kmsort.argtypes = [C.c_void_p, C.c_uint64, C.c_uint32]
    L.mhb_selftest_kmsort_smem.argtypes = [C.c_void_p, C.c_uint64, C.c_uint32, C.c_uint32, C.c_uint32]
    L.mhb_selftest_kmsort_narrow.argtypes = [C.c_void_p, C.c_uint64, C.c_uint32, C.c_int, C.c_uint32, C.c_uint32]
    L.mhb_selftest_read2sdbg_narrow.argtypes = [C.POINTER(BuildArgs), C.POINTER(BuildResult)]
    L.mhb_selftest_iterate_narrow.argtypes = [C.POINTER(IterateArgs), C.POINTER(IterateResult)]
    L.mhb_selftest_r2s_s1_group.argtypes = [C.c_void_p, C.c_uint64, C.c_uint32, C.c_int32, C.c_uint32, C.c_uint64, C.c_int,
                                            C.c_void_p, C.c_void_p, C.c_void_p, C.c_void_p, C.c_void_p]
    L.mhb_selftest_r2s_mercy_read.argtypes = [C.c_uint32, C.c_uint64, C.c_uint64, C.c_uint32, C.c_void_p, C.c_void_p, C.c_void_p,
                                              C.c_void_p, C.c_void_p, C.POINTER(C.c_uint32)]
    L.mhb_buildlib_host.argtypes = [C.POINTER(BuildlibArgs), C.POINTER(BuildlibResult)]
    L.mhb_buildlib_free.argtypes = [C.POINTER(BuildlibResult)]
    L.mhb_buildlib_free.restype = None
    L.mhb_set_buildlib_chunk.argtypes = [C.c_uint64]
    L.mhb_buildlib_run.argtypes = [C.c_char_p, C.c_char_p]
    L.mhb_selftest_fastx.argtypes = [C.c_void_p, C.c_uint64, C.c_void_p, C.c_void_p, C.c_uint64, C.POINTER(C.c_uint64),
                                     C.c_void_p, C.c_uint64, C.POINTER(C.c_uint64)]
    _lib = L
    return L


def _check(rc: int):
    if rc != 0:
        raise MhbError(f"libmhb error {rc}: {load().mhb_last_error().decode()}")


def device_count() -> int:
    return load().mhb_device_count()


def launch_count() -> int:
    L = load()
    L.mhb_launch_count.restype = C.c_uint64
    return int(L.mhb_launch_count())


def plan_rounds(hist256, max_records: int):
    L = load()
    h = np.ascontiguousarray(hist256, dtype=np.uint64)
    assert h.shape == (256,)
    lo, hi = (C.c_uint32 * 256)(), (C.c_uint32 * 256)()
    L.mhb_plan_rounds.argtypes = [C.c_void_p, C.c_uint64, C.c_void_p, C.c_void_p]
    n = L.mhb_plan_rounds(h.ctypes.data, int(max_records), lo, hi)
    if n < 0:
        raise MhbError(L.mhb_last_error().decode())
    return [(int(lo[i]), int(hi[i])) for i in range(n)]


def plan_rounds16(hist256, sub_hist, max_records: int, cap: int = 65536):
    L = load()
    h = np.ascontiguousarray(hist256, dtype=np.uint64)
    sub = None if sub_hist is None else np.ascontiguousarray(sub_hist, dtype=np.uint64).reshape(256, 256)
    lo, hi = (C.c_uint32 * cap)(), (C.c_uint32 * cap)()
    L.mhb_plan_rounds16.argtypes = [C.c_void_p, C.c_void_p, C.c_uint64, C.c_void_p, C.c_void_p, C.c_uint32]
    n = L.mhb_plan_rounds16(h.ctypes.data, sub.ctypes.data if sub is not None else None, int(max_records), lo, hi, cap)
    if n < 0:
        raise MhbError(L.mhb_last_error().decode())
    return [(int(lo[i]), int(hi[i])) for i in range(n)]


def set_round_limit(max_records: int = 0):
    L = load()
    L.mhb_set_round_limit.argtypes = [C.c_uint64]
    _check(L.mhb_set_round_limit(int(max_records)))


def set_s2s_round_limit(max_items: int = 0):
    L = load()
    L.mhb_set_s2s_round_limit.argtypes = [C.c_uint64]
    _check(L.mhb_set_s2s_round_limit(int(max_items)))


def sdbg_round_budget(avail_bytes: int, fixed_bytes: int, k: int, n_total: int) -> int:
    return int(load().mhb_sdbg_round_budget(int(avail_bytes), int(fixed_bytes), int(k), int(n_total)))


def set_r2s_round_limit(s1: int = 0, s2: int = 0):
    L = load()
    L.mhb_set_r2s_round_limit.argtypes = [C.c_uint64, C.c_uint64]
    _check(L.mhb_set_r2s_round_limit(int(s1), int(s2)))


def set_r2s_sparse_mercy(mode: int = 0):
    L = load()
    L.mhb_set_r2s_sparse_mercy.argtypes = [C.c_int]
    _check(L.mhb_set_r2s_sparse_mercy(int(mode)))


def r2s_mercy_stats() -> dict:
    L = load()
    sp, n, b = C.c_int(), C.c_uint64(), C.c_uint64()
    L.mhb_r2s_mercy_stats.argtypes = [C.POINTER(C.c_int), C.POINTER(C.c_uint64), C.POINTER(C.c_uint64)]
    _check(L.mhb_r2s_mercy_stats(C.byref(sp), C.byref(n), C.byref(b)))
    return {"sparse": bool(sp.value), "n_entries": n.value, "host_bytes": b.value}


def r2s_mercy_form(n_bases: int, max_plane_words: int, streamed_bytes: int, m: int, need_mercy: bool, free_bytes: int,
                   force: int = 0) -> dict:
    L = load()
    pl, li, sp = C.c_uint64(), C.c_uint64(), C.c_int()
    L.mhb_selftest_r2s_mercy_form.argtypes = [C.c_uint64, C.c_uint64, C.c_uint64, C.c_int32, C.c_int, C.c_uint64, C.c_int,
                                              C.POINTER(C.c_uint64), C.POINTER(C.c_uint64), C.POINTER(C.c_int)]
    _check(L.mhb_selftest_r2s_mercy_form(n_bases, max_plane_words, streamed_bytes, m, int(need_mercy), free_bytes,
                                         int(force), C.byref(pl), C.byref(li), C.byref(sp)))
    return {"planes": pl.value, "lists": li.value, "sparse": bool(sp.value)}


def selftest_r2s_s1_cand(recs: np.ndarray, k: int, m: int, fixed_len: int, n_reads: int, is_solid: np.ndarray,
                         counting: np.ndarray) -> np.ndarray:
    L = load()
    recs = np.ascontiguousarray(recs, np.uint32)
    out = np.zeros(2 * len(recs) + 1, np.uint64)
    n = C.c_uint64()
    L.mhb_selftest_r2s_s1_cand.argtypes = [C.c_void_p, C.c_uint64, C.c_uint32, C.c_int32, C.c_uint32, C.c_uint64,
                                           C.c_void_p, C.c_void_p, C.c_void_p, C.POINTER(C.c_uint64)]
    _check(L.mhb_selftest_r2s_s1_cand(recs.ctypes.data, len(recs), k, m, fixed_len, n_reads, is_solid.ctypes.data,
                                      counting.ctypes.data, out.ctypes.data, C.byref(n)))
    return out[:n.value].copy()


def selftest_r2s_mercy_lists(k: int, is_solid: np.ndarray, n_reads: int, fixed_len: int = 0, lens=None, base0: int = 0,
                             rounds=None, chunk_first=None, planes=None) -> tuple[np.ndarray, int]:
    L = load()
    is_solid = np.ascontiguousarray(is_solid, np.uint32)
    mercy = np.zeros_like(is_solid)
    lens_a = np.ascontiguousarray(lens if lens is not None else [0], np.uint32)
    added = C.c_uint64()
    L.mhb_selftest_r2s_mercy_lists.argtypes = [C.c_uint32, C.c_uint64, C.c_void_p, C.c_uint64, C.c_uint32, C.c_void_p,
                                               C.c_void_p, C.c_void_p, C.c_uint32, C.c_void_p, C.c_uint32, C.c_void_p,
                                               C.c_uint64, C.c_void_p, C.POINTER(C.c_uint64)]
    if planes is not None:
        planes = np.ascontiguousarray(planes, np.uint32)
        _check(L.mhb_selftest_r2s_mercy_lists(fixed_len, n_reads, lens_a.ctypes.data, base0, k, is_solid.ctypes.data,
                                              None, None, 0, None, 0, planes.ctypes.data, planes.shape[1],
                                              mercy.ctypes.data, C.byref(added)))
        return mercy, added.value
    ent = np.ascontiguousarray(np.concatenate([np.asarray(r, np.uint64) for r in rounds] + [np.zeros(1, np.uint64)]))
    ends = np.cumsum([len(r) for r in rounds]).astype(np.uint64)
    cf = np.ascontiguousarray(chunk_first, np.uint64)
    _check(L.mhb_selftest_r2s_mercy_lists(fixed_len, n_reads, lens_a.ctypes.data, base0, k, is_solid.ctypes.data,
                                          ent.ctypes.data, ends.ctypes.data, len(rounds), cf.ctypes.data, len(cf) - 1,
                                          None, 0, mercy.ctypes.data, C.byref(added)))
    return mercy, added.value


def plan_read_chunks(bin_words: np.ndarray, n_reads: int, max_chunk_bytes: int) -> list[int]:
    L = load()
    b = np.ascontiguousarray(bin_words, np.uint32).reshape(-1)
    L.mhb_plan_read_chunks.argtypes = [C.c_void_p, C.c_uint64, C.c_uint64, C.c_uint64, C.c_void_p, C.c_uint32]
    n = L.mhb_plan_read_chunks(b.ctypes.data if len(b) else None, len(b), int(n_reads), int(max_chunk_bytes), None, 0)
    if n < 0:
        raise MhbError(L.mhb_last_error().decode())
    first = np.zeros(n + 1, np.uint64)
    n = L.mhb_plan_read_chunks(b.ctypes.data if len(b) else None, len(b), int(n_reads), int(max_chunk_bytes),
                               first.ctypes.data, n + 1)
    if n < 0:
        raise MhbError(L.mhb_last_error().decode())
    return [int(x) for x in first]


def read_stream_decide(resident_bytes: int, avail_bytes: int, plan_failed: bool = False, chunk_limit: int = 0) -> bool:
    L = load()
    L.mhb_read_stream_decide.argtypes = [C.c_uint64, C.c_uint64, C.c_int, C.c_uint64]
    return bool(L.mhb_read_stream_decide(int(resident_bytes), int(avail_bytes), int(plan_failed), int(chunk_limit)))


def set_read_chunk_limit(n_bytes: int = 0) -> None:
    L = load()
    L.mhb_set_read_chunk_limit.argtypes = [C.c_uint64]
    _check(L.mhb_set_read_chunk_limit(int(n_bytes)))


def read_stream_stats() -> dict:
    L = load()
    nc, npass, nb = C.c_uint64(), C.c_uint64(), C.c_uint64()
    L.mhb_read_stream_stats.argtypes = [C.POINTER(C.c_uint64)] * 3
    _check(L.mhb_read_stream_stats(C.byref(nc), C.byref(npass), C.byref(nb)))
    h2d, kern, fill, wall = C.c_double(), C.c_double(), C.c_double(), C.c_double()
    L.mhb_read_stream_times.argtypes = [C.POINTER(C.c_double)] * 4
    _check(L.mhb_read_stream_times(C.byref(h2d), C.byref(kern), C.byref(fill), C.byref(wall)))
    return {"n_chunks": nc.value, "n_passes": npass.value, "h2d_bytes": nb.value, "h2d_ms": h2d.value,
            "kernel_ms": kern.value, "fill_ms": fill.value, "pass_ms": wall.value}


def set_s2s_chunk_limit(n_bytes: int = 0) -> None:
    L = load()
    L.mhb_set_s2s_chunk_limit.argtypes = [C.c_uint64]
    _check(L.mhb_set_s2s_chunk_limit(int(n_bytes)))


def plan_seq_chunks(word_off: np.ndarray, length: np.ndarray, k: int, max_chunk_bytes: int) -> list[int]:
    L = load()
    wo = np.ascontiguousarray(word_off, np.uint64)
    ln = np.ascontiguousarray(length, np.uint32)
    n = len(wo) - 1
    L.mhb_plan_seq_chunks.argtypes = [C.c_void_p, C.c_void_p, C.c_uint64, C.c_uint32, C.c_uint64, C.c_void_p, C.c_uint32]
    args = (wo.ctypes.data if n else None, ln.ctypes.data if n else None, n, k, int(max_chunk_bytes))
    nc = L.mhb_plan_seq_chunks(*args, None, 0)
    if nc < 0:
        raise MhbError(L.mhb_last_error().decode())
    first = np.zeros(nc + 1, np.uint64)
    if L.mhb_plan_seq_chunks(*args, first.ctypes.data, nc + 1) < 0:
        raise MhbError(L.mhb_last_error().decode())
    return [int(x) for x in first]


def plan_mercy_segments(edges: np.ndarray, k: int, max_segment_bytes: int) -> list[int]:
    L = load()
    e = np.ascontiguousarray(edges, np.uint32).reshape(-1)
    n = len(e) // words_per_edge(k)
    L.mhb_plan_mercy_segments.argtypes = [C.c_void_p, C.c_uint64, C.c_uint32, C.c_uint64, C.c_void_p, C.c_uint32]
    first = np.zeros(257, np.uint32)
# ... 479 lines not shown
```

Before: 18.79 billion.

## Fuse first radix partition pass into tiled count extraction with segmented gather

Extraction now runs in tiles that locally partition records by byte 5 in shared memory, recording per-tile segment counts and source offsets. The first sort pass then gathers records through a scanned segment table instead of running a full byte-5 radix pass, so the hashed count sorts only bytes 6 and 7. This removes one global read/scatter pass over all records. In exchange extraction does more work (shared-memory scatter, segment tables), and the first sort pass does irregular segment lookups during its loads.

```diff
diff --git a/include/mhb.h b/include/mhb.h
--- a/include/mhb.h
+++ b/include/mhb.h
@@ -99,6 +99,14 @@
 int mhb_count_solid_hashed(void *stream, uint32_t *recs_a, uint32_t *recs_b, uint64_t n, uint32_t k, int32_t m,
                            const uint64_t *hist_byte5, uint32_t *edges_out, uint8_t *aux_out, uint64_t capacity_edges,
                            uint64_t *mul_hist, uint64_t *n_solid_out, void *ws, size_t ws_bytes);
+
+size_t mhb_count_tiles_bytes(uint64_t n_edges);
+int mhb_count_extract_tiles(void *stream, const mhb_dev_reads *reads, uint32_t k, uint32_t *records, uint64_t n_edges,
+                            void *tiles, size_t tiles_bytes);
+int mhb_count_solid_hashed_tiles(void *stream, uint32_t *recs_a, uint32_t *recs_b, uint64_t n, uint32_t k, int32_t m,
+                                 void *tiles, size_t tiles_bytes, uint32_t *edges_out, uint8_t *aux_out,
+                                 uint64_t capacity_edges, uint64_t *mul_hist, uint64_t *n_solid_out, void *ws,
+                                 size_t ws_bytes);
 
 size_t mhb_tipset_bytes(uint64_t n_tip_edges, uint32_t k);
 int mhb_tipset_build(void *stream, const uint32_t *edges, const uint8_t *aux, uint64_t n_solid, uint32_t k,
diff --git a/megahit_b200/csrc/mhb_count.cuh b/megahit_b200/csrc/mhb_count.cuh
--- a/megahit_b200/csrc/mhb_count.cuh
+++ b/megahit_b200/csrc/mhb_count.cuh
@@ -103,6 +103,131 @@
   if (hist)
     for (int i = threadIdx.x; i < 256; i += kExtractThreads)
       if (s_hist[i]) atomicAdd((unsigned long long *)&hist[i], (unsigned long long)s_hist[i]);
+}
+
+struct CountTileGeom {
+  static constexpr int THREADS = 384;
+  static constexpr int IPT = 18;
+  static constexpr int TILE = THREADS * IPT;
+  static constexpr int STAGE_WORDS = 2048;
+  static constexpr size_t SMEM = (size_t)TILE * 8 + STAGE_WORDS * 4 + 3 * 256 * 4 + 16 * 4;
+};
+static constexpr int kTilePartByte = 5, kTileNextByte = 6;
+
+template <int W>
+__global__ void __launch_bounds__(CountTileGeom::THREADS, 2)
+    k_count_extract_tiles(ReadsView rv, u32 k, u64 n, u64 n_tiles, u32 *__restrict__ records, u32 *__restrict__ seg_cnt,
+                          u64 *__restrict__ seg_src, u64 *hist_next) {
+  using G = CountTileGeom;
+  constexpr int THREADS = G::THREADS, IPT = G::IPT, TILE = G::TILE;
+  extern __shared__ __align__(16) unsigned char smem_raw[];
+  u32 *s_recs = reinterpret_cast<u32 *>(smem_raw);
+  u32 *s_stage = s_recs + TILE * 2;
+  u32 *s_cnt = s_stage + G::STAGE_WORDS;
+  u32 *s_base = s_cnt + 256;
+  u32 *s_next = s_base + 256;
+  u32 *s_misc = s_next + 256;
+  const u32 tid = threadIdx.x, lane = tid & 31, warp = tid >> 5;
+  for (int i = tid; i < 512; i += THREADS) s_cnt[i] = 0;
+  for (int i = tid; i < 256; i += THREADS) s_next[i] = 0;
+  const u32 E = rv.fixed_len > k ? rv.fixed_len - k : 0u;
+
+  for (u64 t = blockIdx.x; t < n_tiles; t += gridDim.x) {
+    const u64 p0 = t * TILE;
+    const u32 len = n - p0 < (u64)TILE ? (u32)(n - p0) : (u32)TILE;
+    u64 r0, r1;
+    if (rv.fixed_len) {
+      r0 = p0 / E;
+      r1 = (p0 + len - 1) / E;
+    } else {
+      if (tid < 2) {
+        const u64 p = tid ? p0 + len - 1 : p0;
+        u64 lo = 0, hi = rv.n_reads - 1;
+        while (lo < hi) {
+          const u64 mid = (lo + hi + 1) >> 1;
+          if (rv.edge_off[mid] <= p) lo = mid;
+          else hi = mid - 1;
+        }
+        reinterpret_cast<u64 *>(s_misc + 8)[tid] = lo;
+      }
+      __syncthreads();
+      r0 = reinterpret_cast<const u64 *>(s_misc + 8)[0];
+      r1 = reinterpret_cast<const u64 *>(s_misc + 8)[1];
+    }
+    const u64 w0 = rv.rec_start(r0), w1 = r1 + 1 < rv.n_reads ? rv.rec_start(r1 + 1) : rv.bin_words;
+    const bool staged = w1 - w0 <= (u64)G::STAGE_WORDS;
+    if (staged)
+      for (u32 i = tid; i < (u32)(w1 - w0); i += THREADS) s_stage[i] = rv.bin[w0 + i];
+    __syncthreads();
+
+    u32 rec[IPT][2], rk[IPT];
+#pragma unroll
+    for (int i = 0; i < IPT; ++i) {
+      const u32 j = (u32)i * THREADS + tid;
+      if (j < len) {
+        const u64 p = p0 + j;
+        u64 r;
+        u32 q;
+        if (rv.fixed_len) {
+          const u32 rel = (u32)(p - r0 * E);
+          r = r0 + rel / E;
+          q = rel - (u32)(r - r0) * E;
+        } else {
+          u64 lo = r0, hi = r1;
+          while (lo < hi) {
+            const u64 mid = (lo + hi + 1) >> 1;
+            if (rv.edge_off[mid] <= p) lo = mid;
+            else hi = mid - 1;
+          }
+          r = lo;
+          q = (u32)(p - rv.edge_off[r]);
+        }
+        const u64 ws = rv.rec_start(r);
+        const u32 *s = staged ? s_stage + (ws - w0) : rv.bin + ws;
+        const u32 L = s[0];
+        u32 strand;
+        make_count_record<W, 2>(s + 1, div_ceil(L, 16), L, k, q, rec[i], strand);
+        rk[i] = atomicAdd(&s_cnt[rec_byte<2>(rec[i], kTilePartByte)], 1u);
+      }
+    }
+    __syncthreads();
+
+    if (tid < 256) {
+      const u32 c = s_cnt[tid];
+      s_cnt[tid] = 0;
+      u32 inc = c;
+#pragma unroll
+      for (int dd = 1; dd < 32; dd <<= 1) {
+        const u32 v = __shfl_up_sync(0xffffffffu, inc, dd);
+        if (lane >= (u32)dd) inc += v;
+      }
+      if (lane == 31) s_misc[warp] = inc;
+      s_base[tid] = inc - c;
+      seg_cnt[(u64)tid * n_tiles + t] = c;
+    }
+    __syncthreads();
+    if (tid < 256) {
+      u32 excl = s_base[tid];
+#pragma unroll
+      for (int w = 0; w < 7; ++w) excl += (warp > (u32)w) ? s_misc[w] : 0u;
+      s_base[tid] = excl;
+      seg_src[(u64)tid * n_tiles + t] = p0 + excl;
+    }
+    __syncthreads();
+#pragma unroll
+    for (int i = 0; i < IPT; ++i)
+      if ((u32)i * THREADS + tid < len) st_rec<2>(s_recs, s_base[rec_byte<2>(rec[i], kTilePartByte)] + rk[i], rec[i]);
+    __syncthreads();
+    for (u32 j = tid; j < len; j += THREADS) {
+      u32 q[2];
+      ld_rec<2>(s_recs, j, q);
+      st_rec<2>(records, p0 + j, q);
+      atomicAdd(&s_next[rec_byte<2>(q, kTileNextByte)], 1u);
+    }
+    __syncthreads();
+  }
+  for (int i = tid; i < 256; i += THREADS)
+    if (s_next[i]) atomicAdd((unsigned long long *)&hist_next[i], (unsigned long long)s_next[i]);
 }
 
 static __global__ void __launch_bounds__(kExtractThreads)
diff --git a/megahit_b200/csrc/mhb_device.cu b/megahit_b200/csrc/mhb_device.cu
--- a/megahit_b200/csrc/mhb_device.cu
+++ b/megahit_b200/csrc/mhb_device.cu
@@ -147,6 +147,41 @@
   else
   MHB_FOR_W(M) return mhb_set_error(MHB_ERR_ARG, "unsupported k=%u", k);
 #undef M
+  CK_LAUNCH();
+  return MHB_OK;
+}
+
+static_assert(CountTileGeom::TILE == kCountTileRecs, "tile of the segment table");
+
+extern "C" size_t mhb_count_tiles_bytes(uint64_t n_edges) { return count_tiles_layout(n_edges).total; }
+
+extern "C" int mhb_count_extract_tiles(void *stream, const mhb_dev_reads *reads, uint32_t k, uint32_t *records,
+                                       uint64_t n_edges, void *tiles, size_t tiles_bytes) {
+  if (int rc = check_reads(reads, k)) return rc;
+  if (count_record_words(k) != 2) return mhb_set_error(MHB_ERR_ARG, "tile extraction needs 8-byte records (k <= 28), k=%u", k);
+  const CountTilesLayout TL = count_tiles_layout(n_edges);
+  if (!tiles || tiles_bytes < TL.total) return mhb_set_error(MHB_ERR_ARG, "tile table too small (%zu < %zu)", tiles_bytes, TL.total);
+  if (!records && n_edges) return mhb_set_error(MHB_ERR_ARG, "null records");
+  cudaStream_t st = (cudaStream_t)stream;
+  CK(cudaMemsetAsync(tiles, 0, 256 * 8, st));
+  if (reads->n_reads == 0 || n_edges == 0) return MHB_OK;
+  const ReadsView rv = make_reads_view(reads);
+  if (rv.fixed_len && (rv.fixed_len <= k || n_edges != rv.n_reads * (u64)(rv.fixed_len - k)))
+    return mhb_set_error(MHB_ERR_ARG, "n_edges does not match the fixed-length library");
+  char *t = (char *)tiles;
+  u32 *seg_cnt = (u32 *)(t + TL.off_cnt);
+  u64 *seg_src = (u64 *)(t + TL.off_src);
+  using G = CountTileGeom;
+  static int bps = 0;
+  if (!bps) {
+    CK(cudaFuncSetAttribute(k_count_extract_tiles<1>, cudaFuncAttributeMaxDynamicSharedMemorySize, (int)G::SMEM));
+    CK(cudaFuncSetAttribute(k_count_extract_tiles<2>, cudaFuncAttributeMaxDynamicSharedMemorySize, (int)G::SMEM));
+    CK(cudaOccupancyMaxActiveBlocksPerMultiprocessor(&bps, k_count_extract_tiles<2>, G::THREADS, G::SMEM));
+    if (bps < 1) return mhb_set_error(MHB_ERR_CUDA, "tile extraction does not fit an SM");
+  }
+  const u64 grid = std::min<u64>(TL.n_tiles, (u64)bps * sm_count());
+  auto kern = count_key_words(k) == 1 ? k_count_extract_tiles<1> : k_count_extract_tiles<2>;
+  kern<<<(unsigned)grid, G::THREADS, G::SMEM, st>>>(rv, k, n_edges, TL.n_tiles, records, seg_cnt, seg_src, (u64 *)t);
   CK_LAUNCH();
   return MHB_OK;
 }
diff --git a/megahit_b200/csrc/mhb_hashcount.cu b/megahit_b200/csrc/mhb_hashcount.cu
--- a/megahit_b200/csrc/mhb_hashcount.cu
+++ b/megahit_b200/csrc/mhb_hashcount.cu
@@ -506,6 +506,10 @@
 
 }
 
+static int count_grouped(cudaStream_t st, const uint2 *recs, uint64_t n, uint32_t k, int32_t m, const HcLayout &L, void *ws,
+                         uint32_t *edges_out, uint8_t *aux_out, uint64_t capacity_edges, uint64_t *mul_hist,
+                         uint64_t *n_solid_out);
+
 extern "C" int mhb_count_hashed_supported(uint32_t k, int32_t m) {
   return count_record_words(k) == 2 && 2 * (k + 1) >= 24 && m >= 1 && m <= kHcHist;
 }
@@ -529,7 +533,39 @@
   const uint8_t bytes[3] = {5, 6, 7};
   int in_b = 0;
   if (int rc = mhb_sort_records_impl(st, recs_a, recs_b, n, 2, bytes, 3, hist_byte5, ws, L.sort_ws, &in_b, nullptr)) return rc;
-  const uint2 *recs = (const uint2 *)(in_b ? recs_b : recs_a);
+  return count_grouped(st, (const uint2 *)(in_b ? recs_b : recs_a), n, k, m, L, ws, edges_out, aux_out, capacity_edges,
+                       mul_hist, n_solid_out);
+}
+
+extern "C" int mhb_count_solid_hashed_tiles(void *stream, uint32_t *recs_a, uint32_t *recs_b, uint64_t n, uint32_t k,
+                                            int32_t m, void *tiles, size_t tiles_bytes, uint32_t *edges_out,
+                                            uint8_t *aux_out, uint64_t capacity_edges, uint64_t *mul_hist,
+                                            uint64_t *n_solid_out, void *ws, size_t ws_bytes) {
+  if (!mhb_count_hashed_supported(k, m)) return mhb_set_error(MHB_ERR_ARG, "hashed count needs 8-byte records (13 <= k <= 28) and 1 <= m <= %d", kHcHist);
+  if (!mul_hist || !n_solid_out || !ws || !tiles) return mhb_set_error(MHB_ERR_ARG, "bad args");
+  if (n == 0) return MHB_OK;
+  if (n >= (1ull << 40)) return mhb_set_error(MHB_ERR_ARG, "too many records for one hashed count call");
+  const HcLayout L = hc_layout(n, m);
+  if (ws_bytes < L.total) return mhb_set_error(MHB_ERR_ARG, "hashed count workspace too small (%zu < %zu)", ws_bytes, L.total);
+  const CountTilesLayout TL = count_tiles_layout(n);
+  if (tiles_bytes < TL.total) return mhb_set_error(MHB_ERR_ARG, "tile table too small (%zu < %zu)", tiles_bytes, TL.total);
+  cudaStream_t st = (cudaStream_t)stream;
+  char *t = (char *)tiles;
+  u64 *vstart = (u64 *)(t + TL.off_vstart), *total = (u64 *)(t + TL.off_total);
+  if (int rc = scan_counts(st, (const u32 *)(t + TL.off_cnt), TL.n_seg, vstart, total, (u64 *)(t + TL.off_bsum))) return rc;
+  CK(cudaMemcpyAsync(vstart + TL.n_seg, total, 8, cudaMemcpyDeviceToDevice, st));
+  const uint8_t bytes[2] = {6, 7};
+  int in_b = 0;
+  if (int rc = mhb_sort_records_segmented(st, recs_a, recs_b, n, bytes, 2, (const u64 *)t, vstart, (const u64 *)(t + TL.off_src),
+                                          TL.n_seg, (u32 *)(t + TL.off_first), ws, L.sort_ws, &in_b))
+    return rc;
+  return count_grouped(st, (const uint2 *)(in_b ? recs_b : recs_a), n, k, m, L, ws, edges_out, aux_out, capacity_edges,
+                       mul_hist, n_solid_out);
+}
+
+static int count_grouped(cudaStream_t st, const uint2 *recs, uint64_t n, uint32_t k, int32_t m, const HcLayout &L, void *ws,
+                         uint32_t *edges_out, uint8_t *aux_out, uint64_t capacity_edges, uint64_t *mul_hist,
+                         uint64_t *n_solid_out) {
   char *w = (char *)ws;
   u64 *bounds = (u64 *)(w + L.off_bounds);
   u32 *bcnt = (u32 *)(w + L.off_bcnt);
diff --git a/megahit_b200/csrc/mhb_internal.h b/megahit_b200/csrc/mhb_internal.h
--- a/megahit_b200/csrc/mhb_internal.h
+++ b/megahit_b200/csrc/mhb_internal.h
@@ -86,6 +86,35 @@
 int mhb_sort_records_ex(void *stream, uint32_t *a, uint32_t *b, uint64_t n, uint32_t words, const uint8_t *bytes,
                         uint32_t n_bytes, const uint64_t *first_hist, void *ws, size_t ws_bytes, int *result_in_b,
                         double *pass_ms_host, int relaxed);
+constexpr uint64_t kCountTileRecs = 6912;
+struct CountTilesLayout {
+  uint64_t n_tiles, n_seg;
+  size_t off_total, off_cnt, off_src, off_vstart, off_first, off_bsum, total;
+};
+inline CountTilesLayout count_tiles_layout(uint64_t n) {
+  auto pad = [](size_t b) { return (b + 255) & ~(size_t)255; };
+  CountTilesLayout L;
+  L.n_tiles = (n + kCountTileRecs - 1) / kCountTileRecs;
+  L.n_seg = 256 * L.n_tiles;
+  size_t p = 256 * 8;
+  L.off_total = p;
+  p += 256;
+  L.off_cnt = p;
+  p += pad(L.n_seg * 4);
+  L.off_src = p;
+  p += pad(L.n_seg * 8);
+  L.off_vstart = p;
+  p += pad((L.n_seg + 1) * 8);
+  L.off_first = p;
+  p += pad((L.n_tiles + 1) * 4);
+  L.off_bsum = p;
+  p += pad((L.n_seg / 4096 + 4) * 8);
+  L.total = p;
+  return L;
+}
+int mhb_sort_records_segmented(void *stream, uint32_t *a, uint32_t *b, uint64_t n, const uint8_t *bytes, uint32_t n_bytes,
+                               const uint64_t *first_hist, const uint64_t *seg_vstart, const uint64_t *seg_src,
+                               uint64_t n_seg, uint32_t *first_seg, void *ws, size_t ws_bytes, int *result_in_b);
 int mhb_sort_records_untraced(void *stream, uint32_t *a, uint32_t *b, uint64_t n, uint32_t words, const uint8_t *bytes,
                               uint32_t n_bytes, const uint64_t *first_hist, void *ws, size_t ws_bytes, int *result_in_b);
 
diff --git a/megahit_b200/csrc/mhb_sort3.cuh b/megahit_b200/csrc/mhb_sort3.cuh
--- a/megahit_b200/csrc/mhb_sort3.cuh
+++ b/megahit_b200/csrc/mhb_sort3.cuh
@@ -159,11 +159,77 @@
 #define MHB_TL_FLUSH() ((void)0)
 #endif
 
-template <int WR, bool HAS_NEXT = true>
+struct SegView {
+  const u64 *vstart;
+  const u64 *src;
+  const u32 *first_seg;
+  u64 n_seg;
+};
+static constexpr int kSegCap = 384;
+static constexpr size_t kSegSmem = (size_t)kSegCap * 12;
+
+static __global__ void k_seg_first(const u64 *__restrict__ vstart, u64 n_seg, u32 tile, u64 num_tiles, u32 *__restrict__ first_seg) {
+  const u64 t = (u64)blockIdx.x * blockDim.x + threadIdx.x;
+  if (t >= num_tiles) return;
+  const u64 v = t * tile;
+  u64 lo = 0, hi = n_seg - 1;
+  while (lo < hi) {
+    const u64 mid = (lo + hi + 1) >> 1;
+    if (vstart[mid] <= v) lo = mid;
+    else hi = mid - 1;
+  }
+  first_seg[t] = (u32)lo;
+}
+
+template <int WR>
+__device__ __forceinline__ void load_tile_segmented(const u32 *__restrict__ in, u64 n, u32 t, const SegView &seg,
+                                                    u32 *s_seg ,
+                                                    u32 (&r)[SortGeom<WR>::IPT][WR]) {
+  using G = SortGeom<WR>;
+  constexpr int IPT = G::IPT, TILE = G::TILE;
+  u64 *s_delta = reinterpret_cast<u64 *>(s_seg);
+  u32 *s_start = s_seg + 2 * kSegCap;
+  const u32 tid = threadIdx.x, lane = tid & 31, warp = tid >> 5;
+  const u64 tb = (u64)t * TILE;
+  const u64 s0 = seg.first_seg[t];
+  auto start_rel = [&](u64 x) -> u32 {
+    if (s0 + x >= seg.n_seg) return (u32)TILE;
+    const u64 v = seg.vstart[s0 + x];
+    return v <= tb ? 0u : (v - tb >= (u64)TILE ? (u32)TILE : (u32)(v - tb));
+  };
+  auto delta = [&](u64 x) -> u64 { return seg.src[s0 + x] - seg.vstart[s0 + x]; };
+  static_assert(G::THREADS == kSegCap, "one descriptor per thread");
+  s_start[tid] = start_rel(tid);
+  s_delta[tid] = s0 + tid < seg.n_seg ? delta(tid) : 0ull;
+  __syncthreads();
+  const u32 v0 = warp * 32 * IPT + lane;
+  u32 g = 0;
+  {
+    u32 hi = kSegCap - 1;
+    while (g < hi) {
+      const u32 mid = (g + hi + 1) >> 1;
+      if (s_start[mid] <= v0) g = mid;
+      else hi = mid - 1;
+    }
+  }
+#pragma unroll
+  for (int i = 0; i < IPT; ++i) {
+    const u32 v = v0 + (u32)i * 32;
+    if (tb + v < n) {
+      while ((g + 1 < (u32)kSegCap ? s_start[g + 1] : start_rel(g + 1)) <= v) ++g;
+      ld_rec_pinned<WR>(in, tb + v + (g < (u32)kSegCap ? s_delta[g] : delta(g)), r[i]);
+    } else {
+#pragma unroll
+      for (int j = 0; j < WR; ++j) r[i][j] = 0xFFFFFFFFu;
+    }
+  }
+}
+
+template <int WR, bool HAS_NEXT = true, bool SEG = false>
 __global__ void __launch_bounds__(SortGeom<WR>::THREADS, SortGeom<WR>::MIN_BLOCKS)
     k_radix_pass3(const u32 *__restrict__ in, u64 n, u32 num_tiles, int byte_idx,
                   const u64 *__restrict__ bin_addr , u64 *lookback,
-                  u32 *tile_counter, u64 *next_hist, int next_byte, u32 epoch) {
+                  u32 *tile_counter, u64 *next_hist, int next_byte, u32 epoch, SegView seg) {
   using G = SortGeom<WR>;
   constexpr int THREADS = G::THREADS, IPT = G::IPT, TILE = G::TILE, NW = G::NW;
   constexpr int LB1 = 1, LBW = 2;
@@ -191,6 +257,10 @@
 
   u32 r[IPT][WR];
   auto load_tile = [&](u32 t) {
+    if constexpr (SEG) {
+      load_tile_segmented<WR>(in, n, t, seg, reinterpret_cast<u32 *>(s_recs + TILE * WR), r);
+      return;
+    }
     const u64 tb = (u64)t * TILE;
     const u64 warp_base = tb + (u64)warp * 32 * IPT + lane;
     if (tb + TILE <= n) {
diff --git a/megahit_b200/csrc/mhb_sortdisp.cu b/megahit_b200/csrc/mhb_sortdisp.cu
--- a/megahit_b200/csrc/mhb_sortdisp.cu
+++ b/megahit_b200/csrc/mhb_sortdisp.cu
@@ -22,6 +22,7 @@
 #undef M
   return 0;
 }
+static_assert(SortGeom<2>::TILE == kCountTileRecs, "first_seg holds one entry per tile of the segment table");
 static constexpr size_t kSortHeadBytes = (size_t)(72 + 1) * 256 * 8  + 256 * 8  + 128 * 4 + 256 * 8 ;
 
 extern "C" size_t mhb_sort_workspace_bytes(uint64_t n, uint32_t words) {
@@ -45,10 +46,30 @@
   if (grid > tiles) grid = tiles;
   if (next_hist)
     k_radix_pass3<WR, true><<<(int)grid, G::THREADS, G::SMEM, st>>>(in, n, (u32)tiles, byte_idx, bin_base, lookback,
-                                                                     tile_counter, next_hist, next_byte, epoch);
+                                                                     tile_counter, next_hist, next_byte, epoch, SegView{});
   else
     k_radix_pass3<WR, false><<<(int)grid, G::THREADS, G::SMEM, st>>>(in, n, (u32)tiles, byte_idx, bin_base, lookback,
-                                                                      tile_counter, nullptr, 0, epoch);
+                                                                      tile_counter, nullptr, 0, epoch, SegView{});
+  CK_LAUNCH();
+  return MHB_OK;
+}
+
+static int launch_radix_pass_seg(cudaStream_t st, const u32 *in, u64 n, int byte_idx, const u64 *bin_base, u64 *lookback,
+                                 u32 *tile_counter, u64 *next_hist, int next_byte, u32 epoch, const SegView &seg) {
+  using G = SortGeom<2>;
+  constexpr size_t SMEM = G::SMEM + kSegSmem;
+  static int blocks_per_sm = 0;
+  if (!blocks_per_sm) {
+    CK(cudaFuncSetAttribute(k_radix_pass3<2, true, true>, cudaFuncAttributeMaxDynamicSharedMemorySize, (int)SMEM));
+    CK(cudaOccupancyMaxActiveBlocksPerMultiprocessor(&blocks_per_sm, k_radix_pass3<2, true, true>, G::THREADS, SMEM));
+    if (blocks_per_sm < 1) return mhb_set_error(MHB_ERR_CUDA, "segmented radix pass does not fit an SM");
+    if (getenv("MHB_VERBOSE")) fprintf(stderr, "[mhb] segmented radix pass: %d threads x %d rec, %zu B smem, %d CTA/SM\n", G::THREADS, G::IPT, SMEM, blocks_per_sm);
+  }
+  const u64 tiles = sort_tiles<2>(n);
+  u64 grid = (u64)blocks_per_sm * sm_count();
+  if (grid > tiles) grid = tiles;
+  k_radix_pass3<2, true, true><<<(int)grid, G::THREADS, SMEM, st>>>(in, n, (u32)tiles, byte_idx, bin_base, lookback, tile_counter,
+                                                                     next_hist, next_byte, epoch, seg);
   CK_LAUNCH();
   return MHB_OK;
 }
@@ -101,7 +122,7 @@
 
 static int sort_records_core(void *stream, uint32_t *a, uint32_t *b, uint64_t n, uint32_t words, const uint8_t *bytes,
                              uint32_t n_bytes, const uint64_t *first_hist, void *ws, size_t ws_bytes, int *result_in_b,
-                             double *pass_ms_host, int relaxed, bool trace);
+                             double *pass_ms_host, int relaxed, bool trace, const SegView *seg = nullptr);
 int mhb_sort_records_impl(void *stream, uint32_t *a, uint32_t *b, uint64_t n, uint32_t words, const uint8_t *bytes,
                           uint32_t n_bytes, const uint64_t *first_hist, void *ws, size_t ws_bytes, int *result_in_b,
                           double *pass_ms_host) {
@@ -116,9 +137,20 @@
                               uint32_t n_bytes, const uint64_t *first_hist, void *ws, size_t ws_bytes, int *result_in_b) {
   return sort_records_core(stream, a, b, n, words, bytes, n_bytes, first_hist, ws, ws_bytes, result_in_b, nullptr, 1, false);
 }
+int mhb_sort_records_segmented(void *stream, uint32_t *a, uint32_t *b, uint64_t n, const uint8_t *bytes, uint32_t n_bytes,
+                               const uint64_t *first_hist, const uint64_t *seg_vstart, const uint64_t *seg_src,
+                               uint64_t n_seg, uint32_t *first_seg, void *ws, size_t ws_bytes, int *result_in_b) {
+  if (n == 0 || n_bytes == 0 || n_seg == 0) return sort_records_core(stream, a, b, n, 2, bytes, n_bytes, first_hist, ws, ws_bytes, result_in_b, nullptr, 1, true);
+  if (n_seg >= (1ull << 32)) return mhb_set_error(MHB_ERR_ARG, "too many segments (%llu)", (unsigned long long)n_seg);
+  const u64 tiles = sort_tiles<2>(n);
+  k_seg_first<<<(unsigned)((tiles + 255) / 256), 256, 0, (cudaStream_t)stream>>>(seg_vstart, n_seg, SortGeom<2>::TILE, tiles, first_seg);
+  CK_LAUNCH();
+  const SegView seg{seg_vstart, seg_src, first_seg, n_seg};
+  return sort_records_core(stream, a, b, n, 2, bytes, n_bytes, first_hist, ws, ws_bytes, result_in_b, nullptr, 1, true, &seg);
+}
 static int sort_records_core(void *stream, uint32_t *a, uint32_t *b, uint64_t n, uint32_t words, const uint8_t *bytes,
                              uint32_t n_bytes, const uint64_t *first_hist, void *ws, size_t ws_bytes, int *result_in_b,
-                             double *pass_ms_host, int relaxed, bool trace) {
+                             double *pass_ms_host, int relaxed, bool trace, const SegView *seg) {
   if (pass_ms_host && !trace) return mhb_set_error(MHB_ERR_ARG, "per-pass times need a traced sort");
   if (words < 1 || words > 17 || n_bytes > 72 || !result_in_b)
     return mhb_set_error(MHB_ERR_ARG, "bad sort geometry (words=%u n_bytes=%u)", words, n_bytes);
@@ -161,7 +193,8 @@
     u64 *next_hist = p + 1 < n_bytes ? hist + (u64)(p + 1) * 256 : nullptr;
     const int next_byte = p + 1 < n_bytes ? bytes[p + 1] : 0;
     int rc = MHB_ERR_ARG;
-    if (p == 0 && relaxed && words == 2) rc = launch_part_unstable<2, false>(st, in, n, bytes[p], bin_base, gcursor, tile_counter + p, next_hist, next_byte, nullptr);
+    if (p == 0 && seg) rc = launch_radix_pass_seg(st, in, n, bytes[p], bin_base, lookback, tile_counter + p, next_hist, next_byte, p + 1, *seg);
+    else if (p == 0 && relaxed && words == 2) rc = launch_part_unstable<2, false>(st, in, n, bytes[p], bin_base, gcursor, tile_counter + p, next_hist, next_byte, nullptr);
     else if (p == 0 && relaxed && words == 3) rc = launch_part_unstable<3, false>(st, in, n, bytes[p], bin_base, gcursor, tile_counter + p, next_hist, next_byte, nullptr);
     else {
 #define M(WW) \
diff --git a/megahit_b200/dev.py b/megahit_b200/dev.py
--- a/megahit_b200/dev.py
+++ b/megahit_b200/dev.py
@@ -73,6 +73,7 @@
         self.b = torch.empty(n * self.WR + 4, **i32)
         if self.hashed:
             self.ws = torch.empty(L.mhb_count_hashed_workspace_bytes(n, k, m), dtype=torch.uint8, device=device)
+            self.tiles = torch.empty(L.mhb_count_tiles_bytes(n), dtype=torch.uint8, device=device)
             self.scratch = None
         else:
             self.ws = torch.empty(L.mhb_sort_workspace_bytes(n, self.WR), dtype=torch.uint8, device=device)
@@ -97,6 +98,10 @@
         self.events.setdefault(name, []).append(ev)
 
     def extract(self, bin_dev):
+        if self.hashed:
+            lib._check(self.L.mhb_count_extract_tiles(_stream(), C.byref(self._reads(bin_dev)), self.k, _ptr(self.a), self.n,
+                                                      _ptr(self.tiles), self.tiles.numel()))
+            return
         self.hist0.zero_()
         lib._check(self.L.mhb_count_extract(_stream(), C.byref(self._reads(bin_dev)), self.k, _ptr(self.a), self.n,
                                             _ptr(self.hist0), 5 if self.hashed else self.sort_bytes[0]))
@@ -111,9 +116,10 @@
         self.mul_hist.zero_()
         self.n_solid_dev.zero_()
         if self.hashed:
-            lib._check(self.L.mhb_count_solid_hashed(_stream(), _ptr(self.a), _ptr(self.b), self.n, self.k, self.m,
-                                                     _ptr(self.hist0), _ptr(self.edges), _ptr(self.aux), self.cap_edges,
-                                                     _ptr(self.mul_hist), _ptr(self.n_solid_dev), _ptr(self.ws), self.ws.numel()))
+            lib._check(self.L.mhb_count_solid_hashed_tiles(_stream(), _ptr(self.a), _ptr(self.b), self.n, self.k, self.m,
+                                                           _ptr(self.tiles), self.tiles.numel(), _ptr(self.edges), _ptr(self.aux),
+                                                           self.cap_edges, _ptr(self.mul_hist), _ptr(self.n_solid_dev),
+                                                           _ptr(self.ws), self.ws.numel()))
             return
         lib._check(self.L.mhb_count_solid(_stream(), _ptr(self.sorted), self.n, self.k, self.m, _ptr(self.edges),
                                           _ptr(self.aux), self.cap_edges, _ptr(self.mul_hist), _ptr(self.n_solid_dev),
diff --git a/megahit_b200/lib.py b/megahit_b200/lib.py
--- a/megahit_b200/lib.py
+++ b/megahit_b200/lib.py
@@ -127,7 +127,7 @@
     "mhb_last_error", "mhb_version", "mhb_device_count", "mhb_launch_count", "mhb_count_record_words", "mhb_words_per_edge",
     "mhb_s2s_record_words", "mhb_count_sort_bytes", "mhb_s2s_sort_bytes", "mhb_sort_workspace_bytes",
     "mhb_count_extract", "mhb_count_extract_owners", "mhb_check_fixed_len", "mhb_count_extract_range", "mhb_set_round_limit", "mhb_set_s2s_round_limit", "mhb_set_r2s_round_limit", "mhb_plan_rounds", "mhb_plan_rounds16", "mhb_sort_records", "mhb_sort_records_relaxed", "mhb_sort_pass_ms", "mhb_partition_scatter", "mhb_partition_scatter_hist", "mhb_plan_partition", "mhb_compact_tip_edges", "mhb_dev_malloc", "mhb_dev_free",
-    "mhb_ipc_export", "mhb_ipc_open", "mhb_ipc_close", "mhb_count_solid_scratch_bytes", "mhb_count_solid", "mhb_count_hashed_supported", "mhb_count_hashed_workspace_bytes", "mhb_count_solid_hashed", "mhb_tipset_bytes",
+    "mhb_ipc_export", "mhb_ipc_open", "mhb_ipc_close", "mhb_count_solid_scratch_bytes", "mhb_count_solid", "mhb_count_hashed_supported", "mhb_count_hashed_workspace_bytes", "mhb_count_solid_hashed", "mhb_count_tiles_bytes", "mhb_count_extract_tiles", "mhb_count_solid_hashed_tiles", "mhb_tipset_bytes",
     "mhb_tipset_build", "mhb_count_mark_mercy", "mhb_count_tip_edges", "mhb_s2s_extract", "mhb_s2s_extract_range",
     "mhb_s2s_emit_scratch_bytes", "mhb_s2s_emit", "mhb_set_device", "mhb_count_host", "mhb_s2s_host", "mhb_build_host", "mhb_free",
     "mhb_mercy_candidates_scratch_bytes", "mhb_mercy_candidates", "mhb_mercy_edges_scratch_bytes", "mhb_mercy_edges", "mhb_mercy_edges_count", "mhb_mercy_edges_write", "mhb_mercy_edges_segs", "mhb_mercy_host", "mhb_mercy_planes_words", "mhb_mercy_probe_owned", "mhb_mercy_count_planes", "mhb_edge_lut_bytes", "mhb_edge_lut_build",
@@ -196,6 +196,13 @@
     L.mhb_count_hashed_supported.argtypes = [C.c_uint32, C.c_int32]
     L.mhb_count_solid_hashed.argtypes = [C.c_void_p, C.c_void_p, C.c_void_p, C.c_uint64, C.c_uint32, C.c_int32, C.c_void_p,
                                          C.c_void_p, C.c_void_p, C.c_uint64, C.c_void_p, C.c_void_p, C.c_void_p, C.c_size_t]
+    L.mhb_count_tiles_bytes.restype = C.c_size_t
+    L.mhb_count_tiles_bytes.argtypes = [C.c_uint64]
+    L.mhb_count_extract_tiles.argtypes = [C.c_void_p, C.POINTER(DevReads), C.c_uint32, C.c_void_p, C.c_uint64, C.c_void_p,
+                                          C.c_size_t]
+    L.mhb_count_solid_hashed_tiles.argtypes = [C.c_void_p, C.c_void_p, C.c_void_p, C.c_uint64, C.c_uint32, C.c_int32,
+                                               C.c_void_p, C.c_size_t, C.c_void_p, C.c_void_p, C.c_uint64, C.c_void_p,
+                                               C.c_void_p, C.c_void_p, C.c_size_t]
     L.mhb_tipset_build.argtypes = [C.c_void_p, C.c_void_p, C.c_void_p, C.c_uint64, C.c_uint32, C.c_void_p, C.c_size_t,
                                    C.c_uint64]
     L.mhb_count_mark_mercy.argtypes = [C.c_void_p, C.POINTER(DevReads), C.c_uint32, C.c_void_p, C.c_size_t, C.c_uint64,
```

Result: no change. 18.91 billion, median of 6 (+0.7%).
